# Sbte/RAILS

Hardware: AMD Instinct MI355X
Metric: RAILS iterations/sec (+ A*V SpMM HBM GB/s in roofline), m=1M rows/GPU, k=128, fp64 (higher is better)
Workload: dtype f64

## Files before the change

### include/rails_hip.h

```cpp
#ifndef RAILS_HIP_H
#define RAILS_HIP_H

#include <stddef.h>
#include <stdint.h>

#ifdef __cplusplus
extern "C" {
#endif

#define RAILS_OK 0
#define RAILS_EINVAL -1
#define RAILS_EHIP -2
#define RAILS_ENOMEM -3
#define RAILS_ELAPACK -4
#define RAILS_ECOMM -5
#define RAILS_ENODEV -6

typedef struct rails_ctx rails_ctx;
typedef struct rails_csr rails_csr;
typedef struct rails_panel rails_panel;

const char *rails_last_error(void);
const char *rails_version(void);

// ... 49 lines not shown
typedef struct rails_sptrsv rails_sptrsv;
int rails_sptrsv_create(rails_ctx *ctx, int64_t n, const int64_t *rowptr, const int32_t *col, const double *val, int lower, int unit_diag,
                        rails_sptrsv **out);
void rails_sptrsv_destroy(rails_sptrsv *T);
int64_t rails_sptrsv_levels(const rails_sptrsv *T);
int rails_sptrsv_solve(rails_ctx *ctx, const rails_sptrsv *T, rails_panel *X, int c0, int nc);
int rails_panel_permute_rows(rails_ctx *ctx, const rails_panel *X, int xc0, int nc, const int32_t *perm_dev, int scatter, rails_panel *Y, int yc0);
int rails_index_upload(rails_ctx *ctx, const int32_t *host, int64_t n, int32_t **out_dev);
void rails_index_free(rails_ctx *ctx, int32_t *dev);

typedef struct rails_lu rails_lu;
int rails_lu_create(rails_ctx *ctx, int64_t n, const int64_t *L_rowptr, const int32_t *L_col, const double *L_val, const int64_t *U_rowptr,
                    const int32_t *U_col, const double *U_val, const int32_t *perm_r, const int32_t *perm_c, const int32_t *rows, int64_t m_sub,
                    rails_lu **out);
void rails_lu_destroy(rails_lu *lu);
int rails_lu_solve(rails_ctx *ctx, rails_lu *lu, int trans, const rails_panel *X, int xc0, int nc, rails_panel *Y, int yc0);
int rails_lu_stats(const rails_lu *lu, int64_t *info, int cap);
int rails_csr_create_lu(rails_ctx *ctx, rails_lu *lu, rails_csr **out);


int rails_csr_transpose_host(int64_t n_rows, int64_t n_cols, const int64_t *rowptr, const int32_t *col, const double *val, int64_t *t_rowptr,
                             int32_t *t_col, double *t_val);
int rails_csr_gram_norm2_host(int64_t n_rows, int64_t n_cols, const int64_t *rowptr, const int32_t *col, const double *val,
                              const int64_t *t_rowptr, const int32_t *t_col, const double *t_val, double *out);

typedef struct rails_sprhs rails_sprhs;
int rails_sprhs_create(rails_ctx *ctx, int64_t m_local, int p, const int64_t *rowptr, const int32_t *col, const double *val, rails_sprhs **out);
void rails_sprhs_destroy(rails_sprhs *S);
int64_t rails_sprhs_rows(const rails_sprhs *S);
int64_t rails_sprhs_cols(const rails_sprhs *S);
int64_t rails_sprhs_nnz(const rails_sprhs *S);
double rails_sprhs_gram_norm2(const rails_sprhs *S);
int rails_sprhs_apply(rails_ctx *ctx, rails_sprhs *S, int trans, const rails_panel *X, int xc0, int nc, rails_panel *Y, int yc0);
int rails_csr_create_sprhs(rails_ctx *ctx, rails_sprhs *S, rails_csr **out);
int64_t rails_csr_cols(const rails_csr *A);
rails_sprhs *rails_csr_sprhs(const rails_csr *A);

typedef struct rails_sweep_plan rails_sweep_plan;
int rails_sweep_plan_create(int64_t m, int64_t ncols, const int64_t *rowptr, const int32_t *col, const double *val,
                            const int *params, rails_sweep_plan **out);
int rails_sweep_plan_destroy(rails_sweep_plan *plan);
int rails_sweep_plan_info(const rails_sweep_plan *plan, int64_t *iinfo, double *dinfo);
int rails_sweep_plan_array(const rails_sweep_plan *plan, int which, const void **ptr, int64_t *count);


int rails_panel_create(rails_ctx *ctx, int64_t m_local, int capacity, rails_panel **out);
int rails_panel_create_ld(rails_ctx *ctx, int64_t m_local, int capacity, int ld, rails_panel **out);
int rails_panel_destroy(rails_panel *P);
int64_t rails_panel_rows(const rails_panel *P);
int rails_panel_capacity(const rails_panel *P);
int rails_panel_ld(const rails_panel *P);
void *rails_panel_device_ptr(const rails_panel *P);
int rails_panel_reserve(rails_ctx *ctx, rails_panel *P, int capacity);

int rails_panel_upload(rails_ctx *ctx, rails_panel *P, int c0, int nc, const double *host, int64_t ldh);
int rails_panel_download(rails_ctx *ctx, const rails_panel *P, int c0, int nc, double *host, int64_t ldh);

int rails_panel_fill(rails_ctx *ctx, rails_panel *P, int c0, int nc, double value);
int rails_panel_scale(rails_ctx *ctx, rails_panel *P, int c0, int nc, double s);
int rails_panel_copy(rails_ctx *ctx, const rails_panel *X, int xc0, int nc, rails_panel *Y, int yc0);
int rails_panel_axpy(rails_ctx *ctx, double alpha, const rails_panel *X, int xc0, int nc, rails_panel *Y,
                     int yc0);
int rails_panel_random(rails_ctx *ctx, rails_panel *P, int c0, int nc);

int rails_gram(rails_ctx *ctx, const rails_panel *X, int xc0, int a, const rails_panel *Y, int yc0, int b,
               double *C_host, int ldc);

int rails_panel_gemm(rails_ctx *ctx, double alpha, const rails_panel *X, int xc0, int k, const double *C_host,
                     int ldc, int r, double beta, rails_panel *Y, int yc0);

int rails_ctx_enable_library_gemm(rails_ctx *ctx);
int rails_ctx_library_gemm_ready(const rails_ctx *ctx);

int rails_deferred_reserve(rails_ctx *ctx, int nslots, int64_t doubles_per_slot);
int rails_gram_deferred(rails_ctx *ctx, const rails_panel *X, int xc0, int a, const rails_panel *Y, int yc0, int b, int slot);
int rails_panel_gemm_deferred(rails_ctx *ctx, double alpha, const rails_panel *X, int xc0, int k, int slot, int ld, int r, double beta,
                              rails_panel *Y, int yc0);
int rails_chol_inverse_deferred(rails_ctx *ctx, int slot_in, int w, int slot_out);
int rails_update_gram_deferred(rails_ctx *ctx, double alpha, const rails_panel *X, int xc0, int k, const double *C_host, int ldc, int r,
                               rails_panel *Y, int yc0, int r2, int slot);
int rails_update_gram_deferred_out(rails_ctx *ctx, double alpha, const rails_panel *X, int xc0, int k, const double *C_host, int ldc, int r,
                                   const rails_panel *Y, int yc0, rails_panel *Yout, int oc0, int r2, int slot);
int rails_deferred_fetch(rails_ctx *ctx, int slot, int64_t n, double *host_out);

int rails_panel_gemm_wide(rails_ctx *ctx, double alpha, const rails_panel *X, int xc0, int k, const double *C_host, int ldc, int r,
                          double beta, rails_panel *Y, int yc0);

void rails_dense_set_tile_fit(int on);
int rails_dense_tile_fit(void);
int rails_dense_last_tiles(const rails_ctx *ctx, int *update_gram_nbw, int *gram_cols_ti, int *gemm_wide_tr);

int rails_orthogonalize(rails_ctx *ctx, rails_panel *V, int k_old, int w, int method, int *used);
int rails_orthogonalize_deflated(rails_ctx *ctx, rails_panel *V, int k_old, int w, const rails_panel *N, int nc0, int q, int method, int *used);

int rails_panel_colnorms2(rails_ctx *ctx, const rails_panel *X, int c0, int nc, double *out_host);

int rails_orthogonalize_range(rails_ctx *ctx, rails_panel *V, int k_old, int w, const rails_panel *N, int nc0, int q, double tol, int *kept,
                              int32_t *kept_idx);

int rails_resid_lanczos(rails_ctx *ctx, const rails_panel *AV, int avc0, const rails_panel *MV, int mvc0, int k,
                        const double *T_host, int ldt, const rails_panel *B, int bc0, int p, int L,
                        double *H_host, int ldh, int *steps);

int rails_resid_lanczos_sparse(rails_ctx *ctx, const rails_panel *AV, int avc0, const rails_panel *MV, int mvc0, int k, const double *T_host,
                               int ldt, const rails_sprhs *S, int L, double *H_host, int ldh, int *steps);

int rails_lanczos_start(rails_ctx *ctx, const rails_panel *AV, int avc0, const rails_panel *MV, int mvc0, int k,
                        const rails_panel *B, int bc0, int p, double *sums_host);

int rails_lanczos_vectors(rails_ctx *ctx, const double *S_host, int lds, int w, rails_panel *Out, int oc0);
int rails_lanczos_last_launch(rails_ctx *ctx, int *nch, int *unroll, int *nblocks);
int rails_lanczos_release(rails_ctx *ctx);

int rails_ctx_reserve_staging(rails_ctx *ctx, size_t bytes);
int rails_timer_start(rails_ctx *ctx);
int rails_timer_stop(rails_ctx *ctx, double *ms);


void rails_sb03md(char dico, char job, char fact, char trans, int n, double *A, int lda, double *X, int ldx,
                  double *scale, int *info);
void rails_sb03md_counts(long *smith, long *schur);
void rails_sb03md_adi_counts(long *extended, long *fresh);
void rails_sb03md_set_pause(int calls);
void rails_dsyev(char jobz, char uplo, int n, double *a, int lda, double *w, int *info);
void rails_dsteqr(char compz, int n, double *d, double *e, double *z, int ldz, double *work, int *info);
void rails_dgemm(char transa, char transb, int m, int n, int k, double alpha, const double *A, int lda, const double *B,
                 int ldb, double beta, double *C, int ldc);
void rails_dtrsm(char side, char uplo, char transa, char diag, int m, int n, double alpha, const double *A, int lda, double *B, int ldb);
void rails_dpotrf(char uplo, int n, double *a, int lda, int *info);
void rails_dpstrf(char uplo, int n, double *a, int lda, int *piv, int *rank, double tol, int *info);
void rails_range_basis(int m, int n, double *a, int lda, double tol, double *q, int ldq, int *rank, int *info);
int rails_host_lapack_init(const char *path);
const char *rails_host_lapack_path(void);

#ifdef __cplusplus
}
#endif
#endif
```

### rails_amd/_lib.py

```python
import ctypes as C
import os

_HERE = os.path.dirname(os.path.abspath(__file__))
LIB_PATH = os.path.join(_HERE, "lib", "librails_hip.so")

_dp = C.POINTER(C.c_double)
_ip = C.POINTER(C.c_int)
_i64p = C.POINTER(C.c_int64)
_i32p = C.POINTER(C.c_int32)
_vp = C.c_void_p

ALLREDUCE_FN = C.CFUNCTYPE(C.c_int, C.c_void_p, C.c_void_p, C.c_size_t, C.c_void_p)
HALO_FN = C.CFUNCTYPE(C.c_int, C.c_void_p, C.c_void_p, C.c_void_p, C.c_int, C.c_void_p)
APPLY_FN = C.CFUNCTYPE(C.c_int, C.c_void_p, C.c_int, C.c_void_p, C.c_int, C.c_int, C.c_void_p, C.c_int)

SIGNATURES = {
    "rails_last_error": (C.c_char_p, []),
    "rails_version": (C.c_char_p, []),
    "rails_ctx_create": (C.c_int, [C.c_int, _vp, C.POINTER(_vp)]),
    "rails_ctx_destroy": (C.c_int, [_vp]),
    "rails_ctx_sync": (C.c_int, [_vp]),
    "rails_ctx_stream": (_vp, [_vp]),
    "rails_ctx_set_meter": (C.c_int, [_vp, C.c_int]),
    "rails_ctx_enable_library_gemm": (C.c_int, [_vp]),
    "rails_ctx_library_gemm_ready": (C.c_int, [_vp]),
    "rails_deferred_reserve": (C.c_int, [_vp, C.c_int, C.c_int64]),
    "rails_gram_deferred": (C.c_int, [_vp, _vp, C.c_int, C.c_int, _vp, C.c_int, C.c_int, C.c_int]),
    "rails_update_gram_deferred": (C.c_int, [_vp, C.c_double, _vp, C.c_int, C.c_int, _dp, C.c_int, C.c_int, _vp, C.c_int, C.c_int, C.c_int]),
    "rails_update_gram_deferred_out": (C.c_int, [_vp, C.c_double, _vp, C.c_int, C.c_int, _dp, C.c_int, C.c_int, _vp, C.c_int, _vp, C.c_int, C.c_int, C.c_int]),
    "rails_panel_gemm_deferred": (C.c_int, [_vp, C.c_double, _vp, C.c_int, C.c_int, C.c_int, C.c_int, C.c_int, C.c_double, _vp, C.c_int]),
    "rails_chol_inverse_deferred": (C.c_int, [_vp, C.c_int, C.c_int, C.c_int]),
    "rails_deferred_fetch": (C.c_int, [_vp, C.c_int, C.c_int64, _dp]),
    "rails_ctx_stats": (C.c_int, [_vp, C.c_char_p, C.c_int]),
    "rails_ctx_set_seed": (C.c_int, [_vp, C.c_uint64, C.c_uint64]),
    "rails_ctx_rng_state": (C.c_int, [_vp, C.POINTER(C.c_uint64), C.POINTER(C.c_uint64)]),
    "rails_ctx_set_partition": (C.c_int, [_vp, C.c_int, C.c_int, C.c_int64, C.c_int64]),
    "rails_ctx_set_allreduce": (C.c_int, [_vp, ALLREDUCE_FN, _vp]),
    "rails_rccl_unique_id": (C.c_int, [_vp]),
    "rails_ctx_init_rccl": (C.c_int, [_vp, _vp, C.c_int, C.c_int]),
    "rails_ctx_set_rccl": (C.c_int, [_vp, _vp]),
    "rails_ctx_rccl_size": (C.c_int, [_vp]),
    "rails_csr_set_halo_counts": (C.c_int, [_vp, C.c_int, _i64p, _i64p]),
    "rails_csr_create": (C.c_int, [_vp, C.c_int64, C.c_int64, _i64p, _i32p, _dp, C.POINTER(_vp)]),
    "rails_csr_create_rect": (C.c_int, [_vp, C.c_int64, C.c_int64, _i64p, _i32p, _dp, C.POINTER(_vp)]),
    "rails_csr_create_callback": (C.c_int, [_vp, C.c_int64, APPLY_FN, _vp, C.POINTER(_vp)]),
    "rails_csr_destroy": (C.c_int, [_vp]),
    "rails_csr_rows": (C.c_int64, [_vp]),
    "rails_csr_nnz": (C.c_int64, [_vp]),
    "rails_csr_set_halo": (C.c_int, [_vp, C.c_int64, _i64p, C.c_int64, HALO_FN, _vp]),
    "rails_spmm": (C.c_int, [_vp, _vp, C.c_int, _vp, C.c_int, C.c_int, _vp, C.c_int]),
    "rails_csr_set_variant": (C.c_int, [_vp, C.c_int]),
    "rails_csr_sweep_stats": (C.c_int, [_vp, C.c_int, _dp]),
    "rails_csr_tile_stats": (C.c_int, [_vp, _dp]),
    "rails_csr_prepare": (C.c_int, [_vp, _vp, C.c_int, C.c_int, C.POINTER(C.c_int)]),
    "rails_csr_last_kernel": (C.c_char_p, [_vp]),
    "rails_sweep_plan_create": (C.c_int, [C.c_int64, C.c_int64, _i64p, _i32p, _dp, _ip, C.POINTER(_vp)]),
    "rails_sweep_plan_destroy": (C.c_int, [_vp]),
    "rails_sweep_plan_info": (C.c_int, [_vp, _i64p, _dp]),
    "rails_sweep_plan_array": (C.c_int, [_vp, C.c_int, C.POINTER(_vp), _i64p]),
    "rails_panel_create": (C.c_int, [_vp, C.c_int64, C.c_int, C.POINTER(_vp)]),
    "rails_panel_create_ld": (C.c_int, [_vp, C.c_int64, C.c_int, C.c_int, C.POINTER(_vp)]),
    "rails_panel_destroy": (C.c_int, [_vp]),
    "rails_panel_rows": (C.c_int64, [_vp]),
    "rails_panel_capacity": (C.c_int, [_vp]),
    "rails_panel_ld": (C.c_int, [_vp]),
    "rails_panel_device_ptr": (_vp, [_vp]),
    "rails_panel_reserve": (C.c_int, [_vp, _vp, C.c_int]),
    "rails_panel_upload": (C.c_int, [_vp, _vp, C.c_int, C.c_int, _dp, C.c_int64]),
    "rails_panel_download": (C.c_int, [_vp, _vp, C.c_int, C.c_int, _dp, C.c_int64]),
    "rails_panel_fill": (C.c_int, [_vp, _vp, C.c_int, C.c_int, C.c_double]),
    "rails_panel_scale": (C.c_int, [_vp, _vp, C.c_int, C.c_int, C.c_double]),
    "rails_panel_copy": (C.c_int, [_vp, _vp, C.c_int, C.c_int, _vp, C.c_int]),
    "rails_panel_axpy": (C.c_int, [_vp, C.c_double, _vp, C.c_int, C.c_int, _vp, C.c_int]),
    "rails_sptrsv_create": (C.c_int, [_vp, C.c_int64, _i64p, _i32p, _dp, C.c_int, C.c_int, C.POINTER(_vp)]),
    "rails_sptrsv_destroy": (None, [_vp]),
    "rails_sptrsv_levels": (C.c_int64, [_vp]),
    "rails_sptrsv_solve": (C.c_int, [_vp, _vp, _vp, C.c_int, C.c_int]),
    "rails_panel_permute_rows": (C.c_int, [_vp, _vp, C.c_int, C.c_int, _vp, C.c_int, _vp, C.c_int]),
    "rails_index_upload": (C.c_int, [_vp, _i32p, C.c_int64, C.POINTER(_vp)]),
    "rails_index_free": (None, [_vp, _vp]),
    "rails_lu_create": (C.c_int, [_vp, C.c_int64, _i64p, _i32p, _dp, _i64p, _i32p, _dp, _i32p, _i32p, _i32p, C.c_int64, C.POINTER(_vp)]),
    "rails_lu_destroy": (None, [_vp]),
    "rails_lu_solve": (C.c_int, [_vp, _vp, C.c_int, _vp, C.c_int, C.c_int, _vp, C.c_int]),
    "rails_lu_stats": (C.c_int, [_vp, _i64p, C.c_int]),
    "rails_csr_create_lu": (C.c_int, [_vp, _vp, C.POINTER(_vp)]),
    "rails_csr_transpose_host": (C.c_int, [C.c_int64, C.c_int64, _i64p, _i32p, _dp, _i64p, _i32p, _dp]),
    "rails_csr_gram_norm2_host": (C.c_int, [C.c_int64, C.c_int64, _i64p, _i32p, _dp, _i64p, _i32p, _dp, _dp]),
    "rails_sprhs_create": (C.c_int, [_vp, C.c_int64, C.c_int, _i64p, _i32p, _dp, C.POINTER(_vp)]),
    "rails_sprhs_destroy": (None, [_vp]),
    "rails_sprhs_rows": (C.c_int64, [_vp]),
    "rails_sprhs_cols": (C.c_int64, [_vp]),
    "rails_sprhs_nnz": (C.c_int64, [_vp]),
    "rails_sprhs_gram_norm2": (C.c_double, [_vp]),
    "rails_sprhs_apply": (C.c_int, [_vp, _vp, C.c_int, _vp, C.c_int, C.c_int, _vp, C.c_int]),
    "rails_csr_create_sprhs": (C.c_int, [_vp, _vp, C.POINTER(_vp)]),
    "rails_csr_cols": (C.c_int64, [_vp]),
    "rails_csr_sprhs": (_vp, [_vp]),
    "rails_resid_lanczos_sparse": (C.c_int, [_vp, _vp, C.c_int, _vp, C.c_int, C.c_int, _dp, C.c_int, _vp, C.c_int, _dp, C.c_int, _ip]),
    "rails_panel_random": (C.c_int, [_vp, _vp, C.c_int, C.c_int]),
    "rails_gram": (C.c_int, [_vp, _vp, C.c_int, C.c_int, _vp, C.c_int, C.c_int, _dp, C.c_int]),
    "rails_panel_gemm": (C.c_int, [_vp, C.c_double, _vp, C.c_int, C.c_int, _dp, C.c_int, C.c_int, C.c_double, _vp, C.c_int]),
    "rails_panel_gemm_wide": (C.c_int, [_vp, C.c_double, _vp, C.c_int, C.c_int, _dp, C.c_int, C.c_int, C.c_double, _vp, C.c_int]),
    "rails_dense_set_tile_fit": (None, [C.c_int]),
    "rails_dense_tile_fit": (C.c_int, []),
    "rails_dense_last_tiles": (C.c_int, [_vp, _ip, _ip, _ip]),
    "rails_orthogonalize": (C.c_int, [_vp, _vp, C.c_int, C.c_int, C.c_int, _ip]),
    "rails_orthogonalize_deflated": (C.c_int, [_vp, _vp, C.c_int, C.c_int, _vp, C.c_int, C.c_int, C.c_int, _ip]),
    "rails_panel_colnorms2": (C.c_int, [_vp, _vp, C.c_int, C.c_int, _dp]),
    "rails_orthogonalize_range": (C.c_int, [_vp, _vp, C.c_int, C.c_int, _vp, C.c_int, C.c_int, C.c_double, _ip, _i32p]),
    "rails_resid_lanczos": (C.c_int, [_vp, _vp, C.c_int, _vp, C.c_int, C.c_int, _dp, C.c_int, _vp, C.c_int, C.c_int, C.c_int,
                                      _dp, C.c_int, _ip]),
    "rails_lanczos_start": (C.c_int, [_vp, _vp, C.c_int, _vp, C.c_int, C.c_int, _vp, C.c_int, C.c_int, _dp]),
    "rails_lanczos_vectors": (C.c_int, [_vp, _dp, C.c_int, C.c_int, _vp, C.c_int]),
    "rails_lanczos_last_launch": (C.c_int, [_vp, _ip, _ip, _ip]),
    "rails_lanczos_release": (C.c_int, [_vp]),
# ... 55 lines not shown
```

### rails_amd/csrc/ctx.hip

```cpp
#include "rails_internal.h"

static thread_local char g_err[1024] = "";

void rails_set_error(const char *fmt, ...)
{
    va_list ap;
    va_start(ap, fmt);
    vsnprintf(g_err, sizeof(g_err), fmt, ap);
    va_end(ap);
}

extern "C" const char *rails_last_error(void) { return g_err; }
extern "C" const char *rails_version(void) { return "rails_amd 0.1 (gfx950)"; }


extern "C" int rails_ctx_create(int device, void *stream, rails_ctx **out)
{
    RAILS_REQUIRE(out != nullptr, "rails_ctx_create: out is null");
    int ndev = 0;
    hipError_t e = hipGetDeviceCount(&ndev);
    if (e != hipSuccess || ndev <= 0) {
        rails_set_error("rails_ctx_create: no HIP device visible (%s); the HIP path has no CPU fallback",
                        e == hipSuccess ? "device count 0" : hipGetErrorString(e));
        return RAILS_ENODEV;
// ... 4 lines not shown
    RAILS_HIP_CHECK(hipGetDeviceProperties(&prop, device));
    if (strncmp(prop.gcnArchName, "gfx950", 6) != 0) {
        rails_set_error("rails_ctx_create: device %d is %s; this library is built for gfx950 only", device,
                        prop.gcnArchName);
        return RAILS_ENODEV;
    }
    rails_ctx *c = new rails_ctx();
    c->device = device;
    c->num_cu = prop.multiProcessorCount;
    hipError_t he = hipSuccess;
    if (stream) {
        c->stream = (hipStream_t)stream;
        c->own_stream = false;
    } else {
        he = hipStreamCreateWithFlags(&c->stream, hipStreamNonBlocking);
        c->own_stream = he == hipSuccess;
    }
    if (he == hipSuccess) he = hipEventCreate(&c->ev0);
    if (he == hipSuccess) he = hipEventCreate(&c->ev1);
    if (he == hipSuccess) he = hipEventCreateWithFlags(&c->ev_h2d, hipEventDisableTiming);
    if (he != hipSuccess) {
        rails_set_error("rails_ctx_create: stream / event creation failed: %s", hipGetErrorString(he));
        if (c->ev0) hipEventDestroy(c->ev0);
        if (c->ev1) hipEventDestroy(c->ev1);
        if (c->ev_h2d) hipEventDestroy(c->ev_h2d);
    for (hipEvent_t e : c->meter_events) hipEventDestroy(e);
        if (c->own_stream) hipStreamDestroy(c->stream);
        delete c;
        return RAILS_EHIP;
    }
    rails_host_lapack_init(nullptr);
    *out = c;
    return RAILS_OK;
}

extern "C" int rails_ctx_destroy(rails_ctx *c)
{
    if (!c) return RAILS_OK;
    hipSetDevice(c->device);
    rails_stream_sync(c);
    rails_lanczos_release(c);
    rails_rccl_release(c);
    rails_library_gemm_release(c);
    for (auto &fp : c->free_panels) hipFree(fp.second);
    c->free_panels.clear();
    if (c->ws) hipFree(c->ws);
    if (c->small) hipFree(c->small);
    if (c->pinned) hipHostFree(c->pinned);
    if (c->defer_dev) hipFree(c->defer_dev);
    if (c->defer_pin) hipHostFree(c->defer_pin);
    if (c->ev0) hipEventDestroy(c->ev0);
    if (c->ev1) hipEventDestroy(c->ev1);
    if (c->ev_h2d) hipEventDestroy(c->ev_h2d);
    for (hipEvent_t e : c->meter_events) hipEventDestroy(e);
    if (c->stream2) hipStreamDestroy(c->stream2);
    if (c->ev_fork) hipEventDestroy(c->ev_fork);
    if (c->ev_join) hipEventDestroy(c->ev_join);
    if (c->own_stream) hipStreamDestroy(c->stream);
    delete c;
    return RAILS_OK;
}

int rails_ctx_second_stream(rails_ctx *c)
{
    if (c->stream2) return RAILS_OK;
    RAILS_HIP_CHECK(hipStreamCreateWithFlags(&c->stream2, hipStreamNonBlocking));
    RAILS_HIP_CHECK(hipEventCreateWithFlags(&c->ev_fork, hipEventDisableTiming));
    RAILS_HIP_CHECK(hipEventCreateWithFlags(&c->ev_join, hipEventDisableTiming));
    return RAILS_OK;
}

extern "C" int rails_ctx_sync(rails_ctx *c)
{
    RAILS_REQUIRE(c, "rails_ctx_sync: null context");
    RAILS_HIP_CHECK(rails_stream_sync(c));
    return RAILS_OK;
}

extern "C" int rails_ctx_stats(rails_ctx *c, char *buf, int cap)
{
    RAILS_REQUIRE(c && buf && cap > 0, "rails_ctx_stats: bad argument");
    int n = snprintf(buf, (size_t)cap,
                     "{\"orth_block\": %ld, \"orth_columnwise\": %ld, \"spmm_tiled\": %ld, \"spmm_planes\": %ld, \"spmm_halo_overlapped\": %ld, \"spmm_sweep\": %ld, \"spmm_rowgather\": %ld, \"spmm_callback\": %ld, \"device_allocations\": %ld, \"allreduce\": %ld, "
                     "\"lanczos\": %ld, \"lanczos_start\": %ld, \"orth_repair\": %ld, \"update_gram_fused\": %ld, \"rowquad\": %ld, \"orth_range\": %ld, \"orth_range_passes\": %ld, \"orth_range_syncs\": %ld, \"gpu_busy_ms\": %.3f}",
                     c->n_orth_block, c->n_orth_columnwise, c->n_spmm_tiled, c->n_spmm_planes, c->n_spmm_overlapped, c->n_spmm_sweep, c->n_spmm_rowgather, c->n_spmm_callback, c->n_dev_alloc, c->n_allreduce, c->n_lanczos, c->n_lanczos_start, c->n_orth_repair, c->n_update_gram_fused, c->n_rowquad, c->n_orth_range, c->n_orth_range_passes, c->n_orth_range_syncs, c->gpu_busy_ms);
    RAILS_REQUIRE(n > 0 && n < cap, "rails_ctx_stats: buffer too small");
    return RAILS_OK;
}

extern "C" void *rails_ctx_stream(rails_ctx *c) { return c ? (void *)c->stream : nullptr; }

extern "C" int rails_ctx_set_meter(rails_ctx *c, int on)
{
    RAILS_REQUIRE(c, "rails_ctx_set_meter: null context");
    hipSetDevice(c->device);
    RAILS_HIP_CHECK(rails_stream_sync(c));
    if (on && c->meter_events.empty()) {
        c->meter_events.resize(2 * RAILS_METER_PAIRS, nullptr);
        for (hipEvent_t &e : c->meter_events) RAILS_HIP_CHECK(hipEventCreate(&e));
    }
    c->meter = on != 0;
    return RAILS_OK;
}

extern "C" int rails_ctx_rng_state(rails_ctx *c, uint64_t *seed, uint64_t *next_stream)
{
    RAILS_REQUIRE(c && seed && next_stream, "rails_ctx_rng_state: null argument");
    *seed = c->seed;
    *next_stream = c->next_stream;
    return RAILS_OK;
}

extern "C" int rails_ctx_set_seed(rails_ctx *c, uint64_t seed, uint64_t first_stream)
{
    RAILS_REQUIRE(c, "null context");
    c->seed = seed;
    c->next_stream = first_stream;
    return RAILS_OK;
}

extern "C" int rails_ctx_set_partition(rails_ctx *c, int rank, int nranks, int64_t row0, int64_t m_global)
{
    RAILS_REQUIRE(c, "null context");
    RAILS_REQUIRE(nranks >= 1 && rank >= 0 && rank < nranks && row0 >= 0, "rails_ctx_set_partition: bad rank %d/%d row0 %lld",
                  rank, nranks, (long long)row0);
    c->rank = rank;
    c->nranks = nranks;
    c->row0 = row0;
    c->m_global = m_global;
    return RAILS_OK;
}

extern "C" int rails_ctx_set_allreduce(rails_ctx *c, rails_allreduce_fn fn, void *user)
{
    RAILS_REQUIRE(c, "null context");
    c->allreduce = fn;
    c->allreduce_user = user;
    return RAILS_OK;
}

int rails_allreduce_dev(rails_ctx *c, double *dev, size_t n)
{
    if (n == 0) return RAILS_OK;
    if (c->nranks <= 1 && !c->allreduce && !c->rccl) return RAILS_OK;
    if (!c->allreduce && c->rccl) {
        c->n_allreduce++;
        return rails_rccl_allreduce(c, dev, n);
    }
    if (!c->allreduce) {
        rails_set_error("row-partitioned run (nranks=%d) with neither an RCCL communicator (rails_ctx_init_rccl) nor an all-reduce hook", c->nranks);
        return RAILS_ECOMM;
    }
    c->n_allreduce++;
    int rc = c->allreduce(c->allreduce_user, dev, n, (void *)c->stream);
    if (rc != 0) {
        rails_set_error("all-reduce hook failed with code %d", rc);
        return RAILS_ECOMM;
    }
    return RAILS_OK;
}

static int grow(rails_ctx *c, double **p, size_t *have, size_t need, bool host)
{
    if (need <= *have) return RAILS_OK;
    RAILS_HIP_CHECK(rails_stream_sync(c));
    if (*p) {
        if (host)
            RAILS_HIP_CHECK(hipHostFree(*p));
        else
            RAILS_HIP_CHECK(hipFree(*p));
        *p = nullptr;
        *have = 0;
    }
// ... 213 lines not shown
        tile[i][tx] = (r < m && cc < nc) ? P[r * ld + cc] : 0.0;
    }
    __syncthreads();
    for (int j = ty; j < 32; j += 8) {
        int64_t r = r0 + tx;
        int cc = c0 + j;
        if (r < m && cc < nc) tmp[(int64_t)cc * m + r] = tile[tx][j];
    }
}

extern "C" int rails_panel_upload(rails_ctx *c, rails_panel *P, int c0, int nc, const double *host, int64_t ldh)
{
    if (c) hipSetDevice(c->device);
    RAILS_TRY(check_window(P, c0, nc, "rails_panel_upload"));
    RAILS_REQUIRE(host || nc == 0 || P->m == 0, "rails_panel_upload: null host buffer");
    RAILS_REQUIRE(ldh >= P->m, "rails_panel_upload: ldh %lld < rows %lld", (long long)ldh, (long long)P->m);
    if (nc == 0 || P->m == 0) return RAILS_OK;
    const int chunk = 32;
    RAILS_TRY(rails_ws_reserve(c, (size_t)P->m * chunk * sizeof(double)));
    for (int j0 = 0; j0 < nc; j0 += chunk) {
        int n = nc - j0 < chunk ? nc - j0 : chunk;
        RAILS_HIP_CHECK(hipMemcpy2DAsync(c->ws, (size_t)P->m * sizeof(double), host + (int64_t)j0 * ldh, (size_t)ldh * sizeof(double),
                                         (size_t)P->m * sizeof(double), n, hipMemcpyHostToDevice, c->stream));
        dim3 grid((unsigned)((P->m + 31) / 32), (unsigned)((n + 31) / 32));
        RAILS_LAUNCH(k_scatter_cm_to_panel, grid, dim3(256), 0, c->stream, c->ws, P->d + c0 + j0, P->ld, P->m, n);
        RAILS_HIP_CHECK(rails_stream_sync(c));
    }
    RAILS_HIP_CHECK(hipGetLastError());
    return RAILS_OK;
}

extern "C" int rails_panel_download(rails_ctx *c, const rails_panel *P, int c0, int nc, double *host, int64_t ldh)
{
    if (c) hipSetDevice(c->device);
    RAILS_TRY(check_window(P, c0, nc, "rails_panel_download"));
    RAILS_REQUIRE(host || nc == 0 || P->m == 0, "rails_panel_download: null host buffer");
    RAILS_REQUIRE(ldh >= P->m, "rails_panel_download: ldh %lld < rows %lld", (long long)ldh, (long long)P->m);
    if (nc == 0 || P->m == 0) return RAILS_OK;
    const int chunk = 32;
    RAILS_TRY(rails_ws_reserve(c, (size_t)P->m * chunk * sizeof(double)));
    for (int j0 = 0; j0 < nc; j0 += chunk) {
        int n = nc - j0 < chunk ? nc - j0 : chunk;
        dim3 grid((unsigned)((P->m + 31) / 32), (unsigned)((n + 31) / 32));
        RAILS_LAUNCH(k_gather_panel_to_cm, grid, dim3(256), 0, c->stream, P->d + c0 + j0, P->ld, c->ws, P->m, n);
        RAILS_HIP_CHECK(hipMemcpy2DAsync(host + (int64_t)j0 * ldh, (size_t)ldh * sizeof(double), c->ws, (size_t)P->m * sizeof(double),
                                         (size_t)P->m * sizeof(double), n, hipMemcpyDeviceToHost, c->stream));
        RAILS_HIP_CHECK(rails_stream_sync(c));
    }
    RAILS_HIP_CHECK(hipGetLastError());
    return RAILS_OK;
}


__global__ void k_fill(double *__restrict__ P, int ld, int64_t m, int nc, double v)
{
    int64_t total = m * nc;
    for (int64_t idx = (int64_t)blockIdx.x * blockDim.x + threadIdx.x; idx < total; idx += (int64_t)gridDim.x * blockDim.x) {
        int64_t r = idx / nc;
        int cidx = (int)(idx - r * nc);
        P[r * ld + cidx] = v;
    }
}

__global__ void k_scale(double *__restrict__ P, int ld, int64_t m, int nc, double s)
{
    int64_t total = m * nc;
    for (int64_t idx = (int64_t)blockIdx.x * blockDim.x + threadIdx.x; idx < total; idx += (int64_t)gridDim.x * blockDim.x) {
        int64_t r = idx / nc;
        int cidx = (int)(idx - r * nc);
        P[r * ld + cidx] *= s;
    }
}

__global__ void k_axpy(double alpha, const double *__restrict__ X, int ldx, double *__restrict__ Y, int ldy, int64_t m, int nc)
{
    int64_t total = m * nc;
    for (int64_t idx = (int64_t)blockIdx.x * blockDim.x + threadIdx.x; idx < total; idx += (int64_t)gridDim.x * blockDim.x) {
        int64_t r = idx / nc;
        int cidx = (int)(idx - r * nc);
        Y[r * ldy + cidx] += alpha * X[r * ldx + cidx];
    }
}

__device__ __forceinline__ uint64_t splitmix64(uint64_t x)
{
    x += 0x9E3779B97F4A7C15ull;
    x = (x ^ (x >> 30)) * 0xBF58476D1CE4E5B9ull;
    x = (x ^ (x >> 27)) * 0x94D049BB133111EBull;
    return x ^ (x >> 31);
}

__global__ void k_random(double *__restrict__ P, int ld, int64_t m, int nc, uint64_t seed, uint64_t stream, int64_t row0)
{
    uint64_t hs = splitmix64(seed ^ splitmix64(stream * 0xD1342543DE82EF95ull + 0x632BE59BD9B4E019ull));
    int64_t total = m * nc;
    for (int64_t idx = (int64_t)blockIdx.x * blockDim.x + threadIdx.x; idx < total; idx += (int64_t)gridDim.x * blockDim.x) {
        int64_t r = idx / nc;
        int cidx = (int)(idx - r * nc);
        uint64_t h = splitmix64(hs ^ splitmix64((uint64_t)(row0 + r) * 0x9E3779B97F4A7C15ull + (uint64_t)cidx * 0xC2B2AE3D27D4EB4Full + 1));
        double u = (double)(h >> 11) * (1.0 / 9007199254740992.0);
        P[r * ld + cidx] = 2.0 * u - 1.0;
    }
}

extern "C" int rails_panel_fill(rails_ctx *c, rails_panel *P, int c0, int nc, double value)
{
    if (c) hipSetDevice(c->device);
    RAILS_TRY(check_window(P, c0, nc, "rails_panel_fill"));
    if (nc == 0 || P->m == 0) return RAILS_OK;
    RAILS_LAUNCH(k_fill, dim3(grid_for(c, P->m * nc, 256)), dim3(256), 0, c->stream, P->d + c0, P->ld, P->m, nc, value);
    RAILS_HIP_CHECK(hipGetLastError());
    return RAILS_OK;
}

extern "C" int rails_panel_scale(rails_ctx *c, rails_panel *P, int c0, int nc, double s)
{
    RAILS_TRY(check_window(P, c0, nc, "rails_panel_scale"));
    if (nc == 0 || P->m == 0) return RAILS_OK;
    RAILS_LAUNCH(k_scale, dim3(grid_for(c, P->m * nc, 256)), dim3(256), 0, c->stream, P->d + c0, P->ld, P->m, nc, s);
    RAILS_HIP_CHECK(hipGetLastError());
    return RAILS_OK;
}

extern "C" int rails_panel_copy(rails_ctx *c, const rails_panel *X, int xc0, int nc, rails_panel *Y, int yc0)
{
    RAILS_TRY(check_window(X, xc0, nc, "rails_panel_copy(X)"));
    RAILS_TRY(check_window(Y, yc0, nc, "rails_panel_copy(Y)"));
    RAILS_REQUIRE(X->m == Y->m, "rails_panel_copy: row mismatch %lld vs %lld", (long long)X->m, (long long)Y->m);
    if (nc == 0 || X->m == 0) return RAILS_OK;
    if (X->d == Y->d) {
        if (xc0 == yc0) return RAILS_OK;
        RAILS_REQUIRE(xc0 + nc <= yc0 || yc0 + nc <= xc0, "rails_panel_copy: overlapping windows of one panel");
    }
    RAILS_LAUNCH(k_copy2d, dim3(grid_for(c, X->m * nc, 256)), dim3(256), 0, c->stream, X->d + xc0, X->ld, Y->d + yc0,
                       Y->ld, X->m, nc);
    RAILS_HIP_CHECK(hipGetLastError());
    return RAILS_OK;
}

extern "C" int rails_panel_axpy(rails_ctx *c, double alpha, const rails_panel *X, int xc0, int nc, rails_panel *Y, int yc0)
{
    RAILS_TRY(check_window(X, xc0, nc, "rails_panel_axpy(X)"));
    RAILS_TRY(check_window(Y, yc0, nc, "rails_panel_axpy(Y)"));
    RAILS_REQUIRE(X->m == Y->m, "rails_panel_axpy: row mismatch %lld vs %lld", (long long)X->m, (long long)Y->m);
    if (nc == 0 || X->m == 0) return RAILS_OK;
    RAILS_LAUNCH(k_axpy, dim3(grid_for(c, X->m * nc, 256)), dim3(256), 0, c->stream, alpha, X->d + xc0, X->ld,
                       Y->d + yc0, Y->ld, X->m, nc);
    RAILS_HIP_CHECK(hipGetLastError());
    return RAILS_OK;
}

extern "C" int rails_panel_random(rails_ctx *c, rails_panel *P, int c0, int nc)
{
    if (c) hipSetDevice(c->device);
    RAILS_TRY(check_window(P, c0, nc, "rails_panel_random"));
    uint64_t s = c->next_stream++;
    if (nc == 0 || P->m == 0) return RAILS_OK;
    RAILS_LAUNCH(k_random, dim3(grid_for(c, P->m * nc, 256)), dim3(256), 0, c->stream, P->d + c0, P->ld, P->m, nc,
                       c->seed, s, c->row0);
    RAILS_HIP_CHECK(hipGetLastError());
    return RAILS_OK;
}
```

### rails_amd/csrc/dense.hip

```cpp
#include "rails_internal.h"

#include <dlfcn.h>
#include <atomic>
#include <mutex>

#include <algorithm>

namespace {

typedef double v4f64 __attribute__((ext_vector_type(4)));
typedef double v2f64 __attribute__((ext_vector_type(2)));

std::atomic<int> g_tile_fit{-1};

bool dense_tile_fit()
{
    int v = g_tile_fit.load(std::memory_order_relaxed);
    if (v < 0) {
        const char *e = getenv("RAILS_DENSE_TILE_FIT");
        int undecided = -1;
        g_tile_fit.compare_exchange_strong(undecided, (e ? atoi(e) : 1) ? 1 : 0);
        v = g_tile_fit.load(std::memory_order_relaxed);
    }
    return v != 0;
}

__device__ __forceinline__ v4f64 mfma_f64(double a, double b, v4f64 c)
{
    return __builtin_amdgcn_mfma_f64_16x16x4f64(a, b, c, 0, 0, 0);
}

struct OneSeg {
    const double *X;
    int ld;
    struct Row {
        const double *x;
    };
    __device__ int col(int c) const { return c; }
    __device__ Row row(int64_t r) const { return {X + r * ld}; }
    __device__ static const double *at(Row r, int c) { return r.x + c; }
};
struct TwoSeg {
    const double *X1;
    int ld1, a1;
    const double *X2;
    int ld2;
    struct Col {
        int off;
        bool second;
    };
    struct Row {
        const double *x1, *x2;
    };
    __device__ Col col(int c) const
    {
        const bool second = c >= a1;
        return {second ? c - a1 : c, second};
    }
    __device__ Row row(int64_t r) const { return {X1 + r * ld1, X2 + r * ld2}; }
    __device__ static const double *at(Row r, Col c) { return (c.second ? r.x2 : r.x1) + c.off; }
};

template <int TI, int TJ>
__global__ __launch_bounds__(256) __attribute__((amdgpu_waves_per_eu(3, 8))) void k_gram(const double *__restrict__ X, int ldx, int a, const double *__restrict__ Y, int ldy,
                                              int b, int64_t m, int64_t rows_per_slab, int ngj, double *__restrict__ partial)
{
    const OneSeg Xo{X, ldx};
#include "dense_gram.inc"
}

template <int TI, int TJ>
__global__ __launch_bounds__(256) void k_gram2(const double *__restrict__ X1, int ldx1, int a1, const double *__restrict__ X2, int ldx2, int a,
                                               const double *__restrict__ Y, int ldy, int b, int64_t m, int64_t rows_per_slab, int ngj,
                                               double *__restrict__ partial)
{
    const TwoSeg Xo{X1, ldx1, a1, X2, ldx2};
#include "dense_gram.inc"
}

template <int TI, int TJ, int NE = 0>
__global__ __launch_bounds__(256) __attribute__((amdgpu_waves_per_eu(3, 8))) void k_gram_cols(const double *__restrict__ X, int ldx, int a,
                                                                                             const double *__restrict__ Y, int ldy, int b, int64_t m,
                                                                                             int64_t rows_per_slab, double *__restrict__ partial)
{
    const OneSeg Xo{X, ldx};
#include "dense_gram_cols.inc"
}

template <int TI, int TJ, int NE>
__global__ __launch_bounds__(256) void k_gram_cols2(const double *__restrict__ X1, int ldx1, int a1, const double *__restrict__ X2, int ldx2, int a,
                                                    const double *__restrict__ Y, int ldy, int b, int64_t m, int64_t rows_per_slab,
                                                    double *__restrict__ partial)
{
    const TwoSeg Xo{X1, ldx1, a1, X2, ldx2};
#include "dense_gram_cols.inc"
}

__global__ __launch_bounds__(1024) void k_reduce_partials(const double *__restrict__ partial, int64_t nslab, int64_t n, double *__restrict__ out)
{
    __shared__ double sh[16][64];
    const int tx = threadIdx.x & 63, ty = threadIdx.x >> 6;
    const int64_t e = (int64_t)blockIdx.x * 64 + tx;
    double s = 0.0;
    if (e < n)
        for (int64_t t = ty; t < nslab; t += 16) s += partial[t * n + e];
    sh[ty][tx] = s;
    __syncthreads();
    if (ty == 0 && e < n) {
        double r = 0.0;
#pragma unroll
        for (int g = 0; g < 16; ++g) r += sh[g][tx];
        out[e] = r;
    }
}

template <int TI, int TJ>
void launch_gram(rails_ctx *c, const double *X, int ldx, int a, const double *Y, int ldy, int b, int64_t m, int64_t rps,
                 int64_t nslab, double *partial)
{
    int ngi = (a + 16 * TI - 1) / (16 * TI), ngj = (b + 16 * TJ - 1) / (16 * TJ);
    RAILS_LAUNCH((k_gram<TI, TJ>), dim3((unsigned)nslab, (unsigned)(ngi * ngj)), dim3(256), 0, c->stream, X, ldx, a, Y, ldy, b,
                       m, rps, ngj, partial);
}

template <int TI, int TJ>
void launch_gram2(rails_ctx *c, const double *X1, int ldx1, int a1, const double *X2, int ldx2, int a, const double *Y, int ldy, int b, int64_t m,
                  int64_t rps, int64_t nslab, double *partial)
{
    int ngi = (a + 16 * TI - 1) / (16 * TI), ngj = (b + 16 * TJ - 1) / (16 * TJ);
    RAILS_LAUNCH((k_gram2<TI, TJ>), dim3((unsigned)nslab, (unsigned)(ngi * ngj)), dim3(256), 0, c->stream, X1, ldx1, a1, X2, ldx2, a, Y, ldy, b,
                 m, rps, ngj, partial);
}

template <int TR, int KC>
__global__ __launch_bounds__(256) void k_panel_gemm(double alpha, const double *X, int ldx, int k,
                                                    const double *__restrict__ C, int r, double beta, double *Yp,
                                                    int ldy, int64_t m, int vec_ok)
{
    const OneSeg Xo{X, ldx};
#define RAILS_PG_VEC4(c) (vec_ok && (c) + 4 <= k)
#include "dense_panel_gemm.inc"
}

template <int TR, int KC>
__global__ __launch_bounds__(256) void k_panel_gemm2(double alpha, const double *X1, int ldx1, int a1, const double *X2, int ldx2, int a,
                                                     const double *__restrict__ C, int r, double beta, double *Yp, int ldy, int64_t m, int vec1,
                                                     int vec2)
{
    const TwoSeg Xo{X1, ldx1, a1, X2, ldx2};
    const int k = a;
#define RAILS_PG_VEC4(c) (((c) + 4 <= a1 && vec1) || ((c) >= a1 && (c) + 4 <= a && vec2))
#include "dense_panel_gemm.inc"
}

template <int TR, int KC>
void launch_pg(rails_ctx *c, double alpha, const double *X, int ldx, int k, const double *C, int r, double beta, double *Y,
               int ldy, int64_t m, int vec_ok)
{
    int64_t grid = (m + 63) / 64;
    RAILS_LAUNCH((k_panel_gemm<TR, KC>), dim3((unsigned)grid), dim3(256), 0, c->stream, alpha, X, ldx, k, C, r, beta, Y,
                       ldy, m, vec_ok);
}

__global__ void k_pack_ct(const double *__restrict__ C, int k, int r, int kpad, int RL, double *__restrict__ out)
{
    const int64_t n = (int64_t)kpad * RL;
    for (int64_t q = (int64_t)blockIdx.x * blockDim.x + threadIdx.x; q < n; q += (int64_t)gridDim.x * blockDim.x) {
        const int kl = (int)(q / RL), j = (int)(q % RL);
        out[q] = (kl < k && j < r) ? C[kl + (int64_t)j * k] : 0.0;
    }
}

template <int TR>
__global__ __launch_bounds__(512) void k_panel_gemm_wide(double alpha, const double *__restrict__ X, int ldx, int k, const double *__restrict__ Ct ,
                                                         int r, double beta, double *__restrict__ Yp, int ldy, int64_t m, int vec_ok, int skip_tail)
{
    constexpr int KC = 32, RL = 16 * TR + 4, CHUNK_B = KC * RL * 8, PIECES = CHUNK_B / 1024;
    static_assert(CHUNK_B % 1024 == 0, "whole LDS-DMA pieces per chunk");
    extern __shared__ double Cs[];
    const int lane = threadIdx.x & 63;
    const int wave = __builtin_amdgcn_readfirstlane((int)(threadIdx.x >> 6));
    const int li = lane & 15, kk = lane >> 4;
    const int64_t r0 = ((int64_t)blockIdx.x * 8 + wave) * 16;
    const int64_t myrow = r0 + li;
    const bool rowok = myrow < m;
    const int nchunks = (k + KC - 1) / KC;
    const uint32_t lds_base = (uint32_t)(uintptr_t)(__attribute__((address_space(3))) unsigned char *)Cs;
    const uint32_t lane16 = (uint32_t)lane * 16u;
    auto stage = [&](int chunk) {
        const char *src = reinterpret_cast<const char *>(Ct) + (size_t)chunk * CHUNK_B;
        const uint32_t dst = lds_base + (uint32_t)((chunk & 1) * CHUNK_B);
        for (int p = wave; p < PIECES; p += 8) {
            uint32_t keep;
            asm volatile("s_mov_b32 %0, m0\n\ts_mov_b32 m0, %3\n\ts_nop 0\n\tglobal_load_lds_dwordx4 %1, %2\n\ts_mov_b32 m0, %0"
                         : "=&s"(keep) : "v"(lane16), "s"(src + (size_t)p * 1024), "s"(dst + (uint32_t)(p * 1024)) : "memory");
// ... 73 lines not shown
    const int kpad = (k + 31) / 32 * 32;
    RAILS_LAUNCH(k_pack_ct, dim3((unsigned)std::min<int64_t>(512, ((int64_t)kpad * RL + 255) / 256)), dim3(256), 0, c->stream, C, k, r, kpad, RL, ct);
    const size_t lds = (size_t)2 * 32 * RL * sizeof(double);
    RAILS_HIP_CHECK(hipFuncSetAttribute((const void *)k_panel_gemm_wide<TR>, hipFuncAttributeMaxDynamicSharedMemorySize, (int)lds));
    RAILS_LAUNCH((k_panel_gemm_wide<TR>), dim3((unsigned)((m + 127) / 128)), dim3(512), lds, c->stream, alpha, X, ldx, k, ct, r, beta, Y, ldy, m, vec_ok,
                 dense_tile_fit() ? 1 : 0);
    c->last_gemm_wide_tr = TR;
    return RAILS_OK;
}

void gram_slabs(int64_t m, int a, int b, int64_t *nslab_out, int64_t *rps_out)
{
    double bound = 0.02 * (double)m * (double)(a + b) / ((double)a * (double)b);
    int64_t nslab = (int64_t)std::min<double>(1024.0, std::max<double>(1.0, bound));
    int64_t maxslab = (m + 15) / 16;
    if (nslab > maxslab) nslab = std::max<int64_t>(1, maxslab);
    int64_t rps = (m + nslab - 1) / nslab;
    rps = (rps + 15) / 16 * 16;
    if (rps < 16) rps = 16;
    *nslab_out = std::max<int64_t>(1, (m + rps - 1) / rps);
    *rps_out = rps;
}

int gram_cols_tiles(int ntiles, bool one_tile)
{
    const int cand2[3] = {3, 4, 5}, cand1[3] = {4, 6, 8};
    const int *cand = one_tile ? cand1 : cand2;
    int best = cand[1], best_cost = 1 << 30;
    for (int q = 0; q < 3; ++q) {
        int ti = cand[q], strips = (ntiles + ti - 1) / ti, cost = (strips + 3) / 4 * 4 * ti;
        if (cost < best_cost) best = ti, best_cost = cost;
    }
    if (one_tile && best == 6 && (ntiles + 4) / 5 == (ntiles + 5) / 6 && dense_tile_fit()) best = 5;
    return best;
}

#define RAILS_GRAM_COLS_CASE(K, TI, TJ, NE, ...) RAILS_LAUNCH((K<TI, TJ, NE>), grid, dim3(256), 0, c->stream, __VA_ARGS__, Y, ldy, b, m, rps, c->ws)
#define RAILS_GRAM_COLS(K, ...)                                                                                                            \
    do {                                                                                                                                   \
        const int ntiles = (a + 15) / 16, best = gram_cols_tiles(ntiles, b <= 16 || extra);                                                \
        const dim3 grid((unsigned)nslab, (unsigned)(((ntiles + best - 1) / best + 3) / 4));                                                \
        c->last_gram_cols_ti = best;                                                                                                       \
        if (extra) {                                                                                                                       \
            if (best == 4)                                                                                                                 \
                RAILS_GRAM_COLS_CASE(K, 4, 1, 1, __VA_ARGS__);                                                                             \
            else if (best == 5)                                                                                                            \
                RAILS_GRAM_COLS_CASE(K, 5, 1, 1, __VA_ARGS__);                                                                             \
            else if (best == 6)                                                                                                            \
                RAILS_GRAM_COLS_CASE(K, 6, 1, 1, __VA_ARGS__);                                                                             \
            else                                                                                                                           \
                RAILS_GRAM_COLS_CASE(K, 8, 1, 1, __VA_ARGS__);                                                                             \
        } else if (b <= 16) {                                                                                                              \
            if (best == 4)                                                                                                                 \
                RAILS_GRAM_COLS_CASE(K, 4, 1, 0, __VA_ARGS__);                                                                             \
            else if (best == 5)                                                                                                            \
                RAILS_GRAM_COLS_CASE(K, 5, 1, 0, __VA_ARGS__);                                                                             \
            else if (best == 6)                                                                                                            \
                RAILS_GRAM_COLS_CASE(K, 6, 1, 0, __VA_ARGS__);                                                                             \
            else                                                                                                                           \
                RAILS_GRAM_COLS_CASE(K, 8, 1, 0, __VA_ARGS__);                                                                             \
        } else if (best == 3)                                                                                                              \
            RAILS_GRAM_COLS_CASE(K, 3, 2, 0, __VA_ARGS__);                                                                                 \
        else if (best == 4)                                                                                                                \
            RAILS_GRAM_COLS_CASE(K, 4, 2, 0, __VA_ARGS__);                                                                                 \
        else                                                                                                                               \
            RAILS_GRAM_COLS_CASE(K, 5, 2, 0, __VA_ARGS__);                                                                                 \
    } while (0)

}

extern "C" void rails_dense_set_tile_fit(int on) { g_tile_fit.store(on ? 1 : 0); }

extern "C" int rails_dense_tile_fit(void) { return dense_tile_fit() ? 1 : 0; }

extern "C" int rails_dense_last_tiles(const rails_ctx *c, int *update_gram_nbw, int *gram_cols_ti, int *gemm_wide_tr)
{
    RAILS_REQUIRE(c, "rails_dense_last_tiles: null context");
    if (update_gram_nbw) *update_gram_nbw = c->last_update_gram_nbw;
    if (gram_cols_ti) *gram_cols_ti = c->last_gram_cols_ti;
    if (gemm_wide_tr) *gemm_wide_tr = c->last_gemm_wide_tr;
    return RAILS_OK;
}

int rails_gram_dev(rails_ctx *c, const double *X, int ldx, const double *Y, int ldy, int64_t m, int a, int b, double *C_dev)
{
    if (a <= 0 || b <= 0) return RAILS_OK;
    int64_t nslab, rps;
    gram_slabs(m, a, b, &nslab, &rps);
    size_t n = (size_t)a * b;
    RAILS_TRY(rails_ws_reserve(c, (size_t)nslab * n * sizeof(double)));
    if (b <= 16 && a <= 16)
        launch_gram<1, 1>(c, X, ldx, a, Y, ldy, b, m, rps, nslab, c->ws);
    else if (b <= 32 && a >= 128) {
        static const int cols_form = getenv("RAILS_GRAM_COLS") ? atoi(getenv("RAILS_GRAM_COLS")) : 1;
        if (cols_form) {
            static const int extra_env = getenv("RAILS_GRAM_EXTRA_COLUMN") ? atoi(getenv("RAILS_GRAM_EXTRA_COLUMN")) : 1;
            const bool extra = extra_env && b == 17;
            RAILS_GRAM_COLS(k_gram_cols, X, ldx, a);
        } else if (b <= 16)
            launch_gram<8, 1>(c, X, ldx, a, Y, ldy, b, m, rps, nslab, c->ws);
        else
            launch_gram<4, 2>(c, X, ldx, a, Y, ldy, b, m, rps, nslab, c->ws);
    } else if (b <= 16)
        launch_gram<8, 1>(c, X, ldx, a, Y, ldy, b, m, rps, nslab, c->ws);
    else if (a <= 16)
        launch_gram<1, 8>(c, X, ldx, a, Y, ldy, b, m, rps, nslab, c->ws);
    else if (a <= 32 && b <= 32)
        launch_gram<2, 2>(c, X, ldx, a, Y, ldy, b, m, rps, nslab, c->ws);
    else if (b <= 32)
        launch_gram<4, 2>(c, X, ldx, a, Y, ldy, b, m, rps, nslab, c->ws);
    else if (a <= 32)
        launch_gram<2, 4>(c, X, ldx, a, Y, ldy, b, m, rps, nslab, c->ws);
    else
        launch_gram<2, 4>(c, X, ldx, a, Y, ldy, b, m, rps, nslab, c->ws);
    RAILS_LAUNCH(k_reduce_partials, dim3((unsigned)((n + 63) / 64)), dim3(1024), 0, c->stream, c->ws, nslab, (int64_t)n, C_dev);
    RAILS_HIP_CHECK(hipGetLastError());
    return RAILS_OK;
}

int rails_gram2_dev(rails_ctx *c, const double *X1, int ldx1, int a1, const double *X2, int ldx2, int a2, const double *Y, int ldy, int64_t m, int b,
                    double *C_dev)
{
    const int a = a1 + a2;
    if (a <= 0 || b <= 0) return RAILS_OK;
    int64_t nslab, rps;
    gram_slabs(m, a, b, &nslab, &rps);
    const size_t n = (size_t)a * b;
    RAILS_TRY(rails_ws_reserve(c, (size_t)nslab * n * sizeof(double)));
    if (a >= 128 && b <= 32) {
        const bool extra = b == 17;
        RAILS_GRAM_COLS(k_gram_cols2, X1, ldx1, a1, X2, ldx2, a);
    } else if (a <= 16 && b <= 16)
        launch_gram2<1, 1>(c, X1, ldx1, a1, X2, ldx2, a, Y, ldy, b, m, rps, nslab, c->ws);
    else if (b <= 16)
        launch_gram2<8, 1>(c, X1, ldx1, a1, X2, ldx2, a, Y, ldy, b, m, rps, nslab, c->ws);
    else
        launch_gram2<4, 2>(c, X1, ldx1, a1, X2, ldx2, a, Y, ldy, b, m, rps, nslab, c->ws);
    RAILS_LAUNCH(k_reduce_partials, dim3((unsigned)((n + 63) / 64)), dim3(1024), 0, c->stream, c->ws, nslab, (int64_t)n, C_dev);
    RAILS_HIP_CHECK(hipGetLastError());
    return RAILS_OK;
}

extern "C" int rails_gram(rails_ctx *c, const rails_panel *X, int xc0, int a, const rails_panel *Y, int yc0, int b, double *C_host,
                          int ldc)
{
    if (c) hipSetDevice(c->device);
    rails_slow_guard slow__(c, "rails_gram", a, b);
    RAILS_REQUIRE(c && X && Y, "rails_gram: null argument");
    RAILS_REQUIRE(a >= 0 && b >= 0 && xc0 >= 0 && yc0 >= 0 && xc0 + a <= X->cap && yc0 + b <= Y->cap,
                  "rails_gram: windows [%d,%d) / [%d,%d) outside capacities %d / %d", xc0, xc0 + a, yc0, yc0 + b, X->cap, Y->cap);
    RAILS_REQUIRE(X->m == Y->m, "rails_gram: row mismatch %lld vs %lld", (long long)X->m, (long long)Y->m);
    RAILS_REQUIRE(a == 0 || b == 0 || (C_host && ldc >= a), "rails_gram: bad output buffer (ldc %d < %d)", ldc, a);
    if (a == 0 || b == 0) return RAILS_OK;
    size_t n = (size_t)a * b;
    RAILS_TRY(rails_small_reserve(c, n * sizeof(double)));
    RAILS_TRY(rails_pinned_reserve(c, n * sizeof(double)));
    if (X->m > 0)
        RAILS_TRY(rails_gram_dev(c, X->d + xc0, X->ld, Y->d + yc0, Y->ld, X->m, a, b, c->small));
    else
        RAILS_HIP_CHECK(hipMemsetAsync(c->small, 0, n * sizeof(double), c->stream));
    RAILS_TRY(rails_allreduce_dev(c, c->small, n));
    RAILS_HIP_CHECK(hipMemcpyAsync(c->pinned, c->small, n * sizeof(double), hipMemcpyDeviceToHost, c->stream));
    RAILS_HIP_CHECK(rails_stream_sync(c));
    for (int j = 0; j < b; ++j) memcpy(C_host + (size_t)j * ldc, c->pinned + (size_t)j * a, sizeof(double) * a);
    return RAILS_OK;
}

namespace {

__global__ __launch_bounds__(256) void k_colnorms2(const double *__restrict__ X, int ldx, int nc, int64_t m, int64_t rows_per_slab, int tx_bits,
                                                   int vec_ok, double *__restrict__ partial)
{
    __shared__ double sh[256][2];
    const int TX = 1 << tx_bits, TY = 256 >> tx_bits;
    const int tx = threadIdx.x & (TX - 1), ty = threadIdx.x >> tx_bits;
    const int c = 2 * tx;
    const bool has0 = c < nc, has1 = c + 1 < nc;
    const int64_t r_begin = (int64_t)blockIdx.x * rows_per_slab;
    const int64_t r_end = r_begin + rows_per_slab < m ? r_begin + rows_per_slab : m;
    double s0[4] = {0.0, 0.0, 0.0, 0.0}, s1[4] = {0.0, 0.0, 0.0, 0.0};
    if (has0) {
        const bool pair = has1 && vec_ok;
        auto load = [&](int64_t r, double &a, double &b) {
            const double *src = X + r * ldx + c;
            if (pair) {
                const v2f64 t = *reinterpret_cast<const v2f64 *>(src);
                a = t.x;
                b = t.y;
            } else {
                a = src[0];
                b = has1 ? src[1] : 0.0;
            }
        };
        int64_t r = r_begin + ty;
        for (; r + 3 * (int64_t)TY < r_end; r += 4 * (int64_t)TY) {
            double a[4], b[4];
#pragma unroll
            for (int s = 0; s < 4; ++s) load(r + s * (int64_t)TY, a[s], b[s]);
#pragma unroll
            for (int s = 0; s < 4; ++s) {
                s0[s] += a[s] * a[s];
                s1[s] += b[s] * b[s];
            }
        }
#pragma unroll
        for (int s = 0; s < 3; ++s)
            if (r + s * (int64_t)TY < r_end) {
                double a, b;
                load(r + s * (int64_t)TY, a, b);
                s0[s] += a * a;
                s1[s] += b * b;
            }
    }
    sh[threadIdx.x][0] = ((s0[0] + s0[1]) + s0[2]) + s0[3];
    sh[threadIdx.x][1] = ((s1[0] + s1[1]) + s1[2]) + s1[3];
    __syncthreads();
    for (int half = TY >> 1; half > 0; half >>= 1) {
        if (ty < half) {
            sh[threadIdx.x][0] += sh[threadIdx.x + (half << tx_bits)][0];
            sh[threadIdx.x][1] += sh[threadIdx.x + (half << tx_bits)][1];
        }
        __syncthreads();
    }
    if (ty == 0 && has0) {
        double *dst = partial + (int64_t)blockIdx.x * nc + c;
        dst[0] = sh[tx][0];
        if (has1) dst[1] = sh[tx][1];
    }
}

}

int rails_colnorms2_dev(rails_ctx *c, const double *X, int ldx, int64_t m, int nc, double *out_dev)
{
    if (nc <= 0) return RAILS_OK;
    if (m <= 0) {
        RAILS_HIP_CHECK(hipMemsetAsync(out_dev, 0, (size_t)nc * sizeof(double), c->stream));
        return RAILS_OK;
    }
    const int pairs = (nc + 1) / 2;
    int tx_bits = 0;
    while ((1 << tx_bits) < pairs) ++tx_bits;
    const int TY = 256 >> tx_bits;
    int64_t nslab = std::max<int64_t>(1, std::min<int64_t>(1024, m / ((int64_t)TY * 8)));
    const int64_t rps = (m + nslab - 1) / nslab;
    nslab = (m + rps - 1) / rps;
    RAILS_TRY(rails_ws_reserve(c, (size_t)nslab * nc * sizeof(double)));
    const int vec_ok = ((((uintptr_t)X) & 15) == 0 && (ldx % 2) == 0) ? 1 : 0;
    RAILS_LAUNCH(k_colnorms2, dim3((unsigned)nslab), dim3(256), 0, c->stream, X, ldx, nc, m, rps, tx_bits, vec_ok, c->ws);
    RAILS_LAUNCH(k_reduce_partials, dim3((unsigned)((nc + 63) / 64)), dim3(1024), 0, c->stream, c->ws, nslab, (int64_t)nc, out_dev);
    RAILS_HIP_CHECK(hipGetLastError());
    return RAILS_OK;
}

extern "C" int rails_panel_colnorms2(rails_ctx *c, const rails_panel *X, int c0, int nc, double *out_host)
{
    if (c) hipSetDevice(c->device);
    RAILS_REQUIRE(c && X, "rails_panel_colnorms2: null argument");
    RAILS_REQUIRE(c0 >= 0 && nc >= 0 && c0 + nc <= X->cap, "rails_panel_colnorms2: window [%d,%d) outside capacity %d", c0, c0 + nc, X->cap);
    RAILS_REQUIRE(nc == 0 || out_host, "rails_panel_colnorms2: null output buffer");
    if (nc == 0) return RAILS_OK;
    RAILS_TRY(rails_small_reserve(c, (size_t)nc * sizeof(double)));
    RAILS_TRY(rails_pinned_reserve(c, (size_t)nc * sizeof(double)));
    for (int j0 = 0; j0 < nc; j0 += 512)
        RAILS_TRY(rails_colnorms2_dev(c, X->d + c0 + j0, X->ld, X->m, std::min(512, nc - j0), c->small + j0));
    RAILS_TRY(rails_allreduce_dev(c, c->small, (size_t)nc));
    RAILS_HIP_CHECK(hipMemcpyAsync(c->pinned, c->small, (size_t)nc * sizeof(double), hipMemcpyDeviceToHost, c->stream));
    RAILS_HIP_CHECK(rails_stream_sync(c));
    memcpy(out_host, c->pinned, (size_t)nc * sizeof(double));
    return RAILS_OK;
}


namespace {

__global__ void k_compact_cols(const double *__restrict__ src, int ld, int k, int r, double *__restrict__ dst)
{
    const int64_t n = (int64_t)k * r;
    for (int64_t q = (int64_t)blockIdx.x * blockDim.x + threadIdx.x; q < n; q += (int64_t)gridDim.x * blockDim.x) dst[q] = src[(q / k) * ld + (q % k)];
}

__global__ __launch_bounds__(64) void k_small_chol(const double *__restrict__ G, int w, double *__restrict__ M)
{
    constexpr int LD = 49;
    __shared__ double S[48 * LD], Ri[48 * LD], d[48];
    const int t = threadIdx.x;
    const bool mine = t < w;
    for (int q = t; q < w * w; q += 64) S[(q / w) * LD + (q % w)] = G[q];
    __syncthreads();
    if (mine) d[t] = sqrt(S[t * LD + t]);
    __syncthreads();
    for (int q = t; q < w * w; q += 64) S[(q / w) * LD + (q % w)] /= d[q % w] * d[q / w];
    __syncthreads();
    for (int i = 0; i < w; ++i) {
        const double piv = sqrt(S[i * LD + i]);
        double rij = 0.0;
        if (mine && t >= i) rij = (t == i) ? piv : S[t * LD + i] / piv;
        __syncthreads();
        if (mine && t >= i) S[t * LD + i] = rij;
        __syncthreads();
        if (mine && t > i)
            for (int l = i + 1; l <= t; ++l) S[t * LD + l] -= S[l * LD + i] * rij;
        __syncthreads();
    }
    if (mine) {
        for (int l = 0; l < w; ++l) Ri[t * LD + l] = 0.0;
        for (int i = t; i >= 0; --i) {
            double s = (i == t) ? 1.0 : 0.0;
            for (int l = i + 1; l <= t; ++l) s -= S[l * LD + i] * Ri[t * LD + l];
            Ri[t * LD + i] = s / S[i * LD + i];
        }
    }
    __syncthreads();
    for (int q = t; q < w * w; q += 64) {
        const int j = q / w, i = q % w;
        M[q] = i <= j ? Ri[j * LD + i] / d[i] : 0.0;
    }
}

}

extern "C" int rails_deferred_reserve(rails_ctx *c, int nslots, int64_t doubles_per_slot)
{
    RAILS_REQUIRE(c && nslots >= 1 && doubles_per_slot >= 1, "rails_deferred_reserve: bad argument");
    hipSetDevice(c->device);
    if (c->defer_dev && c->defer_nslots >= nslots && c->defer_slot >= (size_t)doubles_per_slot) return RAILS_OK;
    RAILS_HIP_CHECK(rails_stream_sync(c));
    if (c->defer_dev) hipFree(c->defer_dev);
    if (c->defer_pin) hipHostFree(c->defer_pin);
    c->defer_dev = c->defer_pin = nullptr;
    const size_t slot = ((size_t)doubles_per_slot * 3 / 2 + 63) / 64 * 64, bytes = slot * (size_t)nslots * sizeof(double);
    c->n_dev_alloc++;
    RAILS_HIP_CHECK(hipMalloc((void **)&c->defer_dev, bytes));
    RAILS_HIP_CHECK(hipHostMalloc((void **)&c->defer_pin, bytes, hipHostMallocDefault));
    c->defer_slot = slot;
    c->defer_nslots = nslots;
    return RAILS_OK;
}

#define RAILS_SLOT_CHECK(slot, n, what)                                                                                                    \
    RAILS_REQUIRE(c && c->defer_dev && (slot) >= 0 && (slot) < c->defer_nslots && (size_t)(n) <= c->defer_slot,                            \
                  what ": slot %d / %lld doubles outside the arena (rails_deferred_reserve)", (int)(slot), (long long)(n))

extern "C" int rails_gram_deferred(rails_ctx *c, const rails_panel *X, int xc0, int a, const rails_panel *Y, int yc0, int b, int slot)
{
    if (c) hipSetDevice(c->device);
    RAILS_REQUIRE(c && X && Y, "rails_gram_deferred: null argument");
    RAILS_REQUIRE(a >= 1 && b >= 1 && xc0 >= 0 && yc0 >= 0 && xc0 + a <= X->cap && yc0 + b <= Y->cap && X->m == Y->m, "rails_gram_deferred: bad windows");
    const size_t n = (size_t)a * b;
    RAILS_SLOT_CHECK(slot, n, "rails_gram_deferred");
    double *out = c->defer_dev + (size_t)slot * c->defer_slot;
    if (X->m > 0)
        RAILS_TRY(rails_gram_dev(c, X->d + xc0, X->ld, Y->d + yc0, Y->ld, X->m, a, b, out));
    else
        RAILS_HIP_CHECK(hipMemsetAsync(out, 0, n * sizeof(double), c->stream));
    RAILS_TRY(rails_allreduce_dev(c, out, n));
    RAILS_HIP_CHECK(hipMemcpyAsync(c->defer_pin + (size_t)slot * c->defer_slot, out, n * sizeof(double), hipMemcpyDeviceToHost, c->stream));
    return RAILS_OK;
}

extern "C" int rails_panel_gemm_deferred(rails_ctx *c, double alpha, const rails_panel *X, int xc0, int k, int slot, int ld, int r, double beta,
                                         rails_panel *Y, int yc0)
{
    if (c) hipSetDevice(c->device);
    RAILS_REQUIRE(c && X && Y, "rails_panel_gemm_deferred: null argument");
    RAILS_REQUIRE(k >= 1 && r >= 1 && r <= 256 && ld >= k && xc0 >= 0 && yc0 >= 0 && xc0 + k <= X->cap && yc0 + r <= Y->cap && X->m == Y->m,
                  "rails_panel_gemm_deferred: bad shapes");
    RAILS_SLOT_CHECK(slot, (size_t)ld * r, "rails_panel_gemm_deferred");
    if (X->d == Y->d) RAILS_REQUIRE(xc0 == yc0 || xc0 + k <= yc0 || yc0 + r <= xc0, "rails_panel_gemm_deferred: partially overlapping windows of one panel");
    if (X->m == 0) return RAILS_OK;
    const double *C = c->defer_dev + (size_t)slot * c->defer_slot;
    if (ld != k) {
        RAILS_TRY(rails_small_reserve(c, (size_t)k * r * sizeof(double)));
        RAILS_LAUNCH(k_compact_cols, dim3((unsigned)std::min<int64_t>(256, ((int64_t)k * r + 255) / 256)), dim3(256), 0, c->stream, C, ld, k, r, c->small);
        C = c->small;
    }
    return rails_panel_gemm_dev(c, alpha, X->d + xc0, X->ld, k, C, r, beta, Y->d + yc0, Y->ld, X->m);
}

template <int NBW, int NE>
__global__ __launch_bounds__(256, (NBW <= 6 ? 2 : 1)) void k_update_gram(double alpha, const double *__restrict__ X, int ldx, int k, const double *__restrict__ C, int r,
                                                     const double *Yp, int ldy, double *Yo, int ldo, int r2, int64_t m, int64_t ntiles,
                                                     double *__restrict__ partial)
{
    constexpr int KMAX = 64 * NBW, RL = 20;
    __shared__ double Cs[KMAX * RL];
    __shared__ double red[4][4][64];
    __shared__ double rede[4][1][16];
    __shared__ double awL[16 * 16];
    __shared__ __attribute__((aligned(16))) double T[4][16 * 16];
    const int lane = threadIdx.x & 63, wave = threadIdx.x >> 6;
    const int li = lane & 15, kk = lane >> 4;
    for (int idx = threadIdx.x; idx < KMAX * RL; idx += 256) {
        const int kl = idx / RL, j = idx % RL;
        Cs[idx] = (kl < k && j < r) ? C[kl + (int64_t)j * k] : 0.0;
    }
    v4f64 acc2[NBW];
#pragma unroll
    for (int b = 0; b < NBW; ++b) acc2[b] = (v4f64){0.0, 0.0, 0.0, 0.0};

    const int k4 = (k + 3) & ~3;
    auto fetch = [&](int64_t tile, double (*xs)[4]) {
        const int64_t myrow = (tile < ntiles ? tile : ntiles - 1) * 16 + li;
        const double *xrow = X + (myrow < m ? myrow : m - 1) * ldx;
#pragma unroll
        for (int b = 0; b < NBW; ++b) {
            const int kcol = (b * 4 + wave) * 16 + 4 * kk;
            const double *src = xrow + (kcol < k4 ? kcol : 0);
            const v2f64 t0 = *reinterpret_cast<const v2f64 *>(src);
            const v2f64 t1 = *reinterpret_cast<const v2f64 *>(src + 2);
            xs[b][0] = t0.x;
            xs[b][1] = t0.y;
            xs[b][2] = t1.x;
            xs[b][3] = t1.y;
        }
    };
    const int erow = threadIdx.x & 15, ene = threadIdx.x >> 4;
    auto fetch_y = [&](int64_t tile, double &yv, double &ye) {
        const int64_t t16 = (tile < ntiles ? tile : ntiles - 1) * 16;
        const int64_t yrow = t16 + kk + 4 * wave, er = t16 + erow;
        yv = Yp[(yrow < m ? yrow : m - 1) * ldy + (li < r ? li : 0)];
        ye = NE > 0 ? Yp[(er < m ? er : m - 1) * ldy + (16 + ene < r ? 16 + ene : 0)] : 0.0;
    };
    auto work = [&](int64_t tile, double (*xs)[4], double yv, double ye, double (*xn)[4], double &yvn, double &yen) {
        const int64_t row0 = tile * 16;
        fetch(tile + gridDim.x, xn);
        fetch_y(tile + gridDim.x, yvn, yen);
        const int64_t yrow = row0 + kk + 4 * wave;
        const bool yok = yrow < m && li < r;
        const bool eok = ene < NE && 16 + ene < r && row0 + erow < m;
        v4f64 p = (v4f64){0.0, 0.0, 0.0, 0.0};
        double e[NE > 0 ? NE : 1];
#pragma unroll
        for (int q = 0; q < NE; ++q) e[q] = 0.0;
#pragma unroll
        for (int b = 0; b < NBW; ++b)
#pragma unroll
            for (int s = 0; s < 4; ++s) {
                const double *crow = &Cs[((b * 4 + wave) * 16 + 4 * kk + s) * RL];
                p = mfma_f64(xs[b][s], crow[li], p);
#pragma unroll
                for (int q = 0; q < NE; ++q) e[q] += xs[b][s] * crow[16 + q];
            }
#pragma unroll
        for (int v = 0; v < 4; ++v) red[wave][v][lane] = p[v];
#pragma unroll
        for (int q = 0; q < NE; ++q) {
            double t = e[q];
            t += __shfl_xor(t, 16, 64);
            t += __shfl_xor(t, 32, 64);
            if (kk == 0) rede[wave][q][li] = t;
        }
        __syncthreads();
        {
            const double sum = ((red[0][wave][lane] + red[1][wave][lane]) + red[2][wave][lane]) + red[3][wave][lane];
            const double ynew = yv + alpha * sum;
            if (yok) Yo[yrow * ldo + li] = ynew;
            awL[(kk + 4 * wave) * 16 + li] = (yok && li < r2) ? ynew : 0.0;
            if (NE > 0 && eok) {
                const double se = ((rede[0][ene][erow] + rede[1][ene][erow]) + rede[2][ene][erow]) + rede[3][ene][erow];
                Yo[(row0 + erow) * ldo + 16 + ene] = ye + alpha * se;
            }
        }
        __syncthreads();
        double bq[4];
#pragma unroll
        for (int q = 0; q < 4; ++q) bq[q] = awL[(4 * q + kk) * 16 + li];
        double *Tw = T[wave];
#pragma unroll
        for (int b = 0; b < NBW; ++b) {
            *reinterpret_cast<v2f64 *>(&Tw[li * 16 + 4 * kk]) = (v2f64){xs[b][0], xs[b][1]};
            *reinterpret_cast<v2f64 *>(&Tw[li * 16 + 4 * kk + 2]) = (v2f64){xs[b][2], xs[b][3]};
            __builtin_amdgcn_fence(__ATOMIC_RELEASE, "wavefront");
            __builtin_amdgcn_wave_barrier();
            __builtin_amdgcn_fence(__ATOMIC_ACQUIRE, "wavefront");
            double a4[4];
#pragma unroll
            for (int q = 0; q < 4; ++q) a4[q] = Tw[(4 * q + kk) * 16 + li];
            __builtin_amdgcn_fence(__ATOMIC_RELEASE, "wavefront");
            __builtin_amdgcn_wave_barrier();
#pragma unroll
            for (int q = 0; q < 4; ++q) acc2[b] = mfma_f64(a4[q], bq[q], acc2[b]);
        }
    };
    double xa[NBW][4], xb[NBW][4], yva, yea, yvb, yeb;
    fetch(blockIdx.x, xa);
    fetch_y(blockIdx.x, yva, yea);
    __syncthreads();
    for (int64_t tile = blockIdx.x; tile < ntiles; tile += 2 * (int64_t)gridDim.x) {
        work(tile, xa, yva, yea, xb, yvb, yeb);
        if (tile + gridDim.x < ntiles) work(tile + gridDim.x, xb, yvb, yeb, xa, yva, yea);
    }
    double *P = partial + (int64_t)blockIdx.x * k * r2;
#pragma unroll
    for (int b = 0; b < NBW; ++b)
#pragma unroll
        for (int v = 0; v < 4; ++v) {
            const int ci = (b * 4 + wave) * 16 + kk + 4 * v;
            if (ci < k && li < r2) P[ci + (int64_t)li * k] = acc2[b][v];
        }
}

template <int NBW>
static void launch_update_gram(rails_ctx *c, int ne, unsigned grid, double alpha, const double *X, int ldx, int k, const double *C, int r, const double *Y, int ldy,
                               double *Yo, int ldo, int r2, int64_t m, int64_t ntiles)
{
    if (ne == 0)
        RAILS_LAUNCH((k_update_gram<NBW, 0>), dim3(grid), dim3(256), 0, c->stream, alpha, X, ldx, k, C, r, Y, ldy, Yo, ldo, r2, m, ntiles, c->ws);
    else
        RAILS_LAUNCH((k_update_gram<NBW, 1>), dim3(grid), dim3(256), 0, c->stream, alpha, X, ldx, k, C, r, Y, ldy, Yo, ldo, r2, m, ntiles, c->ws);
    c->last_update_gram_nbw = NBW;
}

extern "C" int rails_update_gram_deferred_out(rails_ctx *c, double alpha, const rails_panel *X, int xc0, int k, const double *C_host, int ldc, int r,
                                              const rails_panel *Y, int yc0, rails_panel *Yout, int oc0, int r2, int slot)
{
    if (c) hipSetDevice(c->device);
    rails_slow_guard slow__(c, "rails_update_gram_deferred", k, r);
    RAILS_REQUIRE(c && X && Y && Yout && C_host, "rails_update_gram_deferred: null argument");
    RAILS_REQUIRE(k >= 1 && r >= 1 && r <= 256 && r2 >= 1 && r2 <= r && ldc >= k && xc0 >= 0 && yc0 >= 0 && xc0 + k <= X->cap && yc0 + r <= Y->cap && X->m == Y->m,
                  "rails_update_gram_deferred: bad shapes");
    RAILS_REQUIRE(oc0 >= 0 && oc0 + r <= Yout->cap && Yout->m == X->m, "rails_update_gram_deferred: output window [%d,%d) outside capacity %d, or row mismatch", oc0,
                  oc0 + r, Yout->cap);
    if (X->d == Y->d) RAILS_REQUIRE(xc0 + k <= yc0 || yc0 + r <= xc0, "rails_update_gram_deferred: overlapping windows of one panel");
    if (X->d == Yout->d) RAILS_REQUIRE(xc0 + k <= oc0 || oc0 + r <= xc0, "rails_update_gram_deferred: overlapping windows of one panel");
    if (Y->d == Yout->d) RAILS_REQUIRE(yc0 == oc0 || yc0 + r <= oc0 || oc0 + r <= yc0, "rails_update_gram_deferred: partially overlapping windows of one panel");
    const size_t n = (size_t)k * r2;
    RAILS_SLOT_CHECK(slot, n, "rails_update_gram_deferred");
    double *out = c->defer_dev + (size_t)slot * c->defer_slot;
    if (X->m == 0) {
        RAILS_HIP_CHECK(hipMemsetAsync(out, 0, n * sizeof(double), c->stream));
    } else {
        const size_t nc = (size_t)k * r;
        RAILS_TRY(rails_small_reserve(c, nc * sizeof(double)));
        RAILS_TRY(rails_pinned_begin_write(c, nc * sizeof(double)));
        for (int j = 0; j < r; ++j) memcpy(c->pinned + (size_t)j * k, C_host + (size_t)j * ldc, sizeof(double) * k);
        RAILS_HIP_CHECK(hipMemcpyAsync(c->small, c->pinned, nc * sizeof(double), hipMemcpyHostToDevice, c->stream));
        RAILS_TRY(rails_pinned_end_write(c));
        static const int fused_env = getenv("RAILS_FUSED_UPDATE_GRAM") ? atoi(getenv("RAILS_FUSED_UPDATE_GRAM")) : 1;
        const double *Xp = X->d + xc0;
        const double *Ypp = Y->d + yc0;
        double *Yop = Yout->d + oc0;
        const int k4 = (k + 3) & ~3;
        const bool rows_ok = ((((uintptr_t)Xp) & 15) == 0 && (X->ld % 2) == 0) && (k4 == k || (X->d == Y->d && yc0 == xc0 + k && r >= k4 - k));
        if (fused_env && rows_ok && r <= 17 && r2 <= 16 && k >= 32 && k <= 512 && X->m >= 4096) {
            const int64_t ntiles = (X->m + 15) / 16;
            const unsigned grid = (unsigned)std::min<int64_t>(ntiles, 2 * (int64_t)std::max(c->num_cu, 1));
            const int ne = r > 16 ? r - 16 : 0;
            RAILS_TRY(rails_ws_reserve(c, (size_t)grid * n * sizeof(double)));
            if (k <= 256)
                launch_update_gram<4>(c, ne, grid, alpha, Xp, X->ld, k, c->small, r, Ypp, Y->ld, Yop, Yout->ld, r2, X->m, ntiles);
            else if (k <= 320 && dense_tile_fit())
                launch_update_gram<5>(c, ne, grid, alpha, Xp, X->ld, k, c->small, r, Ypp, Y->ld, Yop, Yout->ld, r2, X->m, ntiles);
            else if (k <= 384)
                launch_update_gram<6>(c, ne, grid, alpha, Xp, X->ld, k, c->small, r, Ypp, Y->ld, Yop, Yout->ld, r2, X->m, ntiles);
            else
                launch_update_gram<8>(c, ne, grid, alpha, Xp, X->ld, k, c->small, r, Ypp, Y->ld, Yop, Yout->ld, r2, X->m, ntiles);
            RAILS_LAUNCH(k_reduce_partials, dim3((unsigned)((n + 63) / 64)), dim3(1024), 0, c->stream, c->ws, (int64_t)grid, (int64_t)n, out);
            RAILS_HIP_CHECK(hipGetLastError());
            c->n_update_gram_fused++;
        } else {
            if (Yop != Ypp) RAILS_TRY(rails_panel_copy(c, Y, yc0, r, Yout, oc0));
            RAILS_TRY(rails_panel_gemm_dev(c, alpha, Xp, X->ld, k, c->small, r, 1.0, Yop, Yout->ld, X->m));
            RAILS_TRY(rails_gram_dev(c, Xp, X->ld, Yop, Yout->ld, X->m, k, r2, out));
        }
    }
    RAILS_TRY(rails_allreduce_dev(c, out, n));
    RAILS_HIP_CHECK(hipMemcpyAsync(c->defer_pin + (size_t)slot * c->defer_slot, out, n * sizeof(double), hipMemcpyDeviceToHost, c->stream));
    return RAILS_OK;
}

extern "C" int rails_update_gram_deferred(rails_ctx *c, double alpha, const rails_panel *X, int xc0, int k, const double *C_host, int ldc, int r,
                                          rails_panel *Y, int yc0, int r2, int slot)
{
    return rails_update_gram_deferred_out(c, alpha, X, xc0, k, C_host, ldc, r, Y, yc0, Y, yc0, r2, slot);
}

extern "C" int rails_chol_inverse_deferred(rails_ctx *c, int slot_in, int w, int slot_out)
{
    if (c) hipSetDevice(c->device);
    RAILS_REQUIRE(c && w >= 1 && w <= 48 && slot_in != slot_out, "rails_chol_inverse_deferred: bad argument (w = %d)", w);
    RAILS_SLOT_CHECK(slot_in, (size_t)w * w, "rails_chol_inverse_deferred");
    RAILS_SLOT_CHECK(slot_out, (size_t)w * w, "rails_chol_inverse_deferred");
    RAILS_LAUNCH(k_small_chol, dim3(1), dim3(64), 0, c->stream, c->defer_dev + (size_t)slot_in * c->defer_slot, w, c->defer_dev + (size_t)slot_out * c->defer_slot);
    RAILS_HIP_CHECK(hipGetLastError());
    RAILS_HIP_CHECK(hipMemcpyAsync(c->defer_pin + (size_t)slot_out * c->defer_slot, c->defer_dev + (size_t)slot_out * c->defer_slot, (size_t)w * w * sizeof(double),
                                   hipMemcpyDeviceToHost, c->stream));
    return RAILS_OK;
}

extern "C" int rails_deferred_fetch(rails_ctx *c, int slot, int64_t n, double *host_out)
{
    RAILS_REQUIRE(host_out && n >= 0, "rails_deferred_fetch: bad argument");
    RAILS_SLOT_CHECK(slot, n, "rails_deferred_fetch");
    memcpy(host_out, c->defer_pin + (size_t)slot * c->defer_slot, (size_t)n * sizeof(double));
    return RAILS_OK;
}

int rails_panel_gemm_dev(rails_ctx *c, double alpha, const double *X, int ldx, int k, const double *C_dev, int r, double beta,
                         double *Y, int ldy, int64_t m)
{
    if (r <= 0 || m <= 0) return RAILS_OK;
    int vec_ok = ((((uintptr_t)X) & 15) == 0 && (ldx % 2) == 0) ? 1 : 0;
    int tr = (r + 15) / 16;
    if (tr <= 1)
        launch_pg<1, 32>(c, alpha, X, ldx, k, C_dev, r, beta, Y, ldy, m, vec_ok);
    else if (tr <= 2)
        launch_pg<2, 32>(c, alpha, X, ldx, k, C_dev, r, beta, Y, ldy, m, vec_ok);
    else if (tr <= 4)
        launch_pg<4, 32>(c, alpha, X, ldx, k, C_dev, r, beta, Y, ldy, m, vec_ok);
    else if (tr <= 8)
        launch_pg<8, 32>(c, alpha, X, ldx, k, C_dev, r, beta, Y, ldy, m, vec_ok);
    else
        launch_pg<16, 16>(c, alpha, X, ldx, k, C_dev, r, beta, Y, ldy, m, vec_ok);
    RAILS_HIP_CHECK(hipGetLastError());
    return RAILS_OK;
}

int rails_panel_gemm2_dev(rails_ctx *c, double alpha, const double *X1, int ldx1, int a1, const double *X2, int ldx2, int a2, const double *C_dev,
                          int r, double *Y, int ldy, int64_t m)
{
    if (r <= 0 || m <= 0) return RAILS_OK;
    const int a = a1 + a2;
    const int vec1 = ((((uintptr_t)X1) & 15) == 0 && (ldx1 % 2) == 0) ? 1 : 0;
    const int vec2 = ((((uintptr_t)X2) & 15) == 0 && (ldx2 % 2) == 0 && (a1 % 2) == 0) ? 1 : 0;
    const unsigned grid = (unsigned)((m + 63) / 64);
    if (r <= 16)
        RAILS_LAUNCH((k_panel_gemm2<1, 32>), dim3(grid), dim3(256), 0, c->stream, alpha, X1, ldx1, a1, X2, ldx2, a, C_dev, r, 1.0, Y, ldy, m, vec1, vec2);
    else
        RAILS_LAUNCH((k_panel_gemm2<2, 32>), dim3(grid), dim3(256), 0, c->stream, alpha, X1, ldx1, a1, X2, ldx2, a, C_dev, r, 1.0, Y, ldy, m, vec1, vec2);
    RAILS_HIP_CHECK(hipGetLastError());
    return RAILS_OK;
}

namespace {
struct RocblasApi {
    void *handle = nullptr;
    int (*create)(void **) = nullptr;
    int (*destroy)(void *) = nullptr;
    int (*set_stream)(void *, hipStream_t) = nullptr;
    int (*dgemm)(void *, int, int, int, int, int, const double *, const double *, int, const double *, int, const double *, double *, int) = nullptr;
    bool tried = false, ok = false;
};
RocblasApi g_rocblas;
std::mutex g_rocblas_mutex;

bool load_rocblas()
{
    std::lock_guard<std::mutex> lock(g_rocblas_mutex);
    if (g_rocblas.tried) return g_rocblas.ok;
    g_rocblas.tried = true;
    const char *e = getenv("RAILS_WIDE_GEMM");
    if (!e || strcmp(e, "rocblas")) return false;
    const char *names[] = {getenv("RAILS_ROCBLAS_LIB"), "librocblas.so", "/opt/rocm/lib/librocblas.so", "librocblas.so.5", "librocblas.so.4"};
    for (const char *n : names) {
        if (!n || !*n) continue;
        if ((g_rocblas.handle = dlopen(n, RTLD_NOW | RTLD_LOCAL))) break;
    }
    if (!g_rocblas.handle) return false;
    g_rocblas.create = (int (*)(void **))dlsym(g_rocblas.handle, "rocblas_create_handle");
    g_rocblas.destroy = (int (*)(void *))dlsym(g_rocblas.handle, "rocblas_destroy_handle");
    g_rocblas.set_stream = (int (*)(void *, hipStream_t))dlsym(g_rocblas.handle, "rocblas_set_stream");
    g_rocblas.dgemm = (decltype(g_rocblas.dgemm))dlsym(g_rocblas.handle, "rocblas_dgemm");
    g_rocblas.ok = g_rocblas.create && g_rocblas.destroy && g_rocblas.set_stream && g_rocblas.dgemm;
    return g_rocblas.ok;
}
constexpr int ROCBLAS_OP_N = 111, ROCBLAS_OP_T = 112;
}

namespace {
// ... 127 lines not shown
```

### rails_amd/csrc/rails_internal.h

```cpp
#ifndef RAILS_INTERNAL_H
#define RAILS_INTERNAL_H

#include <hip/hip_runtime.h>

#include <cstdarg>
#include <cstdint>
#include <cstdio>
#include <cstring>
#include <ctime>
#include <string>
#include <vector>

#include "rails_hip.h"

void rails_set_error(const char *fmt, ...);

#define RAILS_HIP_CHECK(expr)                                                                      \
    do {                                                                                           \
        hipError_t e__ = (expr);                                                                   \
        if (e__ != hipSuccess) {                                                                   \
            rails_set_error("%s:%d: %s failed: %s", __FILE__, __LINE__, #expr, hipGetErrorString(e__)); \
            return RAILS_EHIP;                                                                     \
        }                                                                                          \
    } while (0)

#define RAILS_REQUIRE(cond, ...)                                                                   \
    do {                                                                                           \
        if (!(cond)) {                                                                             \
            rails_set_error(__VA_ARGS__);                                                          \
            return RAILS_EINVAL;                                                                   \
        }                                                                                          \
    } while (0)

#define RAILS_TRY(expr)                                                                            \
    do {                                                                                           \
        int rc__ = (expr);                                                                         \
        if (rc__ != RAILS_OK) return rc__;                                                         \
    } while (0)

static inline int rails_pad_ld(int capacity) { return ((capacity < 1 ? 1 : capacity) + 15) / 16 * 16; }

struct rails_ctx {
    int device = 0;
    hipStream_t stream = nullptr;
    bool own_stream = false;
    hipStream_t stream2 = nullptr;
    hipEvent_t ev_fork = nullptr, ev_join = nullptr;
    int num_cu = 256;
    uint64_t seed = 1;
    uint64_t next_stream = 0;
    int rank = 0, nranks = 1;
    int64_t row0 = 0, m_global = -1;
    rails_allreduce_fn allreduce = nullptr;
    void *allreduce_user = nullptr;
    void *rccl = nullptr;
    bool own_rccl = false;
    int rccl_nranks = 0, rccl_rank = 0;
    double *ws = nullptr;
    size_t ws_bytes = 0;
    std::vector<std::pair<size_t, double *>> free_panels;
    size_t free_panel_bytes = 0;
    double *small = nullptr;
    size_t small_bytes = 0;
    double *pinned = nullptr;
    size_t pinned_bytes = 0;
    hipEvent_t ev0 = nullptr, ev1 = nullptr;
    hipEvent_t ev_h2d = nullptr;
    bool h2d_pending = false;
    double *defer_dev = nullptr, *defer_pin = nullptr;
    size_t defer_slot = 0;
    int defer_nslots = 0;
    bool meter = false;
    std::vector<hipEvent_t> meter_events;
    int meter_open = 0;
    long meter_missed = 0;
    double gpu_busy_ms = 0.0;
    void *lz = nullptr;
    long n_orth_block = 0, n_orth_columnwise = 0, n_spmm_tiled = 0, n_spmm_planes = 0, n_spmm_overlapped = 0, n_spmm_sweep = 0, n_spmm_rowgather = 0, n_spmm_callback = 0, n_dev_alloc = 0, n_allreduce = 0, n_lanczos = 0, n_lanczos_start = 0, n_orth_repair = 0, n_update_gram_fused = 0, n_rowquad = 0;
    long n_orth_range = 0, n_orth_range_passes = 0, n_orth_range_syncs = 0;
    int last_update_gram_nbw = 0, last_gram_cols_ti = 0, last_gemm_wide_tr = 0;
};

constexpr int RAILS_METER_PAIRS = 512;
inline bool rails_meter_before(rails_ctx *c)
{
    if (!c->meter) return false;
    if (c->meter_open >= RAILS_METER_PAIRS) {
        c->meter_missed++;
        return false;
    }
    hipEventRecord(c->meter_events[2 * c->meter_open], c->stream);
    return true;
}
inline void rails_meter_after(rails_ctx *c) { hipEventRecord(c->meter_events[2 * c->meter_open++ + 1], c->stream); }
inline hipError_t rails_stream_sync(rails_ctx *c)
{
    const hipError_t e = hipStreamSynchronize(c->stream);
    for (int i = 0; i < c->meter_open; ++i) {
        float ms = 0.0f;
        if (e == hipSuccess && hipEventElapsedTime(&ms, c->meter_events[2 * i], c->meter_events[2 * i + 1]) == hipSuccess) c->gpu_busy_ms += ms;
    }
    c->meter_open = 0;
    return e;
}
#define RAILS_LAUNCH(...)                                                                                                                  \
    do {                                                                                                                                   \
        const bool rails_metered = rails_meter_before(c);                                                                                  \
        hipLaunchKernelGGL(__VA_ARGS__);                                                                                                   \
        if (rails_metered) rails_meter_after(c);                                                                                           \
    } while (0)

struct rails_panel {
    rails_ctx *ctx = nullptr;
    double *d = nullptr;
    int64_t m = 0;
    int cap = 0;
    int ld = 0;
};

struct rails_planes_plan;
struct rails_sweep_cache;
struct rails_tile_cache;

struct rails_csr {
    rails_ctx *ctx = nullptr;
    rails_sweep_cache *sweep = nullptr;
    rails_planes_plan *planes = nullptr;
    rails_tile_cache *tiled = nullptr;
    int64_t m = 0, ncols_ext = 0, nnz = 0;
    bool rect = false;
    int64_t *rowptr = nullptr;
    int32_t *col = nullptr;
    double *val = nullptr;
    int max_row_nnz = 0;
    int64_t window_rows = 0;
    rails_csr *AT = nullptr;
    std::vector<int64_t> h_rowptr;
    std::vector<int32_t> h_col;
    std::vector<double> h_val;
    int64_t n_send = 0, n_ghost = 0;
    int64_t int_lo = 0, int_hi = 0;
    int64_t window_rows_int = 0;
    int64_t *send_rows = nullptr;
    double *send_buf = nullptr;
    double *ext = nullptr;
    size_t send_cap = 0, ext_cap = 0;
    rails_halo_fn halo = nullptr;
    void *halo_user = nullptr;
    std::vector<int64_t> send_counts, recv_counts;
    int variant = 0;
    int is_grid = -1;
    const char *last_kernel = "";
    rails_apply_fn apply_cb = nullptr;
    void *apply_user = nullptr;
    rails_lu *lu = nullptr;
    rails_sprhs *sprhs = nullptr;
};

constexpr int RAILS_SPRHS_SHORT = 32;
constexpr int RAILS_SPRHS_CHUNK = 512;
struct rails_sprhs {
    rails_ctx *ctx = nullptr;
    int64_t m = 0, nnz = 0;
    int p = 0;
    rails_csr *B = nullptr;
    rails_csr *Bt = nullptr;
    double gram_norm2 = 0.0;
    int64_t n_items = 0, n_long = 0;
    int64_t *item_beg = nullptr;
    int32_t *item_len = nullptr;
    int32_t *long_row = nullptr;
    int64_t *long_item0 = nullptr;
    double *item_partial = nullptr;
};

struct rails_slow_guard {
    rails_ctx *c;
    const char *what;
    long long a, b;
    double t0 = 0.0;
    static double limit_ms()
    {
        static const double v = getenv("RAILS_TRACE_SLOW_MS") ? atof(getenv("RAILS_TRACE_SLOW_MS")) : 0.0;
        return v;
    }
    static double now()
    {
        timespec ts;
        clock_gettime(CLOCK_MONOTONIC, &ts);
        return ts.tv_sec * 1e3 + ts.tv_nsec * 1e-6;
    }
    rails_slow_guard(rails_ctx *ctx, const char *w, long long a_ = 0, long long b_ = 0) : c(ctx), what(w), a(a_), b(b_)
    {
        if (limit_ms() > 0.0 && c) {
            hipStreamSynchronize(c->stream);
            t0 = now();
        }
    }
    ~rails_slow_guard()
    {
        if (limit_ms() > 0.0 && c) {
            hipStreamSynchronize(c->stream);
            const double dt = now() - t0;
            if (dt > limit_ms()) fprintf(stderr, "[rails slow] %s(%lld, %lld): %.2f ms\n", what, a, b, dt);
        }
    }
};

inline int spmm_env(const char *name, int def)
{
    const char *e = getenv(name);
    return e ? atoi(e) : def;
}

int rails_ws_reserve(rails_ctx *ctx, size_t bytes);
void rails_library_gemm_release(rails_ctx *ctx);
int rails_small_reserve(rails_ctx *ctx, size_t bytes);
int rails_pinned_reserve(rails_ctx *ctx, size_t bytes);
int rails_pinned_begin_write(rails_ctx *ctx, size_t bytes);
int rails_pinned_end_write(rails_ctx *ctx);
int rails_allreduce_dev(rails_ctx *ctx, double *dev, size_t n);
int rails_ctx_second_stream(rails_ctx *ctx);

int rails_rccl_allreduce(rails_ctx *c, double *dev, size_t n);
int rails_rccl_halo(rails_ctx *c, const rails_csr *A, const double *send_buf, double *recv_buf, int ncols);
void rails_rccl_release(rails_ctx *c);

int rails_spmm_sweep(rails_ctx *c, rails_csr *A, const double *X, int ldx, const double *Xg, int ldg, double *Y, int ldy, int nc, bool aligned,
                     bool force, bool *done);
int rails_sweep_prepare(rails_ctx *c, rails_csr *A, int nc, bool *fits);
void rails_sweep_release(rails_csr *A);
int rails_spmm_sweep_interior(rails_ctx *c, rails_csr *A, const double *X, int ldx, double *Y, int ldy, int nc, bool aligned, hipStream_t st, bool *done);
int rails_sweep_prepare_interior(rails_ctx *c, rails_csr *A, int nc, bool *fits);
int rails_spmm_planes(rails_ctx *c, rails_csr *A, const double *X, int ldx, double *Y, int ldy, int nc, bool aligned, bool build, bool *done);
void rails_planes_release(rails_csr *A);
int rails_spmm_planes_interior(rails_ctx *c, rails_csr *A, const double *X, int ldx, double *Y, int ldy, int nc, bool aligned, hipStream_t st, bool *done);
bool planes_last_interior(const rails_csr *A);
int rails_spmm_tiled(rails_ctx *c, rails_csr *A, const double *X, int ldx, const double *Xg, int ldg, double *Y, int ldy, int nc, bool vec2,
                     int x_room, bool *done);
void rails_tiled_release(rails_csr *A);
int rails_gram_dev(rails_ctx *ctx, const double *X, int ldx, const double *Y, int ldy, int64_t m, int a, int b,
                   double *C_dev);
int rails_panel_gemm_dev(rails_ctx *ctx, double alpha, const double *X, int ldx, int k, const double *C_dev,
                         int r, double beta, double *Y, int ldy, int64_t m);
int rails_colnorms2_dev(rails_ctx *ctx, const double *X, int ldx, int64_t m, int nc, double *out_dev);
int rails_gram2_dev(rails_ctx *ctx, const double *X1, int ldx1, int a1, const double *X2, int ldx2, int a2, const double *Y, int ldy, int64_t m,
                    int b, double *C_dev);
int rails_panel_gemm2_dev(rails_ctx *ctx, double alpha, const double *X1, int ldx1, int a1, const double *X2, int ldx2, int a2,
                          const double *C_dev, int r, double *Y, int ldy, int64_t m);

#endif
```

### rails_amd/csrc/solver_capi.cpp

```cpp
#include <cmath>
#include <cstdio>
#include <cstring>
#include <map>
#include <string>
#include <vector>

#include <exception>
#include <new>

#include "rails/HipSolverOps.hpp"
#include "rails/SubspaceSolverOps.hpp"
#include "rails_solution.h"
#include "rails_solver.h"

void rails_set_error(const char *fmt, ...);

namespace
{

class ParameterList
{
    std::map<std::string, double> params_;

public:
// ... 246 lines not shown
    s->start = rails::HipMultiVectorWrapper();
    return RAILS_OK;
}

extern "C" int rails_solver_set_start_space(rails_solver *s, const rails_panel *P, int c0, int k)
{
    if (!s || !P) {
        rails_set_error("rails_solver_set_start_space: null argument");
        return RAILS_EINVAL;
    }
    if (k < 1 || c0 < 0 || c0 + k > rails_panel_capacity(P)) {
        rails_set_error("rails_solver_set_start_space: columns [%d,%d) of a panel of capacity %d", c0, c0 + k, rails_panel_capacity(P));
        return RAILS_EINVAL;
    }
    if (rails_panel_rows(P) != s->m_local) {
        rails_set_error("rails_solver_set_start_space: the panel has %lld rows, the solver %lld local rows", (long long)rails_panel_rows(P),
                        (long long)s->m_local);
        return RAILS_EINVAL;
    }
    rails::HipMultiVectorWrapper W(s->m_local, k, s->ctx);
    W.set_global_rows(s->m_global);
    const int rc = rails_panel_copy(s->ctx, P, c0, k, W.panel(), 0);
    if (rc != RAILS_OK) return rc;
    s->start = W;
    s->have_start = true;
    s->have_V0 = false;
    return RAILS_OK;
}

extern "C" int rails_solver_start_rank(rails_solver *s) { return s ? s->start_rank : -1; }

static int solve_in_coordinates(rails_solver *s)
{
    const int p = s->B.N();
    const int restart = s->params.get("Restart size", -1);
    const int expand = s->params.get("Expand size", 3);
    rails::HipSolver::Projection proj;
    const bool pair = rails::HipSolver::parse_projection(s->params.get("Projection method", 1.0), proj) && proj.pair;
    const int kmax = std::max(restart > 0 ? restart : 100, 1) + (pair ? 2 : 1) * expand + 100 + (s->have_start ? s->start.N() : 0);
    auto basis = std::make_shared<rails::SubspaceBasis>(s->ctx, s->m_local, s->m_global, 2 * kmax + p + 128);
    if (restart > 0 || s->params.get("Restart iterations", 20) > 0) basis->preallocate_compress_panel();
    rails::SubspaceMultiVector Bc = rails::SubspaceMultiVector::Absorb(basis, s->B);
    rails::SubspaceOperator Ac(s->A, basis);
    rails::SubspaceOperator Mc(s->mass ? s->M : s->A, basis);
    rails::SubspaceSolver solver(Ac, Bc, Mc);
    if (s->has_inv) solver.set_inverse(rails::SubspaceOperator(s->Ainv, basis));
    if (s->null_q > 0) solver.set_nullspace(rails::SubspaceMultiVector::Absorb(basis, s->N));
    ParameterList params = s->params;
    if (s->have_start) params.set("Restart from solution", 1.0);
    int prc = solver.set_parameters(params);
    if (prc != 0) return prc + 100;
    solver.set_verbose(s->verbose);
    solver.set_max_trips(s->max_trips);
    solver.use_mass_matrix(s->mass);
    solver.use_mass_orthogonalisation(s->ortho_m);
    if (s->trip_fn) solver.set_trip_callback([s](int trip) { s->trip_fn(s->trip_user, trip); });
    solver.set_failure_check([basis]() { return basis->failed; });
    rails::SubspaceMultiVector Vc(basis, 1);
    if (s->have_V0) {
        Vc = rails::SubspaceMultiVector::Absorb(basis, s->V);
        Vc.set_orthogonalized(Vc.N());
    }
    if (s->have_start) {
        if (s->start.orthogonalize_range(nullptr, 0.0) < 1) {
            if (rails::sticky_error() == RAILS_OK) std::cerr << "rails::Solver: no column of the start space is left after orthonormalisation" << std::endl;
            return -2;
        }
        const bool overlap = basis->overlap;
        basis->overlap = false;
        Vc = rails::SubspaceMultiVector::Absorb(basis, s->start);
        basis->overlap = overlap;
        Vc.set_orthogonalized(Vc.N());
    }
    int rc = solver.solve(Vc, s->T);
    s->null_rank = solver.nullspace_rank();
    s->start_rank = solver.start_rank();
    if (rc == -2) return rc;
    s->V = Vc.materialise();
    s->V.set_orthogonalized(s->V.N());
    s->sub_trips = solver.trips();
    s->sub_hist = solver.residual_history();
    s->sub_profile = solver.profile();
    char buf[1536];
    snprintf(buf, sizeof(buf), "{\"dim\": %d, \"absorb\": %ld, \"absorb_columns\": %ld, \"one_by_one\": %ld, \"dropped\": %ld, \"compress\": %ld, \"materialise\": %ld, \"prefetched_random\": %ld, \"second_rounds\": %ld, \"delicate_blocks\": %ld, \"reprojected_blocks\": %ld, \"overlapped_blocks\": %ld, \"scratch_blocks\": %ld, \"replaced_columns\": %ld, \"verified\": %d, \"verify_representation\": %.3e, \"verify_orthonormality\": %.3e, \"seconds\": {\"materialise\": %.4f, \"absorb\": %.4f, \"compress_qr\": %.4f, \"compress_rotate\": %.4f, "
             "\"compress_coefficients\": %.4f}}",
             basis->dim, basis->n_absorb, basis->n_absorb_cols, basis->n_single, basis->n_dropped, basis->n_compress, basis->n_materialise, basis->n_prefetched, basis->n_second_round, basis->n_delicate, basis->n_reprojected, basis->n_overlapped, basis->n_scratch_blocks, basis->n_replaced, basis->verify ? 1 : 0, basis->verify_repr, basis->verify_orth,
             basis->t_materialise, basis->t_absorb, basis->t_qr, basis->t_rotate, basis->t_recoef);
    s->sub_stats = buf;
    if (basis->failed) {
        rails_set_error("coordinate-space back end: a device operation failed (%s)", rails_last_error());
        return -1000;
    }
    return rc;
}

extern "C" int rails_solver_solve(rails_solver *s, int *code, int *k)
{
    if (!s) return RAILS_EINVAL;
    const bool restart_from_solution = s->params.get("Restart from solution", 0.0) != 0.0;
    s->last_was_subspace = s->subspace && !s->sprhs && (s->have_V0 || s->have_start || !restart_from_solution) && !(s->have_start && s->null_q > 0);
    {
        rails::HipSolver::Projection proj;
        const double method = s->params.get("Projection method", 1.0);
        if (!rails::HipSolver::parse_projection(method, proj)) {
            rails_set_error("rails_solver_solve: 'Projection method' %g is none of 1, 1.1, 1.2, 1.3, 2.1, 2.2, 2.3", method);
            return RAILS_EINVAL;
        }
        if (proj.uses_inverse() && !s->has_inv) {
            rails_set_error("rails_solver_solve: 'Projection method' %g needs an inverse (rails_solver_set_inverse)", method);
            return RAILS_EINVAL;
        }
    }
    rails::clear_sticky_error();
    int rc;
    try {
        if (s->last_was_subspace) {
            rc = solve_in_coordinates(s);
            if (rc == -1000) return RAILS_EHIP;
        } else if (s->have_start) {
            const bool was_warm = s->solver->settings().warm_start;
            struct Restore {
                rails_solver *s;
                bool warm;
                ~Restore()
                {
                    ParameterList back = s->params;
                    back.set("Restart from solution", warm ? 1.0 : 0.0);
                    s->solver->set_raw_start_space(false);
                    s->solver->set_parameters(back);
                }
            } restore{s, was_warm};
            ParameterList params = s->params;
            params.set("Restart from solution", 1.0);
            const int prc = s->solver->set_parameters(params);
            if (prc != 0) {
                rails_set_error("rails_solver_solve: the parameters are not valid (code %d, rails_solver_apply_parameters)", prc);
                return RAILS_EINVAL;
            }
            s->solver->set_raw_start_space(true);
            rails::HipMultiVectorWrapper Vs = s->start;
            rc = s->solver->solve(Vs, s->T);
            s->null_rank = s->solver->nullspace_rank();
            s->start_rank = s->solver->start_rank();
            if (rc != -2) s->V = Vs;
        } else {
            rc = s->solver->solve(s->V, s->T);
            s->null_rank = s->solver->nullspace_rank();
            s->start_rank = s->solver->start_rank();
        }
    } catch (std::bad_alloc const &) {
        rails_set_error("rails_solver_solve: out of host memory");
        return RAILS_ENOMEM;
    } catch (std::exception const &e) {
        rails_set_error("rails_solver_solve: %s", e.what());
        return RAILS_EINVAL;
    }
    s->have_start = false;
    s->start = rails::HipMultiVectorWrapper();
    s->have_V0 = false;
    if (code) *code = rc;
    if (k) *k = s->V.N();
    if (rails_ctx_sync(s->ctx) != RAILS_OK) return RAILS_EHIP;
    if (rails::sticky_error() != RAILS_OK) {
        const int err = rails::sticky_error();
        rails_set_error("rails_solver_solve: a device operation failed during the solve (code %d, first failure; see stderr): %s", err, rails_last_error());
        return err;
    }
    return RAILS_OK;
}
// ... 157 lines not shown
```

### rails_amd/csrc/spmm.hip

```cpp
#include "rails_internal.h"
#include "row_choice.h"
#include "tile_plan.h"

#include <algorithm>

namespace {

typedef double double2_t __attribute__((ext_vector_type(2)));
typedef double2_t double2_a8_t __attribute__((aligned(8)));

template <int VEC>
struct Acc;
template <>
struct Acc<1> {
    double v;
    __device__ __forceinline__ void zero() { v = 0.0; }
    __device__ __forceinline__ void fma(double a, const double *x) { v = __builtin_fma(a, *x, v); }
    __device__ __forceinline__ void store(double *y) { *y = v; }
};
template <>
struct Acc<2> {
    double2_t v;
    __device__ __forceinline__ void zero() { v = (double2_t){0.0, 0.0}; }
    __device__ __forceinline__ void fma(double a, const double *x)
    {
        double2_t t = *reinterpret_cast<const double2_a8_t *>(x);
        v.x = __builtin_fma(a, t.x, v.x);
        v.y = __builtin_fma(a, t.y, v.y);
    }
    __device__ __forceinline__ void store(double *y) { *reinterpret_cast<double2_a8_t *>(y) = v; }
};

template <int LPR, int VEC, int RPG>
__global__ __launch_bounds__(256) void k_spmm_rowgather(int64_t m, const int64_t *__restrict__ rowptr,
                                                        const int32_t *__restrict__ col, const double *__restrict__ val,
                                                        const double *__restrict__ X, int ldx, const double *__restrict__ Xg,
                                                        int ldg, double *__restrict__ Y, int ldy, int nc, int64_t blocks_per_xcd, int64_t mc)
{
    constexpr int GROUPS = 256 / LPR;
    constexpr int U = 8;
    const int g = threadIdx.x / LPR;
    const int l = threadIdx.x % LPR;
    int64_t lb = blockIdx.x;
    if (blocks_per_xcd > 0) lb = (int64_t)(blockIdx.x & 7) * blocks_per_xcd + (blockIdx.x >> 3);
    int64_t row_base = (lb * GROUPS + g) * RPG;
    if (LPR == 64) row_base = (lb * GROUPS + __builtin_amdgcn_readfirstlane(g)) * RPG;

    for (int rr = 0; rr < RPG; ++rr) {
        const int64_t row = row_base + rr;
        if (row >= m) break;
        const int64_t p0 = rowptr[row], p1 = rowptr[row + 1];
        for (int cb = l * VEC; cb < nc; cb += LPR * VEC) {
            const bool full = (cb + VEC <= nc);
            Acc<VEC> acc;
            acc.zero();
            double tail = 0.0;
            for (int64_t p = p0; p < p1; p += U) {
                int32_t c[U];
                double a[U];
                const int cnt = (int)((p1 - p) < U ? (p1 - p) : U);
#pragma unroll
                for (int u = 0; u < U; ++u) {
                    const bool ok = u < cnt;
                    c[u] = col[ok ? p + u : p0];
                    a[u] = ok ? val[p + u] : 0.0;
                }
                const double *src[U];
#pragma unroll
                for (int u = 0; u < U; ++u)
                    src[u] = (c[u] < mc) ? (X + (int64_t)c[u] * ldx + cb) : (Xg + ((int64_t)c[u] - mc) * ldg + cb);
                if (full) {
#pragma unroll
                    for (int u = 0; u < U; ++u) acc.fma(a[u], src[u]);
                } else {
#pragma unroll
                    for (int u = 0; u < U; ++u) tail = __builtin_fma(a[u], *src[u], tail);
                }
            }
            double *dst = Y + row * ldy + cb;
            if (full)
                acc.store(dst);
            else
                *dst = tail;
        }
    }
}

__global__ void k_pack_rows(const int64_t *__restrict__ rows, int64_t n, const double *__restrict__ X, int ldx, int nc,
                            double *__restrict__ out)
{
    int64_t total = n * nc;
    for (int64_t idx = (int64_t)blockIdx.x * blockDim.x + threadIdx.x; idx < total; idx += (int64_t)gridDim.x * blockDim.x) {
        int64_t i = idx / nc;
        int cidx = (int)(idx - i * nc);
        out[idx] = X[rows[i] * ldx + cidx];
    }
}

struct RowSpan {
    int64_t r0 = 0, nrows = -1;
    hipStream_t st = nullptr;
};
#define RAILS_LAUNCH_ON(st__, kern__, grid__, block__, lds__, ...)                           \
    do {                                                                                     \
        if ((st__) == c->stream)                                                             \
            RAILS_LAUNCH(kern__, grid__, block__, lds__, c->stream, __VA_ARGS__);            \
        else                                                                                 \
            hipLaunchKernelGGL(kern__, grid__, block__, lds__, (st__), __VA_ARGS__);        \
    } while (0)

template <int LPR, int VEC>
int launch_rg(rails_ctx *c, const rails_csr *A, const double *X, int ldx, const double *Xg, int ldg, double *Y, int ldy, int nc, const RowSpan &sp)
{
    const int64_t m_rows = sp.nrows < 0 ? A->m : sp.nrows;
    hipStream_t st = sp.st ? sp.st : c->stream;
    constexpr int GROUPS = 256 / LPR;
    constexpr int RPG = (LPR >= 32) ? 4 : 2;
    int64_t rows_per_block = (int64_t)GROUPS * RPG;
    int64_t grid = (m_rows + rows_per_block - 1) / rows_per_block;
    static const int xcd_aware = spmm_env("RAILS_SPMM_XCD", 1);
    int64_t bpx = 0;
    if (xcd_aware && grid >= 64) {
        bpx = (grid + 7) / 8;
        grid = bpx * 8;
    }
    RAILS_REQUIRE(grid <= 0x7fffffffLL, "rails_spmm: grid too large");
    RAILS_LAUNCH_ON(st, (k_spmm_rowgather<LPR, VEC, RPG>), dim3((unsigned)grid), dim3(256), 0, m_rows, A->rowptr + sp.r0, A->col,
                    A->val, X, ldx, Xg, ldg, Y + sp.r0 * ldy, ldy, nc, bpx, A->m);
    return RAILS_OK;
}


template <int LPR, int RPG>
__global__ __launch_bounds__(256) void k_spmm_rowgather_cc(int64_t m, const int64_t *__restrict__ rowptr, const int32_t *__restrict__ col,
                                                           const double *__restrict__ val, const double *__restrict__ X, int ldx,
                                                           const double *__restrict__ Xg, int ldg, double *__restrict__ Y, int ldy, int nc,
                                                           int64_t blocks_per_xcd, int lds_cap, int y_vec, int64_t mc)
{
    constexpr int GROUPS = 256 / LPR;
    constexpr int ROWS = GROUPS * RPG;
    constexpr int CC = 2 * LPR;
    constexpr int U = 8;
    extern __shared__ double smem[];
    double *s_val = smem;
    int32_t *s_col = reinterpret_cast<int32_t *>(smem + lds_cap);
    const int g = threadIdx.x / LPR;
    const int l = threadIdx.x % LPR;
    const int64_t s = blockIdx.x >> 3;
    const int chunk = (int)(s / blocks_per_xcd);
    const int64_t lb = (int64_t)(blockIdx.x & 7) * blocks_per_xcd + (s - (int64_t)chunk * blocks_per_xcd);
    const int64_t r0 = lb * ROWS;
    if (r0 >= m) return;
    const int64_t r1 = (r0 + ROWS < m) ? r0 + ROWS : m;
    const int64_t nz0 = rowptr[r0], nz1 = rowptr[r1];
    const bool staged = (nz1 - nz0) <= lds_cap;
    if (staged) {
        for (int64_t q = nz0 + threadIdx.x; q < nz1; q += 256) {
            s_col[q - nz0] = col[q];
            s_val[q - nz0] = val[q];
        }
        __syncthreads();
    }
    const int cb = chunk * CC + l * 2;
    if (cb >= nc) return;
    const bool full = (cb + 2 <= nc);
    for (int rr = 0; rr < RPG; ++rr) {
        const int64_t row = r0 + (int64_t)rr * GROUPS + g;
        if (row >= m) break;
        const int64_t p0 = rowptr[row], p1 = rowptr[row + 1];
        double2_t acc = (double2_t){0.0, 0.0};
        for (int64_t p = p0; p < p1; p += U) {
            int32_t c[U];
            double a[U];
            const int cnt = (int)((p1 - p) < U ? (p1 - p) : U);
#pragma unroll
            for (int u = 0; u < U; ++u) {
                const bool ok = u < cnt;
                const int64_t q = ok ? p + u : p0;
                c[u] = staged ? s_col[q - nz0] : col[q];
                const double av = staged ? s_val[q - nz0] : val[q];
                a[u] = ok ? av : 0.0;
            }
            if (full) {
                double2_t x[U];
#pragma unroll
                for (int u = 0; u < U; ++u) {
                    const double *src = (c[u] < mc) ? (X + (int64_t)c[u] * ldx + cb) : (Xg + ((int64_t)c[u] - mc) * ldg + cb);
                    x[u] = *reinterpret_cast<const double2_t *>(src);
                }
#pragma unroll
                for (int u = 0; u < U; ++u) {
                    acc.x = __builtin_fma(a[u], x[u].x, acc.x);
                    acc.y = __builtin_fma(a[u], x[u].y, acc.y);
                }
            } else {
#pragma unroll
                for (int u = 0; u < U; ++u) {
                    const double *src = (c[u] < mc) ? (X + (int64_t)c[u] * ldx + cb) : (Xg + ((int64_t)c[u] - mc) * ldg + cb);
                    acc.x = __builtin_fma(a[u], *src, acc.x);
                }
            }
        }
        double *dst = Y + row * ldy + cb;
        if (full && y_vec)
            *reinterpret_cast<double2_t *>(dst) = acc;
        else if (full) {
            dst[0] = acc.x;
            dst[1] = acc.y;
        } else
            *dst = acc.x;
    }
}

template <int RPG, bool GHOST, int LPR = 8>
__global__ __launch_bounds__(256) void k_spmm_narrow(int64_t m, const int64_t *__restrict__ rowptr, const int32_t *__restrict__ col,
                                                     const double *__restrict__ val, const double *__restrict__ X, uint32_t ldx8,
                                                     const double *__restrict__ Xg, uint32_t ldg8, double *__restrict__ Y, int ldy, int nc,
                                                     int64_t blocks_per_xcd, int y_vec, int64_t mc)
{
    constexpr int GROUPS = 256 / LPR, ROWS = GROUPS * RPG, CAP = 2048;
    __shared__ double s_val[CAP];
    __shared__ int32_t s_col[CAP];
    const int g = threadIdx.x / LPR;
    const int l = threadIdx.x % LPR;
    const int64_t lb = (int64_t)(blockIdx.x & 7) * blocks_per_xcd + (blockIdx.x >> 3);
    const int64_t r0 = lb * ROWS;
    if (r0 >= m) return;
    const int64_t r1 = (r0 + ROWS < m) ? r0 + ROWS : m;
    const int64_t nz0 = rowptr[r0], nz1 = rowptr[r1];
    const bool staged = (nz1 - nz0) <= CAP;
    if (staged) {
        for (int q = threadIdx.x; q < (int)(nz1 - nz0); q += 256) {
            s_col[q] = col[nz0 + q];
            s_val[q] = val[nz0 + q];
        }
        __syncthreads();
    }
    const int cb = l * 2;
    if (cb >= nc) return;
    const bool full = (cb + 2 <= nc);
    const uint32_t cb8 = (uint32_t)cb * 8u, m32 = (uint32_t)mc;
    const char *Xb = reinterpret_cast<const char *>(X), *Gb = reinterpret_cast<const char *>(Xg);
    auto xrow = [&](uint32_t c) -> const char * {
        if (!GHOST) return Xb + (__umul24(c, ldx8) + cb8);
        const bool local = c < m32;
        return (local ? Xb : Gb) + ((local ? __umul24(c, ldx8) : __umul24(c - m32, ldg8)) + cb8);
    };
    for (int rr = 0; rr < RPG; ++rr) {
        const int64_t row = r0 + (int64_t)rr * GROUPS + g;
        if (row >= m) break;
        double2_t acc = (double2_t){0.0, 0.0};
        if (staged && full) {
            int i = (int)(rowptr[row] - nz0);
            const int i1 = (int)(rowptr[row + 1] - nz0);
            for (; i + 8 <= i1; i += 8) {
                double2_t x[8];
                double a[8];
#pragma unroll
                for (int u = 0; u < 8; ++u) {
                    x[u] = *reinterpret_cast<const double2_a8_t *>(xrow((uint32_t)s_col[i + u]));
                    a[u] = s_val[i + u];
                }
#pragma unroll
                for (int u = 0; u < 8; ++u) {
                    acc.x = __builtin_fma(a[u], x[u].x, acc.x);
                    acc.y = __builtin_fma(a[u], x[u].y, acc.y);
                }
            }
            for (; i < i1; i += 4) {
                double2_t x[4];
                double a[4];
#pragma unroll
                for (int u = 0; u < 4; ++u) {
                    const int q = i + u < i1 ? i + u : i1 - 1;
                    x[u] = *reinterpret_cast<const double2_a8_t *>(xrow((uint32_t)s_col[q]));
                    a[u] = i + u < i1 ? s_val[q] : 0.0;
                }
#pragma unroll
                for (int u = 0; u < 4; ++u) {
                    acc.x = __builtin_fma(a[u], x[u].x, acc.x);
                    acc.y = __builtin_fma(a[u], x[u].y, acc.y);
                }
            }
        } else {
            for (int64_t p = rowptr[row]; p < rowptr[row + 1]; ++p) {
                const double a = val[p];
                const double *src = reinterpret_cast<const double *>(xrow((uint32_t)col[p]));
                acc.x = __builtin_fma(a, src[0], acc.x);
                if (full) acc.y = __builtin_fma(a, src[1], acc.y);
            }
        }
        double *dst = Y + row * ldy + cb;
        if (full && y_vec)
            *reinterpret_cast<double2_t *>(dst) = acc;
        else if (full) {
            dst[0] = acc.x;
            dst[1] = acc.y;
        } else
            *dst = acc.x;
    }
}

template <int LPR>
int launch_rg_cc(rails_ctx *c, const rails_csr *A, const RowChoice &ch, const double *X, int ldx, const double *Xg, int ldg, double *Y, int ldy, int nc,
                 const RowSpan &sp)
{
    const int64_t m_rows = sp.nrows < 0 ? A->m : sp.nrows;
    hipStream_t st = sp.st ? sp.st : c->stream;
    const int64_t *rowptr = A->rowptr + sp.r0;
    Y += sp.r0 * ldy;
    constexpr int GROUPS = 256 / LPR;
    constexpr int RPG = (LPR >= 32) ? 8 : (LPR >= 16 ? 4 : 2);
    constexpr int ROWS = GROUPS * RPG;
    constexpr int CC = 2 * LPR;
    constexpr int NLPR = LPR == 16 ? 16 : 8;
    const int nchunks = (nc + CC - 1) / CC;
    const int64_t blocks = (m_rows + ROWS - 1) / ROWS;
    const int64_t bpx = (blocks + 7) / 8;
    const int64_t grid = bpx * 8 * nchunks;
    RAILS_REQUIRE(grid <= 0x7fffffffLL, "rails_spmm: grid too large");
    const int y_vec = ch.y_vec ? 1 : 0;
    if (ch.kind == RowChoice::NARROW && !ch.ghost)
        RAILS_LAUNCH_ON(st, (k_spmm_narrow<RPG, false, NLPR>), dim3((unsigned)grid), dim3(256), 0, m_rows, rowptr, A->col, A->val, X, (uint32_t)ldx * 8u, X, 0u, Y, ldy, nc,
                        bpx, y_vec, A->m);
    else if (ch.kind == RowChoice::NARROW)
        RAILS_LAUNCH_ON(st, (k_spmm_narrow<RPG, true, NLPR>), dim3((unsigned)grid), dim3(256), 0, m_rows, rowptr, A->col, A->val, X, (uint32_t)ldx * 8u, Xg,
                        (uint32_t)ldg * 8u, Y, ldy, nc, bpx, y_vec, A->m);
    else {
        const int lds_cap = 2048;
        RAILS_LAUNCH_ON(st, (k_spmm_rowgather_cc<LPR, RPG>), dim3((unsigned)grid), dim3(256), (size_t)lds_cap * 12, m_rows, rowptr, A->col, A->val, X, ldx, Xg, ldg, Y,
                        ldy, nc, bpx, lds_cap, y_vec, A->m);
    }
    return RAILS_OK;
}

template <int VEC>
int dispatch_rg(rails_ctx *c, const rails_csr *A, int lpr, const double *X, int ldx, const double *Xg, int ldg, double *Y, int ldy, int nc, const RowSpan &sp)
{
    switch (lpr) {
    case 64: return launch_rg<64, VEC>(c, A, X, ldx, Xg, ldg, Y, ldy, nc, sp);
    case 32: return launch_rg<32, VEC>(c, A, X, ldx, Xg, ldg, Y, ldy, nc, sp);
    case 16: return launch_rg<16, VEC>(c, A, X, ldx, Xg, ldg, Y, ldy, nc, sp);
    case 8: return launch_rg<8, VEC>(c, A, X, ldx, Xg, ldg, Y, ldy, nc, sp);
    case 4: return launch_rg<4, VEC>(c, A, X, ldx, Xg, ldg, Y, ldy, nc, sp);
    case 2: return launch_rg<2, VEC>(c, A, X, ldx, Xg, ldg, Y, ldy, nc, sp);
    default: return launch_rg<1, VEC>(c, A, X, ldx, Xg, ldg, Y, ldy, nc, sp);
    }
}

RowFacts row_facts(const rails_csr *A, int nc, bool x_vec2, bool y_vec2, bool vec2, const double *X, int ldx, const double *Xg, int ldg, int span_ghost)
{
    static const int narrow_cc = spmm_env("RAILS_SPMM_NARROW_CC", 1), narrow_fast = spmm_env("RAILS_SPMM_NARROW_FAST", 1),
                     chunk_env = spmm_env("RAILS_SPMM_CHUNK", 0);
    RowFacts f;
    f.variant = A->variant; f.max_row_nnz = A->max_row_nnz; f.m = A->m; f.ncols_ext = A->ncols_ext; f.n_ghost = A->n_ghost; f.rect = A->rect;
    f.nc = nc; f.x_vec2 = x_vec2; f.y_vec2 = y_vec2; f.vec2 = vec2; f.ldx = ldx; f.ldg = ldg;
    f.xg_is_tail = Xg == X + (int64_t)A->m * ldx;
    f.span_ghost = span_ghost;
    f.narrow_cc = narrow_cc != 0; f.narrow_fast = narrow_fast != 0; f.chunk_env = chunk_env;
    return f;
}

const char *const ROW_KERNEL[3] = {"k_spmm_rowgather", "k_spmm_rowgather_cc", "k_spmm_narrow"};

int launch_rows(rails_ctx *c, const rails_csr *A, const RowChoice &ch, const double *X, int ldx, const double *Xg, int ldg, double *Y, int ldy, int nc,
                const RowSpan &sp = RowSpan())
{
    if (ch.kind == RowChoice::PLAIN)
        return ch.vec == 2 ? dispatch_rg<2>(c, A, ch.lpr, X, ldx, Xg, ldg, Y, ldy, nc, sp) : dispatch_rg<1>(c, A, ch.lpr, X, ldx, Xg, ldg, Y, ldy, nc, sp);
    if (ch.lpr == 8) return launch_rg_cc<8>(c, A, ch, X, ldx, Xg, ldg, Y, ldy, nc, sp);
    if (ch.lpr == 16) return launch_rg_cc<16>(c, A, ch, X, ldx, Xg, ldg, Y, ldy, nc, sp);
    return launch_rg_cc<32>(c, A, ch, X, ldx, Xg, ldg, Y, ldy, nc, sp);
}

int spmm_span(rails_ctx *c, const rails_csr *A, const RowChoice &ch, const double *X, int ldx, const double *Xg, int ldg, double *Y, int ldy, int nc,
              const RowSpan &sp)
{
    return sp.nrows <= 0 ? RAILS_OK : launch_rows(c, A, ch, X, ldx, Xg, ldg, Y, ldy, nc, sp);
}

int64_t mean_row_window(const int64_t *rowptr, const int32_t *col, int64_t r0, int64_t r1)
{
    const int64_t stride = std::max<int64_t>(1, (r1 - r0) / 4096);
    int64_t sum = 0, cnt = 0;
    for (int64_t i = r0; i < r1; i += stride) {
        if (rowptr[i + 1] == rowptr[i]) continue;
        int32_t lo = col[rowptr[i]], hi = lo;
        for (int64_t q = rowptr[i]; q < rowptr[i + 1]; ++q) {
            lo = std::min(lo, col[q]);
            hi = std::max(hi, col[q]);
        }
        sum += (int64_t)hi - lo + 1;
        cnt++;
    }
    return cnt ? sum / cnt : 0;
}

int build_transpose(rails_csr *A)
{
    if (A->AT) return RAILS_OK;
    RAILS_REQUIRE(A->n_ghost == 0 && A->ncols_ext == A->m, "rails_spmm: transposed apply is single-GPU only");
    const int64_t m = A->m, nnz = A->nnz;
    std::vector<int64_t> rp(m + 1, 0);
    for (int64_t p = 0; p < nnz; ++p) rp[A->h_col[p] + 1]++;
    for (int64_t i = 0; i < m; ++i) rp[i + 1] += rp[i];
    std::vector<int32_t> ci(nnz);
    std::vector<double> va(nnz);
    std::vector<int64_t> next(rp.begin(), rp.end() - 1);
    for (int64_t i = 0; i < m; ++i)
        for (int64_t p = A->h_rowptr[i]; p < A->h_rowptr[i + 1]; ++p) {
// ... 135 lines not shown
    RAILS_REQUIRE(!A->sprhs, "rails_csr_set_halo: a sparse right-hand side is single GPU only");
    RAILS_REQUIRE(n_send >= 0 && n_ghost >= 0 && A->m + n_ghost == A->ncols_ext,
                  "rails_csr_set_halo: m_local %lld + ghosts %lld != extended columns %lld", (long long)A->m, (long long)n_ghost,
                  (long long)A->ncols_ext);
    RAILS_REQUIRE((n_send == 0 && n_ghost == 0) || fn || A->ctx->rccl,
                  "rails_csr_set_halo: neither a halo hook nor an RCCL communicator on the context (rails_ctx_init_rccl)");
    for (int64_t i = 0; i < n_send; ++i)
        RAILS_REQUIRE(send_rows[i] >= 0 && send_rows[i] < A->m, "rails_csr_set_halo: send row %lld out of range", (long long)send_rows[i]);
    rails_ctx *c = A->ctx;
    if (A->send_rows) {
        RAILS_HIP_CHECK(rails_stream_sync(c));
        RAILS_HIP_CHECK(hipFree(A->send_rows));
        A->send_rows = nullptr;
    }
    A->n_send = n_send;
    A->n_ghost = n_ghost;
    A->halo = fn;
    A->halo_user = user;
    A->int_lo = 0;
    A->int_hi = A->m;
    if (n_ghost > 0) {
        const int64_t m = A->m, mid = m / 2;
        for (int64_t r = 0; r < m; ++r) {
            bool boundary = false;
            for (int64_t p2 = A->h_rowptr[r]; p2 < A->h_rowptr[r + 1] && !boundary; ++p2) boundary = A->h_col[p2] >= m;
            if (!boundary) continue;
            if (r < mid)
                A->int_lo = r + 1;
            else {
                A->int_hi = r;
                break;
            }
        }
        A->window_rows_int = mean_row_window(A->h_rowptr.data(), A->h_col.data(), A->int_lo, A->int_hi);
    }
    if (n_send) {
        RAILS_HIP_CHECK(hipMalloc((void **)&A->send_rows, (size_t)n_send * sizeof(int64_t)));
        RAILS_HIP_CHECK(hipMemcpy(A->send_rows, send_rows, (size_t)n_send * sizeof(int64_t), hipMemcpyHostToDevice));
    }
    return RAILS_OK;
}

static bool rails_csr_is_grid(rails_csr *A)
{
    if (A->is_grid < 0) {
        int64_t gx = 0, gy = 0, gz = 0;
        A->is_grid = (spmm_env("RAILS_SPMM_TILE_BOX", 1) && rails_detect_grid(A->m, A->h_rowptr.data(), A->h_col.data(), &gx, &gy, &gz)) ? 1 : 0;
    }
    return A->is_grid == 1;
}

static bool sweep_worthwhile(rails_csr *A, int nc)
{
    if (!(nc >= 64 && nc <= 256 && nc % 16 == 0 && 32 % (nc / 16) == 0 && A->n_ghost == 0 && A->window_rows > 0)) return false;
    const int64_t phases = 32 / (nc / 16), part_rows = A->m / 8;
    if (!(A->window_rows + 256 <= (phases - 1) * 2816 && A->m >= 8 * phases * 2816 &&
          (double)phases * (double)(part_rows + A->window_rows + 1024) <= 8.0 * (double)part_rows))
        return false;
    return !rails_csr_is_grid(A);
}

extern "C" int rails_csr_prepare(rails_ctx *c, rails_csr *A, int trans, int nc, int *kernel_ready)
{
    RAILS_REQUIRE(c && A && nc >= 1, "rails_csr_prepare: bad argument");
    if (kernel_ready) *kernel_ready = 0;
    if (A->apply_cb || A->lu || A->sprhs) return RAILS_OK;
    if (trans) {
        RAILS_TRY(build_transpose(A));
        A->AT->variant = A->variant;
        return rails_csr_prepare(c, A->AT, 0, nc, kernel_ready);
    }
    if (A->variant == 7 || (A->variant == 0 && sweep_worthwhile(A, nc))) {
        bool fits = false;
        RAILS_TRY(rails_sweep_prepare(c, A, nc, &fits));
        if (kernel_ready) *kernel_ready = fits ? 1 : 0;
    } else if (A->variant == 0 && A->n_ghost > 0 && !rails_csr_is_grid(A)) {
        bool fits = false;
        RAILS_TRY(rails_sweep_prepare_interior(c, A, nc, &fits));
        if (kernel_ready) *kernel_ready = fits ? 1 : 0;
    }
    return RAILS_OK;
}

extern "C" int rails_spmm(rails_ctx *c, rails_csr *A, int trans, const rails_panel *X, int xc0, int nc, rails_panel *Y, int yc0)
{
    if (c) hipSetDevice(c->device);
    rails_slow_guard slow__(c, "rails_spmm", nc, A ? A->m : 0);
    RAILS_REQUIRE(c && A && X && Y, "rails_spmm: null argument");
    if (A->sprhs) return rails_sprhs_apply(c, A->sprhs, trans, X, xc0, nc, Y, yc0);
    RAILS_REQUIRE(xc0 >= 0 && nc >= 0 && xc0 + nc <= X->cap, "rails_spmm: X columns [%d,%d) outside capacity %d", xc0, xc0 + nc, X->cap);
    RAILS_REQUIRE(yc0 >= 0 && yc0 + nc <= Y->cap, "rails_spmm: Y columns [%d,%d) outside capacity %d", yc0, yc0 + nc, Y->cap);
    RAILS_REQUIRE(X->m == (A->rect ? A->ncols_ext : A->m) && Y->m == A->m, "rails_spmm: operator is %lld x %lld, X has %lld rows, Y %lld", (long long)A->m,
                  (long long)(A->rect ? A->ncols_ext : A->m), (long long)X->m, (long long)Y->m);
    RAILS_REQUIRE(!(A->rect && trans), "rails_spmm: a rectangular operator has no transposed apply (create the transposed matrix)");
    if (X->d == Y->d) RAILS_REQUIRE(xc0 + nc <= yc0 || yc0 + nc <= xc0, "rails_spmm: X and Y windows alias");
    if (nc == 0 || A->m == 0) return RAILS_OK;
    if (A->lu) return rails_lu_solve(c, A->lu, trans, X, xc0, nc, Y, yc0);
    if (A->apply_cb) {
        int rc = A->apply_cb(A->apply_user, trans ? 1 : 0, X, xc0, nc, Y, yc0);
        if (rc != 0) {
            rails_set_error("rails_spmm: the operator callback failed with code %d", rc);
            return RAILS_ECOMM;
        }
        c->n_spmm_callback++;
        return RAILS_OK;
    }
    if (trans) {
        RAILS_TRY(build_transpose(A));
        A->AT->variant = A->variant;
        int rc = rails_spmm(c, A->AT, 0, X, xc0, nc, Y, yc0);
        A->last_kernel = A->AT->last_kernel;
        return rc;
    }
    const double *Xp = X->d + xc0;
    double *Yp = Y->d + yc0;
    const double *Xg = A->rect ? Xp + (size_t)std::min(A->m, A->ncols_ext) * X->ld : Xp;
    int ldg = X->ld;
    if (A->n_ghost > 0 || A->n_send > 0) {
        size_t sbytes = (size_t)(A->n_send ? A->n_send : 1) * nc * sizeof(double);
        size_t gbytes = (size_t)(A->n_ghost ? A->n_ghost : 1) * nc * sizeof(double);
        if (sbytes > A->send_cap) {
            RAILS_HIP_CHECK(rails_stream_sync(c));
            if (A->send_buf) RAILS_HIP_CHECK(hipFree(A->send_buf));
            A->send_buf = nullptr;
            RAILS_HIP_CHECK(hipMalloc((void **)&A->send_buf, sbytes));
            A->send_cap = sbytes;
        }
        if (gbytes > A->ext_cap) {
            RAILS_HIP_CHECK(rails_stream_sync(c));
            if (A->ext) RAILS_HIP_CHECK(hipFree(A->ext));
            A->ext = nullptr;
            RAILS_HIP_CHECK(hipMalloc((void **)&A->ext, gbytes));
            A->ext_cap = gbytes;
        }
        const int overlap_env = spmm_env("RAILS_SPMM_HALO_OVERLAP", 1);
        const bool x_vec2o = (xc0 & 1) == 0 && (X->ld % 2 == 0) && (nc % 2 == 0), y_vec2o = (yc0 & 1) == 0 && (Y->ld % 2 == 0);
        bool interior_sweep = false;
        const bool overlap = overlap_env && A->n_ghost > 0 && !A->rect && (A->variant == 0 || A->variant == 1 || A->variant == 3) &&
                             A->int_hi - A->int_lo >= A->m / 2 && A->int_hi - A->int_lo >= 1024;
        if (overlap) {
            RAILS_TRY(rails_ctx_second_stream(c));
            RAILS_HIP_CHECK(hipEventRecord(c->ev_fork, c->stream));
            RAILS_HIP_CHECK(hipStreamWaitEvent(c->stream2, c->ev_fork, 0));
            const RowSpan in = {A->int_lo, A->int_hi - A->int_lo, c->stream2};
            bool planes_done = false, sweep_done = false;
            RAILS_TRY(rails_spmm_planes_interior(c, A, Xp, X->ld, Yp, Y->ld, nc, x_vec2o, c->stream2, &planes_done));
            if (!planes_done) RAILS_TRY(rails_spmm_sweep_interior(c, A, Xp, X->ld, Yp, Y->ld, nc, x_vec2o && y_vec2o, c->stream2, &sweep_done));
            interior_sweep = sweep_done;
            if (!planes_done && !sweep_done)
                RAILS_TRY(spmm_span(c, A, rails_row_choice(row_facts(A, nc, x_vec2o, y_vec2o, false, Xp, X->ld, Xp, X->ld, 0)), Xp, X->ld, Xp, X->ld, Yp, Y->ld, nc, in));
            RAILS_HIP_CHECK(hipEventRecord(c->ev_join, c->stream2));
            c->n_spmm_overlapped++;
        }
        if (A->n_send) {
            int64_t total = A->n_send * nc;
            int grid = (int)std::min<int64_t>((total + 255) / 256, (int64_t)c->num_cu * 8);
            RAILS_LAUNCH(k_pack_rows, dim3(grid), dim3(256), 0, c->stream, A->send_rows, A->n_send, Xp, X->ld, nc, A->send_buf);
        }
        if (A->halo) {
            int rc = A->halo(A->halo_user, A->send_buf, A->ext, nc, (void *)c->stream);
            if (rc != 0) {
                rails_set_error("rails_spmm: halo hook failed with code %d", rc);
                return RAILS_ECOMM;
            }
        } else {
            RAILS_REQUIRE(c->rccl, "rails_spmm: ghost rows but neither a halo hook nor an RCCL communicator");
            RAILS_TRY(rails_rccl_halo(c, A, A->send_buf, A->ext, nc));
        }
        if (overlap) {
            const RowSpan lo = {0, A->int_lo, nullptr}, hi = {A->int_hi, A->m - A->int_hi, nullptr};
            const RowChoice ch = rails_row_choice(row_facts(A, nc, x_vec2o, y_vec2o, false, Xp, X->ld, A->ext, nc, 1));
            RAILS_TRY(spmm_span(c, A, ch, Xp, X->ld, A->ext, nc, Yp, Y->ld, nc, lo));
            RAILS_TRY(spmm_span(c, A, ch, Xp, X->ld, A->ext, nc, Yp, Y->ld, nc, hi));
            RAILS_HIP_CHECK(hipStreamWaitEvent(c->stream, c->ev_join, 0));
            static const char *const overlapped[3][3] = {
                {"k_spmm_rowgather (halo overlapped)", "k_spmm_rowgather_cc (halo overlapped)", "k_spmm_narrow (halo overlapped)"},
                {"k_spmm_rowgather + k_spmm_planes (halo overlapped)", "k_spmm_rowgather + k_spmm_planes (halo overlapped)", "k_spmm_narrow + k_spmm_planes (halo overlapped)"},
                {"k_spmm_rowgather + k_spmm_sweep (halo overlapped)", "k_spmm_rowgather + k_spmm_sweep (halo overlapped)", "k_spmm_rowgather + k_spmm_sweep (halo overlapped)"}};
            const RowChoice::Kind boundary = (lo.nrows > 0 || hi.nrows > 0) ? ch.kind : RowChoice::PLAIN;
            A->last_kernel = overlapped[interior_sweep ? 2 : planes_last_interior(A) ? 1 : 0][boundary];
            c->n_spmm_rowgather++;
            RAILS_HIP_CHECK(hipGetLastError());
            return RAILS_OK;
        }
        Xg = A->ext;
        ldg = nc;
    }
    bool done = false;
    const bool vec2 = ((xc0 | yc0) & 1) == 0 && (ldg % 2 == 0);
    const bool sweep_auto = A->variant == 0 && sweep_worthwhile(A, nc);
    if (A->variant == 7 || sweep_auto) {
        const bool al = ((xc0 | yc0) & 1) == 0 && X->ld % 2 == 0 && Y->ld % 2 == 0 && ldg % 2 == 0;
        RAILS_TRY(rails_spmm_sweep(c, A, Xp, X->ld, Xg, ldg, Yp, Y->ld, nc, al, A->variant == 7, &done));
        if (done) return RAILS_OK;
    }
    if (A->variant == 9 || (A->variant == 0 && nc >= 2 && A->n_ghost == 0 && !A->rect && spmm_env("RAILS_SPMM_PLANES", 1) && rails_csr_is_grid(A))) {
        const bool al = (xc0 & 1) == 0 && X->ld % 2 == 0;
        RAILS_TRY(rails_spmm_planes(c, A, Xp, X->ld, Yp, Y->ld, nc, al, true, &done));
        if (done) {
            c->n_spmm_planes++;
            return RAILS_OK;
        }
        RAILS_REQUIRE(A->variant != 9, "rails_spmm: plane-sweep kernel requested but not applicable to this operator/shape");
    }
    static const int narrow_first = spmm_env("RAILS_SPMM_NARROW_CC", 1) && spmm_env("RAILS_SPMM_NARROW_FAST", 1);
    const bool leave_to_narrow = A->variant == 0 && narrow_first && nc > 8 && nc <= 16 && A->max_row_nnz <= 64 && A->ncols_ext < (1 << 24);
    if ((A->variant == 0 && !leave_to_narrow) || A->variant == 2 || A->variant == 6)
        RAILS_TRY(rails_spmm_tiled(c, A, Xp, X->ld, Xg, ldg, Yp, Y->ld, nc, vec2, X->ld - xc0, &done));
    if (done) c->n_spmm_tiled++;
    if (!done) {
        RAILS_REQUIRE(A->variant != 2 && A->variant != 6, "rails_spmm: LDS-staged kernel requested but not applicable to this operator/shape");
        const bool x_vec2 = (xc0 & 1) == 0 && (X->ld % 2 == 0) && (ldg % 2 == 0);
        const bool y_vec2 = (yc0 & 1) == 0 && (Y->ld % 2 == 0);
        const RowChoice ch = rails_row_choice(row_facts(A, nc, x_vec2, y_vec2, vec2, Xp, X->ld, Xg, ldg, -1));
        RAILS_TRY(launch_rows(c, A, ch, Xp, X->ld, Xg, ldg, Yp, Y->ld, nc));
        A->last_kernel = ROW_KERNEL[ch.kind];
        c->n_spmm_rowgather++;
    }
    RAILS_HIP_CHECK(hipGetLastError());
    return RAILS_OK;
}
```

### rails_amd/include/rails/HipWrappers.hpp

```cpp
#ifndef RAILS_HIPWRAPPERS_HPP
#define RAILS_HIPWRAPPERS_HPP

#include <algorithm>
#include <cmath>
#include <cstring>
#include <functional>
#include <iostream>
#include <memory>
#include <vector>

#include "rails/HostDenseMatrix.hpp"
#include "rails_hip.h"
#include "rails_solution.h"

namespace rails
{

inline rails_ctx *&default_context()
{
    static rails_ctx *ctx = nullptr;
    return ctx;
}
inline void set_default_context(rails_ctx *ctx) { default_context() = ctx; }

// ... 471 lines not shown
    HipOperatorWrapper(rails_ctx *ctx, rails_csr *A, int64_t m_global = -1)
        : ctx_(ctx ? ctx : default_context()), transpose_(false), m_global_(m_global < 0 && A ? rails_csr_rows(A) : m_global)
    {
        if (A) h_ = std::make_shared<CsrHandle>(ctx_, A, false);
        if (A && rails_csr_sprhs(A)) n_cols_ = rails_csr_cols(A);
    }

    HipOperatorWrapper(rails_ctx *ctx, rails_sprhs *S) : ctx_(ctx ? ctx : default_context()), transpose_(false), m_global_(S ? rails_sprhs_rows(S) : -1)
    {
        rails_csr *A = nullptr;
        if (S && hip_ok(rails_csr_create_sprhs(ctx_, S, &A), "rails_csr_create_sprhs")) {
            h_ = std::make_shared<CsrHandle>(ctx_, A);
            n_cols_ = rails_sprhs_cols(S);
        }
    }

    typedef std::function<bool(bool, HipMultiVectorWrapper const &, HipMultiVectorWrapper &)> ApplyFunction;
    static HipOperatorWrapper FromCallback(rails_ctx *ctx, int64_t m_local, ApplyFunction apply, int64_t m_global = -1)
    {
        HipOperatorWrapper out;
        out.ctx_ = ctx ? ctx : default_context();
        out.m_global_ = m_global < 0 ? m_local : m_global;
        auto h = std::make_shared<CsrHandle>(out.ctx_, nullptr);
        h->apply = std::move(apply);
        if (hip_ok(rails_csr_create_callback(out.ctx_, m_local, &HipOperatorWrapper::trampoline, h.get(), &h->A), "rails_csr_create_callback")) out.h_ = h;
        return out;
    }

    virtual ~HipOperatorWrapper() {}

    rails_csr *csr() const { return h_ ? h_->A : nullptr; }
    bool transposed() const { return transpose_; }
    rails_ctx *context() const { return ctx_; }

    int M() const { return (int)m_global_; }
    int N() const { return (int)(n_cols_ < 0 ? m_global_ : n_cols_); }
    rails_sprhs *sprhs() const { return h_ && h_->A ? rails_csr_sprhs(h_->A) : nullptr; }

    HipOperatorWrapper transpose() const
    {
        HipOperatorWrapper out(*this);
        out.transpose_ = !transpose_;
        return out;
    }

    bool prepare(int nc) const
    {
        int ready = 0;
        if (!h_ || !hip_ok(rails_csr_prepare(ctx_, h_->A, transpose_ ? 1 : 0, nc, &ready), "rails_csr_prepare")) return false;
        return ready != 0;
    }

private:
    static int trampoline(void *user, int trans, const rails_panel *X, int xc0, int nc, rails_panel *Y, int yc0)
    {
        CsrHandle *h = static_cast<CsrHandle *>(user);
        HipMultiVectorWrapper x = HipMultiVectorWrapper::Window(h->ctx, const_cast<rails_panel *>(X), xc0, nc);
        HipMultiVectorWrapper y = HipMultiVectorWrapper::Window(h->ctx, Y, yc0, nc);
        return h->apply(trans != 0, x, y) ? 0 : RAILS_EINVAL;
    }

public:
    HipMultiVectorWrapper operator*(HipMultiVectorWrapper const &X) const
    {
        if (n_cols_ >= 0) {
            HipMultiVectorWrapper out(transpose_ ? n_cols_ : m_global_, X.n_, ctx_);
            if (h_) apply_into(X, out, 0);
            return out;
        }
        HipMultiVectorWrapper out(X, X.n_);
        out.m_global_ = X.m_global_;
        if (!h_) {
            std::cerr << "rails_amd: operator* on an empty HipOperatorWrapper" << std::endl;
            return out;
        }
        apply_into(X, out, 0);
        return out;
    }

    bool apply_into(HipMultiVectorWrapper const &X, HipMultiVectorWrapper &Y, int ycol) const
    {
        if (X.n_ <= 0) return true;
        return hip_ok(rails_spmm(ctx_, h_->A, transpose_ ? 1 : 0, X.panel_->p, X.c0_, X.n_, Y.panel_->p, Y.c0_ + ycol), "rails_spmm");
    }

    double norm_rectangular(int64_t m, int64_t nc) const
    {
        const int steps = (int)std::min<int64_t>(nc, 200);
        HipMultiVectorWrapper v(nc, 1, ctx_), vp(nc, 1, ctx_), w(nc, 1, ctx_), y(m, 1, ctx_);
        v.random();
        const double nv = v.norm();
        if (nv == 0.0) return 0.0;
        v /= nv;
        std::vector<double> d, e;
        double beta = 0.0;
        for (int j = 0; j < steps; ++j) {
            if (rails_spmm(ctx_, h_->A, transpose_ ? 1 : 0, v.panel_->p, 0, 1, y.panel_->p, 0) != RAILS_OK) return 0.0;
            if (rails_spmm(ctx_, h_->A, transpose_ ? 0 : 1, y.panel_->p, 0, 1, w.panel_->p, 0) != RAILS_OK) return 0.0;
            const double ny = y.norm(), alpha = ny * ny;
            d.push_back(alpha);
            rails_panel_axpy(ctx_, -alpha, v.panel_->p, 0, 1, w.panel_->p, 0);
            if (j > 0) rails_panel_axpy(ctx_, -beta, vp.panel_->p, 0, 1, w.panel_->p, 0);
            beta = w.norm();
            if (j + 1 == steps || !(beta > 1e-14 * d[0])) break;
            e.push_back(beta);
            w /= beta;
            std::swap(vp.panel_, v.panel_);
            std::swap(v.panel_, w.panel_);
        }
        const int n = (int)d.size();
        e.resize(std::max(n, 1), 0.0);
        std::vector<double> work(1);
        int info = 0;
        rails_dsteqr('N', n, d.data(), e.data(), nullptr, 1, work.data(), &info);
        if (info != 0) return 0.0;
        const double lam = *std::max_element(d.begin(), d.end());
        return lam > 0.0 ? std::sqrt(lam) : 0.0;
    }

    double norm() const
    {
        if (!h_) return 0.0;
        int64_t m = rails_csr_rows(h_->A), nc = rails_csr_cols(h_->A);
        if (transpose_) std::swap(m, nc);
        if (m == 0 || nc == 0) return 0.0;
        if (n_cols_ >= 0) return norm_rectangular(m, nc);
        HipMultiVectorWrapper x(nc, 1, ctx_), y(m, 1, ctx_);
        x.random();
        double lam = 0.0;
        for (int it = 0; it < 200; ++it) {
            double nx = x.norm();
            if (nx == 0.0) return 0.0;
            x /= nx;
            rails_spmm(ctx_, h_->A, transpose_ ? 1 : 0, x.panel_->p, 0, 1, y.panel_->p, 0);
            rails_spmm(ctx_, h_->A, transpose_ ? 0 : 1, y.panel_->p, 0, 1, x.panel_->p, 0);
            double l2 = y.norm();
            if (std::abs(l2 - lam) <= 1e-14 * l2) {
                lam = l2;
                break;
            }
            lam = l2;
        }
        return lam;
    }
};

}

#endif
```

### rails_amd/include/rails/SubspaceWrappers.hpp

```cpp
#ifndef RAILS_SUBSPACEWRAPPERS_HPP
#define RAILS_SUBSPACEWRAPPERS_HPP

#include <algorithm>
#include <chrono>
#include <cmath>
#include <cstdlib>
#include <cstring>
#include <iostream>
#include <memory>
#include <vector>

#include "rails/BlockOrthHost.hpp"
#include "rails/HipWrappers.hpp"

namespace rails
{

class SubspaceBasis
{
public:
    rails_ctx *ctx;
    int64_t m_local, m_global;
    HipMultiVectorWrapper P, P2;
    int dim = 0;
    int row_cap;
    std::vector<std::weak_ptr<CoefStore>> live;
    long n_absorb = 0, n_absorb_cols = 0, n_single = 0, n_compress = 0, n_materialise = 0, n_dropped = 0, n_prefetched = 0, n_second_round = 0, n_delicate = 0, n_reprojected = 0;
    bool failed = false;
    long n_replaced = 0;
    double t_materialise = 0, t_absorb = 0, t_qr = 0, t_rotate = 0, t_recoef = 0;
    bool profile_sync = getenv("RAILS_SUBSPACE_PROFILE") != nullptr;
    bool trace = getenv("RAILS_SUBSPACE_TRACE") != nullptr;
    double reorth_survival = getenv("RAILS_SUBSPACE_REORTH") ? atof(getenv("RAILS_SUBSPACE_REORTH")) : block_orth::reorth_survival;
    double slow_ms = getenv("RAILS_SUBSPACE_SLOW_MS") ? atof(getenv("RAILS_SUBSPACE_SLOW_MS")) : 0.0;
    struct Tick {
        SubspaceBasis *b;
        double *acc;
        const char *what;
        std::chrono::steady_clock::time_point t0;
        Tick(SubspaceBasis *bb, double *a, const char *w = "") : b(bb), acc(a), what(w)
        {
            if (b->profile_sync) rails_ctx_sync(b->ctx);
            t0 = std::chrono::steady_clock::now();
        }
        ~Tick()
        {
            if (b->profile_sync) rails_ctx_sync(b->ctx);
            const double dt = std::chrono::duration<double>(std::chrono::steady_clock::now() - t0).count();
            *acc += dt;
            if (b->slow_ms > 0.0 && dt * 1e3 > b->slow_ms)
                std::cerr << "[subspace] " << what << ": " << dt * 1e3 << " ms (dim " << b->dim << ", absorbs so far " << b->n_absorb << ")" << std::endl;
        }
    };
    std::shared_ptr<CoefStore> cached_random;
    bool cached_valid = false;
    bool prefetch_random = true;

    bool overlap = !(getenv("RAILS_SUBSPACE_OVERLAP") && atoi(getenv("RAILS_SUBSPACE_OVERLAP")) == 0);
    double overlap_min_survival = block_orth::overlap_min_survival;
    long n_overlapped = 0;
    struct Pending {
        bool active = false;
        int dim0 = 0, w = 0, w2 = 0;
        std::vector<double> Rfp;
        std::vector<double> g0diag;
    } pending;
    enum { SLOT_C2 = 0, SLOT_G = 1, SLOT_M1 = 2, SLOT_G2 = 3, SLOT_M2 = 4, N_SLOTS = 5 };
    bool block_scratch = !(getenv("RAILS_SUBSPACE_BLOCK_SCRATCH") && atoi(getenv("RAILS_SUBSPACE_BLOCK_SCRATCH")) == 0);
    long n_scratch_blocks = 0;
    std::shared_ptr<PanelHandle> S;
    rails_panel *scratch_panel(int w)
    {
        if (S && S->p && rails_panel_capacity(S->p) >= w) return S->p;
        const int ld = (w + 1) & ~1;
        S = std::make_shared<PanelHandle>(ctx, m_local, ld, ld);
        return S->p;
    }

    SubspaceBasis(rails_ctx *c, int64_t ml, int64_t mg, int rows) : ctx(c), m_local(ml), m_global(mg), P(ml, std::max(rows, 16), c), row_cap(std::max(rows, 16))
    {
        P.set_global_rows(mg);
        P.resize(0);
    }

    void preallocate_compress_panel()
    {
        const size_t cap = (size_t)P.capacity();
        hip_ok(rails_ctx_reserve_staging(ctx, cap * cap / 2 * sizeof(double)), "rails_ctx_reserve_staging");
        if (P2.N() >= 0 && P2.capacity() >= P.capacity()) return;
        P2 = HipMultiVectorWrapper(m_local, P.capacity(), ctx);
        P2.set_global_rows(m_global);
        const int kw = std::min(256, (int)P.capacity());
        if (kw >= 64 && rails_ctx_library_gemm_ready(ctx)) {
            std::vector<double> Z((size_t)kw * kw, 0.0);
            const int keep = P.N();
            P.resize(kw);
            P2.resize(kw);
            hip_ok(rails_panel_fill(ctx, P.panel(), keep, kw - keep, 0.0), "rails_panel_fill");
            hip_ok(rails_panel_gemm_wide(ctx, 1.0, P.panel(), 0, kw, Z.data(), kw, kw, 0.0, P2.panel(), 0), "rails_panel_gemm_wide");
            P.resize(keep);
        }
        P2.resize(0);
    }

    std::shared_ptr<CoefStore> new_store(int ncap, bool in_basis, int rows = 0)
    {
        auto s = std::make_shared<CoefStore>(in_basis ? row_cap : rows, ncap, in_basis);
        if (in_basis) live.push_back(s);
        return s;
    }

    void ensure_rows(int need)
    {
        if (need <= row_cap) return;
        int ncap = std::max(need + 64, row_cap + row_cap / 2);
        for (auto &w : live)
            if (auto s = w.lock()) {
                std::vector<double> nc((size_t)ncap * s->ncap, 0.0);
                for (int j = 0; j < s->ncap; ++j) memcpy(nc.data() + (size_t)j * ncap, s->col(j), sizeof(double) * dim);
                s->c.swap(nc);
                s->ld = ncap;
            }
        row_cap = ncap;
    }

    HipMultiVectorWrapper scratch;
    HipMultiVectorWrapper materialise(const double *C, int ldc, int n)
    {
        if (scratch.N() < 0 || scratch.capacity() < std::max(n, 1)) {
            scratch = HipMultiVectorWrapper(m_local, std::max(n, 16), ctx);
            scratch.set_global_rows(m_global);
        }
        if (!resolve_pending()) return scratch;
        scratch.resize(n);
        HipMultiVectorWrapper out;
        out = scratch;
        n_materialise++;
        Tick tick(this, &t_materialise, "materialise");
        if (n <= 0) return out;
        if (dim == 0) {
            out = 0.0;
            return out;
        }
        for (int j0 = 0; j0 < n; j0 += 128) {
            int nc = std::min(128, n - j0);
            if (!hip_ok(rails_panel_gemm(ctx, 1.0, P.panel(), 0, dim, C + (size_t)j0 * ldc, ldc, nc, 0.0, out.panel(), j0), "rails_panel_gemm")) failed = true;
        }
        return out;
    }

    int tail(int w)
    {
        if (dim + w > P.capacity()) {
            P.resize(dim);
            P.resize(dim + w + 64);
        }
        P.resize(dim);
        ensure_rows(dim + w);
        return dim;
    }

    template <class Fill, class Dest>
    void absorb_filled(int n, Fill &&fill, Dest &&dest)
    {
        for (int j0 = 0; j0 < n; j0 += 64) {
// ... 70 lines not shown
                ncols += s->ncap;
            }
        live.swap(still);
        if (dim == 0 || ncols == 0) return;
        std::vector<double> Call((size_t)dim * ncols);
        int c0 = 0;
        for (auto &s : stores)
            for (int j = 0; j < s->ncap; ++j)
                if (s->in_use(j, dim)) memcpy(Call.data() + (size_t)c0++ * dim, s->col(j), sizeof(double) * dim);
        ncols = c0;
        if (trace) {
            std::cerr << "compress: dim " << dim << ", " << stores.size() << " live stores, columns in use:";
            for (auto &st : stores) {
                int used = 0;
                for (int j = 0; j < st->ncap; ++j) used += st->in_use(j, dim) ? 1 : 0;
                std::cerr << " " << used << "/" << st->ncap;
            }
            std::cerr << " -> " << ncols << " columns" << std::endl;
        }
        if (ncols == 0) return;
        std::vector<double> Q((size_t)dim * std::min(dim, ncols));
        int rank = 0, info = 0;
        {
            Tick tick(this, &t_qr, "compress: pivoted QR");
            rails_range_basis(dim, ncols, Call.data(), dim, 1e-14, Q.data(), dim, &rank, &info);
        }
        if (info != 0 || rank <= 0 || rank >= dim - 8) return;
        if (P2.N() < 0 || P2.capacity() < rank + 64) {
            P2 = HipMultiVectorWrapper(m_local, rank + 128, ctx);
            P2.set_global_rows(m_global);
        }
        P2.resize(rank);
        {
            Tick rot(this, &t_rotate, "compress: rotation");
            if (!hip_ok(rails_panel_gemm_wide(ctx, 1.0, P.panel(), 0, dim, Q.data(), dim, rank, 0.0, P2.panel(), 0), "rails_panel_gemm_wide")) {
                failed = true;
                return;
            }
        }
        Tick tick(this, &t_recoef, "compress: coefficients");
        for (auto &s : stores) {
            int used = 0;
            for (int j = s->ncap - 1; j >= 0 && !used; --j)
                if (s->in_use(j, dim)) used = j + 1;
            if (used == 0) continue;
            std::vector<double> nc((size_t)rank * used);
            rails_dgemm('T', 'N', rank, used, dim, 1.0, Q.data(), dim, s->c.data(), s->ld, 0.0, nc.data(), rank);
            for (int j = 0; j < used; ++j) {
                memcpy(s->col(j), nc.data() + (size_t)j * rank, sizeof(double) * rank);
                std::fill(s->col(j) + rank, s->col(j) + dim, 0.0);
            }
        }
        std::swap(P, P2);
        dim = rank;
        n_compress++;
    }

    bool start_overlapped(int w, int w2, double *coef, std::vector<double> const &CG, std::vector<double> const &G0)
    {
        const int ld = row_cap, dw = dim + w;
        if (!block_orth::predict_block(CG.data(), dim, w, pending.Rfp)) return false;
        if (!hip_ok(rails_deferred_reserve(ctx, N_SLOTS, (int64_t)(P.capacity() + 64) * (w <= 32 ? 32 : 48)), "rails_deferred_reserve")) return false;
        rails_panel *pp = P.panel();
        rails_panel *bp = pp;
        int b0 = dim;
        if (block_scratch) {
            bp = scratch_panel(w);
            b0 = 0;
            if (!bp) return fail("no scratch panel for the overlapped block orthogonalisation");
        }
        bool ok = true;
        rails_panel *xp = bp;
        int x0 = b0;
        if (w2 > 0) {
            ok = ok && hip_ok(rails_update_gram_deferred_out(ctx, -1.0, pp, 0, dim, CG.data(), dw, w, pp, dim, bp, b0, w2, SLOT_C2), "rails_update_gram_deferred_out");
            ok = ok && hip_ok(rails_panel_gemm_deferred(ctx, -1.0, pp, 0, dim, SLOT_C2, dim, w2, 1.0, bp, b0), "rails_panel_gemm_deferred");
        } else {
            ok = ok && hip_ok(rails_panel_gemm(ctx, -1.0, pp, 0, dim, CG.data(), dw, w, 1.0, pp, dim), "rails_panel_gemm");
            xp = pp;
            x0 = dim;
        }
        ok = ok && hip_ok(rails_gram_deferred(ctx, xp, x0, w, xp, x0, w, SLOT_G), "rails_gram_deferred");
        ok = ok && hip_ok(rails_chol_inverse_deferred(ctx, SLOT_G, w, SLOT_M1), "rails_chol_inverse_deferred");
        ok = ok && hip_ok(rails_panel_gemm_deferred(ctx, 1.0, xp, x0, w, SLOT_M1, w, w, 0.0, bp, b0), "rails_panel_gemm_deferred");
        ok = ok && hip_ok(rails_gram_deferred(ctx, bp, b0, w, bp, b0, w, SLOT_G2), "rails_gram_deferred");
        ok = ok && hip_ok(rails_chol_inverse_deferred(ctx, SLOT_G2, w, SLOT_M2), "rails_chol_inverse_deferred");
        ok = ok && hip_ok(rails_panel_gemm_deferred(ctx, 1.0, bp, b0, w, SLOT_M2, w, w, 0.0, pp, dim), "rails_panel_gemm_deferred");
        if (!ok) return fail("the overlapped block orthogonalisation could not be queued");
        pending.active = true;
        pending.dim0 = dim;
        pending.w = w;
        pending.w2 = w2;
        pending.g0diag.resize(w);
        for (int b = 0; b < w; ++b) {
            pending.g0diag[b] = G0[b + (size_t)b * w];
            for (int a = 0; a <= b; ++a) coef[(dim + a) + (size_t)b * ld] = pending.Rfp[a + (size_t)b * w];
        }
        if (w2 > 0) n_second_round++;
        n_overlapped++;
        if (block_scratch) n_scratch_blocks++;
        static const long spoil = getenv("RAILS_SUBSPACE_TEST_SPOIL_PREDICTION") ? atol(getenv("RAILS_SUBSPACE_TEST_SPOIL_PREDICTION")) : 0;
        if (spoil > 0 && n_overlapped == spoil) {
            pending.Rfp[0] *= 1.01;
            coef[dim] = pending.Rfp[0];
        }
        dim += w;
        P.resize(dim);
        return true;
    }

    bool resolve_pending()
    {
        if (!pending.active) return !failed;
        pending.active = false;
        const int d0 = pending.dim0, w = pending.w, w2 = pending.w2;
        if (!hip_ok(rails_ctx_sync(ctx), "rails_ctx_sync")) return fail();
        std::vector<double> C2((size_t)d0 * w, 0.0), G((size_t)w * w), G2((size_t)w * w);
        if (w2 > 0 && !hip_ok(rails_deferred_fetch(ctx, SLOT_C2, (int64_t)d0 * w2, C2.data()), "rails_deferred_fetch")) return fail();
        if (!hip_ok(rails_deferred_fetch(ctx, SLOT_G, (int64_t)w * w, G.data()), "rails_deferred_fetch")) return fail();
        if (!hip_ok(rails_deferred_fetch(ctx, SLOT_G2, (int64_t)w * w, G2.data()), "rails_deferred_fetch")) return fail();
        block_orth::RebaseMaps maps;
        if (const char *why = block_orth::rebase_maps(C2.data(), d0, w2, G.data(), G2.data(), w, pending.Rfp, pending.g0diag, maps)) return fail(why);
        if (trace) std::cerr << "absorb (overlapped): dim " << d0 << " w " << w << ": prediction off by " << maps.off << std::endl;
        for (auto &wk : live)
            if (auto st = wk.lock())
                for (int j = 0; j < st->ncap; ++j)
                    if (st->in_use(j, d0 + w, d0)) block_orth::rebase_column(maps, st->col(j));
        if (verify && !failed) {
            OrthDefect o;
            if (!measure_orthonormality(dim, o)) return false;
            if (trace) std::cerr << "absorb (overlapped) verified: dim " << d0 << " -> " << dim << ": |P'P - I| = " << o.orth << std::endl;
            verify_orth = std::max(verify_orth, o.orth);
        }
        return !failed;
    }

private:
    bool fail(const char *what = nullptr)
    {
        if (what) std::cerr << "rails_amd: SubspaceBasis: " << what << std::endl;
        failed = true;
        return false;
    }

    struct OrthDefect { double orth = 0.0, against_old = 0.0; int i = -1, j = -1; };
    bool measure_orthonormality(int dim_before, OrthDefect &o)
    {
        std::vector<double> PP((size_t)dim * dim);
        if (!hip_ok(rails_gram(ctx, P.panel(), 0, dim, P.panel(), 0, dim, PP.data(), dim), "rails_gram")) return fail();
        for (int j = 0; j < dim; ++j)
            for (int i = 0; i < dim; ++i) {
                const double e = std::fabs(PP[i + (size_t)j * dim] - (i == j ? 1.0 : 0.0));
                if (e > o.orth) { o.orth = e; o.i = i; o.j = j; }
                if (j >= dim_before && i < dim_before) o.against_old = std::max(o.against_old, e);
            }
        return true;
    }

    static void add_scaled(double *coefcol, const double *Ccol, int nb, double scale) { for (int i = 0; i < nb; ++i) coefcol[i] += scale * Ccol[i]; }
    bool project_tail(int c, int n, int nb, std::vector<double> &C, int rows, double scale = 0.0, double *coef = nullptr)
    {
        C.resize((size_t)rows * n);
        if (!hip_ok(rails_gram(ctx, P.panel(), 0, rows, P.panel(), dim + c, n, C.data(), rows), "rails_gram")) return fail();
        if (!hip_ok(rails_panel_gemm(ctx, -1.0, P.panel(), 0, nb, C.data(), rows, n, 1.0, P.panel(), dim + c), "rails_panel_gemm")) return fail();
        for (int j = 0; coef && j < n; ++j) add_scaled(coef + (size_t)j * row_cap, C.data() + (size_t)j * rows, nb, scale);
        return true;
    }

// ... 479 lines not shown
            for (int l = 0; l < r; ++l) v[l] /= nr;
        }
        orthogonalized_ = n_;
    }

public:
    HipMultiVectorWrapper materialise() const { return basis_->materialise(cptr(), ld(), n_); }
    void to_host(double *data, int64_t ldd) const
    {
        if (!in_basis()) {
            for (int j = 0; j < n_; ++j) memcpy(data + (size_t)j * ldd, cptr(j), sizeof(double) * rows());
            return;
        }
        materialise().to_host(data, ldd);
    }

    void from_host(const double *data, int64_t ldd)
    {
        orthogonalized_ = 0;
        if (!store_ || n_ <= 0) return;
        if (!in_basis()) {
            for (int j = 0; j < n_; ++j) memcpy(cptr(j), data + (size_t)j * ldd, sizeof(double) * rows());
            return;
        }
        HipMultiVectorWrapper X(basis_->m_local, n_, basis_->ctx);
        X.from_host(data, ldd);
        SubspaceMultiVector tmp = Absorb(basis_, X);
        for (int j = 0; j < n_; ++j) memcpy(cptr(j), tmp.cptr(j), sizeof(double) * ld());
    }
    int64_t local_rows() const { return in_basis() ? basis_->m_local : rows(); }
    int orthogonalized() const { return orthogonalized_; }
    void set_orthogonalized(int n) { orthogonalized_ = n; }
    int capacity() const { return store_ ? store_->ncap - c0_ : 0; }
    bool replicated() const { return !in_basis(); }
    const double *host_data() const { return cptr(); }

    static SubspaceMultiVector Absorb(std::shared_ptr<SubspaceBasis> const &b, HipMultiVectorWrapper const &X)
    {
        const int n = X.N();
        SubspaceMultiVector out(b, n);
        b->absorb_filled(n, [&](int t0, int j0, int w) { return hip_ok(rails_panel_copy(b->ctx, X.panel(), X.offset() + j0, w, b->P.panel(), t0), "rails_panel_copy"); },
                         [&](int j0) { return out.cptr(j0); });
        return out;
    }
};

inline SubspaceMultiVector operator*(double d, SubspaceMultiVector const &o)
{
    SubspaceMultiVector out(o);
    out *= d;
    return out;
}

class SubspaceOperator
{
    HipOperatorWrapper A_;
    std::shared_ptr<SubspaceBasis> basis_;

public:
    SubspaceOperator() {}
    SubspaceOperator(HipOperatorWrapper const &A, std::shared_ptr<SubspaceBasis> const &b) : A_(A), basis_(b) {}
    virtual ~SubspaceOperator() {}

    int M() const { return A_.M(); }
    int N() const { return A_.N(); }
    SubspaceOperator transpose() const { return SubspaceOperator(A_.transpose(), basis_); }
    double norm() const { return A_.norm(); }

    SubspaceMultiVector operator*(SubspaceMultiVector const &X) const
    {
        SubspaceBasis &b = *basis_;
        const int n = X.N();
        SubspaceMultiVector out(basis_, n);
        if (n <= 0) return out;
        HipMultiVectorWrapper Xd = X.materialise();
        auto product = [&](int t0, int j0, int w) { return A_.apply_into((w == 1) ? Xd.view(j0) : Xd.view(j0, j0 + w - 1), b.P, t0); };
        const int wl = n - (n - 1) / 64 * 64;
        const bool pre = b.prefetch_random && !b.cached_valid && wl < 64;
        const int n_main = pre ? n - wl : n;
        b.absorb_filled(n_main, product, [&](int j0) { return out.cptr(j0); });
        if (!pre) return out;
        std::vector<double> coef;
        b.absorb_filled(wl + 1, [&](int t0, int, int) {
            const bool ok = product(t0, n_main, wl);
            return hip_ok(rails_panel_random(b.ctx, b.P.panel(), t0 + wl, 1), "rails_panel_random") && ok;
        }, [&](int) { return coef.resize((size_t)b.row_cap * (wl + 1)), coef.data(); });
        for (int j = 0; j < wl; ++j) memcpy(out.cptr(n_main + j), coef.data() + (size_t)j * b.row_cap, sizeof(double) * b.row_cap);
        if (!b.cached_random || b.cached_random->ld != b.row_cap) b.cached_random = b.new_store(1, true);
        memcpy(b.cached_random->col(0), coef.data() + (size_t)wl * b.row_cap, sizeof(double) * b.row_cap);
        b.cached_valid = true;
        b.n_prefetched++;
        return out;
    }
};

}

#endif
```

Measured before the change: 237.9.

## Fuse orthogonalisation tail GEMM+Gram, mirror small results to pinned, fuse random column into SpMM

Adds a fused kernel that applies the Cholesky-inverse GEMM and accumulates the Gram of the result in one pass, so the panel does not have to be re-read for the second Gram. Reduction and Cholesky kernels can now write their outputs straight into pinned host memory, removing separate device-to-host copies. The narrow SpMM kernel can also generate the prefetched random column inline, avoiding a separate random-fill launch. All three are enabled by default through an environment flag. The cost is more kernel complexity and a new path that only applies when w is at most 32.

```diff
diff --git a/include/rails_hip.h b/include/rails_hip.h
--- a/include/rails_hip.h
+++ b/include/rails_hip.h
@@ -155,6 +155,17 @@
 int rails_update_gram_deferred_out(rails_ctx *ctx, double alpha, const rails_panel *X, int xc0, int k, const double *C_host, int ldc, int r,
                                    const rails_panel *Y, int yc0, rails_panel *Yout, int oc0, int r2, int slot);
 int rails_deferred_fetch(rails_ctx *ctx, int slot, int64_t n, double *host_out);
+int rails_panel_gemm_gram_deferred(rails_ctx *ctx, double alpha, const rails_panel *X, int xc0, int w, int slot_c, rails_panel *Y, int yc0,
+                                   int slot_g);
+
+#define RAILS_FUSED_TAIL_GEMM_GRAM 2
+#define RAILS_FUSED_TAIL_MIRRORS 4
+#define RAILS_FUSED_TAIL_RANDOM_COLUMN 8
+#define RAILS_FUSED_TAIL_ALL 14
+int rails_ctx_set_fused_tail(rails_ctx *ctx, int parts);
+int rails_ctx_fused_tail(rails_ctx *ctx);
+
+int rails_spmm_random_column(rails_ctx *ctx, rails_csr *A, int trans, const rails_panel *X, int xc0, int nc, rails_panel *Y, int yc0, int *fused);
 
 int rails_panel_gemm_wide(rails_ctx *ctx, double alpha, const rails_panel *X, int xc0, int k, const double *C_host, int ldc, int r,
                           double beta, rails_panel *Y, int yc0);
diff --git a/rails_amd/_lib.py b/rails_amd/_lib.py
--- a/rails_amd/_lib.py
+++ b/rails_amd/_lib.py
@@ -31,6 +31,10 @@
     "rails_panel_gemm_deferred": (C.c_int, [_vp, C.c_double, _vp, C.c_int, C.c_int, C.c_int, C.c_int, C.c_int, C.c_double, _vp, C.c_int]),
     "rails_chol_inverse_deferred": (C.c_int, [_vp, C.c_int, C.c_int, C.c_int]),
     "rails_deferred_fetch": (C.c_int, [_vp, C.c_int, C.c_int64, _dp]),
+    "rails_panel_gemm_gram_deferred": (C.c_int, [_vp, C.c_double, _vp, C.c_int, C.c_int, C.c_int, _vp, C.c_int, C.c_int]),
+    "rails_ctx_set_fused_tail": (C.c_int, [_vp, C.c_int]),
+    "rails_ctx_fused_tail": (C.c_int, [_vp]),
+    "rails_spmm_random_column": (C.c_int, [_vp, _vp, C.c_int, _vp, C.c_int, C.c_int, _vp, C.c_int, _ip]),
     "rails_ctx_stats": (C.c_int, [_vp, C.c_char_p, C.c_int]),
     "rails_ctx_set_seed": (C.c_int, [_vp, C.c_uint64, C.c_uint64]),
     "rails_ctx_rng_state": (C.c_int, [_vp, C.POINTER(C.c_uint64), C.POINTER(C.c_uint64)]),
diff --git a/rails_amd/csrc/ctx.hip b/rails_amd/csrc/ctx.hip
--- a/rails_amd/csrc/ctx.hip
+++ b/rails_amd/csrc/ctx.hip
@@ -110,13 +110,22 @@
     RAILS_REQUIRE(c && buf && cap > 0, "rails_ctx_stats: bad argument");
     int n = snprintf(buf, (size_t)cap,
                      "{\"orth_block\": %ld, \"orth_columnwise\": %ld, \"spmm_tiled\": %ld, \"spmm_planes\": %ld, \"spmm_halo_overlapped\": %ld, \"spmm_sweep\": %ld, \"spmm_rowgather\": %ld, \"spmm_callback\": %ld, \"device_allocations\": %ld, \"allreduce\": %ld, "
-                     "\"lanczos\": %ld, \"lanczos_start\": %ld, \"orth_repair\": %ld, \"update_gram_fused\": %ld, \"rowquad\": %ld, \"orth_range\": %ld, \"orth_range_passes\": %ld, \"orth_range_syncs\": %ld, \"gpu_busy_ms\": %.3f}",
-                     c->n_orth_block, c->n_orth_columnwise, c->n_spmm_tiled, c->n_spmm_planes, c->n_spmm_overlapped, c->n_spmm_sweep, c->n_spmm_rowgather, c->n_spmm_callback, c->n_dev_alloc, c->n_allreduce, c->n_lanczos, c->n_lanczos_start, c->n_orth_repair, c->n_update_gram_fused, c->n_rowquad, c->n_orth_range, c->n_orth_range_passes, c->n_orth_range_syncs, c->gpu_busy_ms);
+                     "\"lanczos\": %ld, \"lanczos_start\": %ld, \"orth_repair\": %ld, \"update_gram_fused\": %ld, \"rowquad\": %ld, \"orth_range\": %ld, \"orth_range_passes\": %ld, \"orth_range_syncs\": %ld, \"gemm_gram_fused\": %ld, \"spmm_random_column\": %ld, \"gpu_busy_ms\": %.3f}",
+                     c->n_orth_block, c->n_orth_columnwise, c->n_spmm_tiled, c->n_spmm_planes, c->n_spmm_overlapped, c->n_spmm_sweep, c->n_spmm_rowgather, c->n_spmm_callback, c->n_dev_alloc, c->n_allreduce, c->n_lanczos, c->n_lanczos_start, c->n_orth_repair, c->n_update_gram_fused, c->n_rowquad, c->n_orth_range, c->n_orth_range_passes, c->n_orth_range_syncs, c->n_gemm_gram_fused, c->n_spmm_random_column, c->gpu_busy_ms);
     RAILS_REQUIRE(n > 0 && n < cap, "rails_ctx_stats: buffer too small");
     return RAILS_OK;
 }
 
 extern "C" void *rails_ctx_stream(rails_ctx *c) { return c ? (void *)c->stream : nullptr; }
+
+extern "C" int rails_ctx_set_fused_tail(rails_ctx *c, int parts)
+{
+    RAILS_REQUIRE(c && parts >= 0 && (parts & ~RAILS_FUSED_TAIL_ALL) == 0, "rails_ctx_set_fused_tail: bad argument (parts = %d)", parts);
+    c->fused_tail = parts;
+    return RAILS_OK;
+}
+
+extern "C" int rails_ctx_fused_tail(rails_ctx *c) { return c ? rails_fused_tail(c) : 0; }
 
 extern "C" int rails_ctx_set_meter(rails_ctx *c, int on)
 {
@@ -496,24 +505,14 @@
     }
 }
 
-__device__ __forceinline__ uint64_t splitmix64(uint64_t x)
-{
-    x += 0x9E3779B97F4A7C15ull;
-    x = (x ^ (x >> 30)) * 0xBF58476D1CE4E5B9ull;
-    x = (x ^ (x >> 27)) * 0x94D049BB133111EBull;
-    return x ^ (x >> 31);
-}
-
 __global__ void k_random(double *__restrict__ P, int ld, int64_t m, int nc, uint64_t seed, uint64_t stream, int64_t row0)
 {
-    uint64_t hs = splitmix64(seed ^ splitmix64(stream * 0xD1342543DE82EF95ull + 0x632BE59BD9B4E019ull));
+    uint64_t hs = rails_random_stream_hash(seed, stream);
     int64_t total = m * nc;
     for (int64_t idx = (int64_t)blockIdx.x * blockDim.x + threadIdx.x; idx < total; idx += (int64_t)gridDim.x * blockDim.x) {
         int64_t r = idx / nc;
         int cidx = (int)(idx - r * nc);
-        uint64_t h = splitmix64(hs ^ splitmix64((uint64_t)(row0 + r) * 0x9E3779B97F4A7C15ull + (uint64_t)cidx * 0xC2B2AE3D27D4EB4Full + 1));
-        double u = (double)(h >> 11) * (1.0 / 9007199254740992.0);
-        P[r * ld + cidx] = 2.0 * u - 1.0;
+        P[r * ld + cidx] = rails_random_value(hs, row0 + r, cidx);
     }
 }
 
diff --git a/rails_amd/csrc/dense.hip b/rails_amd/csrc/dense.hip
--- a/rails_amd/csrc/dense.hip
+++ b/rails_amd/csrc/dense.hip
@@ -96,7 +96,8 @@
 #include "dense_gram_cols.inc"
 }
 
-__global__ __launch_bounds__(1024) void k_reduce_partials(const double *__restrict__ partial, int64_t nslab, int64_t n, double *__restrict__ out)
+__global__ __launch_bounds__(1024) void k_reduce_partials(const double *__restrict__ partial, int64_t nslab, int64_t n, double *__restrict__ out,
+                                                          double *__restrict__ mirror)
 {
     __shared__ double sh[16][64];
     const int tx = threadIdx.x & 63, ty = threadIdx.x >> 6;
@@ -111,6 +112,7 @@
 #pragma unroll
         for (int g = 0; g < 16; ++g) r += sh[g][tx];
         out[e] = r;
+        if (mirror) mirror[e] = r;
     }
 }
 
@@ -350,7 +352,7 @@
     return RAILS_OK;
 }
 
-int rails_gram_dev(rails_ctx *c, const double *X, int ldx, const double *Y, int ldy, int64_t m, int a, int b, double *C_dev)
+int rails_gram_dev(rails_ctx *c, const double *X, int ldx, const double *Y, int ldy, int64_t m, int a, int b, double *C_dev, double *mirror)
 {
     if (a <= 0 || b <= 0) return RAILS_OK;
     int64_t nslab, rps;
@@ -381,7 +383,7 @@
         launch_gram<2, 4>(c, X, ldx, a, Y, ldy, b, m, rps, nslab, c->ws);
     else
         launch_gram<2, 4>(c, X, ldx, a, Y, ldy, b, m, rps, nslab, c->ws);
-    RAILS_LAUNCH(k_reduce_partials, dim3((unsigned)((n + 63) / 64)), dim3(1024), 0, c->stream, c->ws, nslab, (int64_t)n, C_dev);
+    RAILS_LAUNCH(k_reduce_partials, dim3((unsigned)((n + 63) / 64)), dim3(1024), 0, c->stream, c->ws, nslab, (int64_t)n, C_dev, mirror);
     RAILS_HIP_CHECK(hipGetLastError());
     return RAILS_OK;
 }
@@ -389,6 +391,7 @@
 int rails_gram2_dev(rails_ctx *c, const double *X1, int ldx1, int a1, const double *X2, int ldx2, int a2, const double *Y, int ldy, int64_t m, int b,
                     double *C_dev)
 {
+    double *const mirror = nullptr;
     const int a = a1 + a2;
     if (a <= 0 || b <= 0) return RAILS_OK;
     int64_t nslab, rps;
@@ -404,7 +407,7 @@
         launch_gram2<8, 1>(c, X1, ldx1, a1, X2, ldx2, a, Y, ldy, b, m, rps, nslab, c->ws);
     else
         launch_gram2<4, 2>(c, X1, ldx1, a1, X2, ldx2, a, Y, ldy, b, m, rps, nslab, c->ws);
-    RAILS_LAUNCH(k_reduce_partials, dim3((unsigned)((n + 63) / 64)), dim3(1024), 0, c->stream, c->ws, nslab, (int64_t)n, C_dev);
+    RAILS_LAUNCH(k_reduce_partials, dim3((unsigned)((n + 63) / 64)), dim3(1024), 0, c->stream, c->ws, nslab, (int64_t)n, C_dev, mirror);
     RAILS_HIP_CHECK(hipGetLastError());
     return RAILS_OK;
 }
@@ -423,12 +426,13 @@
     size_t n = (size_t)a * b;
     RAILS_TRY(rails_small_reserve(c, n * sizeof(double)));
     RAILS_TRY(rails_pinned_reserve(c, n * sizeof(double)));
+    const bool by_producer = X->m > 0 && rails_producer_mirrors(c);
     if (X->m > 0)
-        RAILS_TRY(rails_gram_dev(c, X->d + xc0, X->ld, Y->d + yc0, Y->ld, X->m, a, b, c->small));
+        RAILS_TRY(rails_gram_dev(c, X->d + xc0, X->ld, Y->d + yc0, Y->ld, X->m, a, b, c->small, by_producer ? c->pinned : nullptr));
     else
         RAILS_HIP_CHECK(hipMemsetAsync(c->small, 0, n * sizeof(double), c->stream));
     RAILS_TRY(rails_allreduce_dev(c, c->small, n));
-    RAILS_HIP_CHECK(hipMemcpyAsync(c->pinned, c->small, n * sizeof(double), hipMemcpyDeviceToHost, c->stream));
+    if (!by_producer) RAILS_HIP_CHECK(hipMemcpyAsync(c->pinned, c->small, n * sizeof(double), hipMemcpyDeviceToHost, c->stream));
     RAILS_HIP_CHECK(rails_stream_sync(c));
     for (int j = 0; j < b; ++j) memcpy(C_host + (size_t)j * ldc, c->pinned + (size_t)j * a, sizeof(double) * a);
     return RAILS_OK;
@@ -516,7 +520,7 @@
     RAILS_TRY(rails_ws_reserve(c, (size_t)nslab * nc * sizeof(double)));
     const int vec_ok = ((((uintptr_t)X) & 15) == 0 && (ldx % 2) == 0) ? 1 : 0;
     RAILS_LAUNCH(k_colnorms2, dim3((unsigned)nslab), dim3(256), 0, c->stream, X, ldx, nc, m, rps, tx_bits, vec_ok, c->ws);
-    RAILS_LAUNCH(k_reduce_partials, dim3((unsigned)((nc + 63) / 64)), dim3(1024), 0, c->stream, c->ws, nslab, (int64_t)nc, out_dev);
+    RAILS_LAUNCH(k_reduce_partials, dim3((unsigned)((nc + 63) / 64)), dim3(1024), 0, c->stream, c->ws, nslab, (int64_t)nc, out_dev, (double *)nullptr);
     RAILS_HIP_CHECK(hipGetLastError());
     return RAILS_OK;
 }
@@ -548,7 +552,7 @@
     for (int64_t q = (int64_t)blockIdx.x * blockDim.x + threadIdx.x; q < n; q += (int64_t)gridDim.x * blockDim.x) dst[q] = src[(q / k) * ld + (q % k)];
 }
 
-__global__ __launch_bounds__(64) void k_small_chol(const double *__restrict__ G, int w, double *__restrict__ M)
+__global__ __launch_bounds__(64) void k_small_chol(const double *__restrict__ G, int w, double *__restrict__ M, double *__restrict__ mirror )
 {
     constexpr int LD = 49;
     __shared__ double S[48 * LD], Ri[48 * LD], d[48];
@@ -582,7 +586,135 @@
     __syncthreads();
     for (int q = t; q < w * w; q += 64) {
         const int j = q / w, i = q % w;
-        M[q] = i <= j ? Ri[j * LD + i] / d[i] : 0.0;
+        const double v = i <= j ? Ri[j * LD + i] / d[i] : 0.0;
+        M[q] = v;
+        if (mirror) mirror[q] = v;
+    }
+}
+
+template <int T, bool VEC>
+__global__ __launch_bounds__(256) __attribute__((amdgpu_waves_per_eu(3, 8))) void k_panel_gemm_gram(double alpha, const double *X, int ldx, int w, const double *__restrict__ C, double *Yp, int ldy, int64_t m,
+                                                         int64_t rows_per_slab, double *__restrict__ partial)
+{
+    constexpr int KC = 32, RL = 16 * T + 4;
+    __shared__ double Cs[KC * RL];
+    __shared__ double red[T * T * 256];
+    const int lane = threadIdx.x & 63;
+    const int wave = threadIdx.x >> 6;
+    const int li = lane & 15, kk = lane >> 4;
+    const int64_t r_begin = (int64_t)blockIdx.x * rows_per_slab;
+    int64_t r_end = r_begin + rows_per_slab;
+    if (r_end > m) r_end = m;
+    for (int idx = threadIdx.x; idx < KC * 16 * T; idx += 256) {
+        const int kl = idx % KC, j = idx / KC;
+        Cs[kl * RL + j] = (kl < w && j < w) ? C[kl + (int64_t)j * w] : 0.0;
+    }
+    __syncthreads();
+    const double *crow = &Cs[(4 * kk) * RL + li];
+
+    v4f64 acc2[T][T];
+#pragma unroll
+    for (int i = 0; i < T; ++i)
+#pragma unroll
+        for (int j = 0; j < T; ++j) acc2[i][j] = (v4f64){0.0, 0.0, 0.0, 0.0};
+
+    const int rin = 16 * (li >> 2) + 4 * wave + (li & 3);
+    auto fetch = [&](int64_t base, double (*xs)[4]) {
+        const int64_t row = base + rin;
+        const bool rok = row < r_end;
+        const double *xrow = X + (rok ? row : r_end - 1) * ldx;
+#pragma unroll
+        for (int h = 0; h < 2; ++h) {
+            const int c0 = 16 * h + 4 * kk;
+            if (VEC) {
+#pragma unroll
+                for (int q = 0; q < 2; ++q) {
+                    const int cq = c0 + 2 * q;
+                    const v2f64 t = *reinterpret_cast<const v2f64 *>(xrow + (cq < w ? cq : 0));
+                    xs[h][2 * q] = (rok && cq < w) ? t.x : 0.0;
+                    xs[h][2 * q + 1] = (rok && cq + 1 < w) ? t.y : 0.0;
+                }
+            } else {
+#pragma unroll
+                for (int s = 0; s < 4; ++s) {
+                    const double t = xrow[c0 + s < w ? c0 + s : 0];
+                    xs[h][s] = (rok && c0 + s < w) ? t : 0.0;
+                }
+            }
+        }
+    };
+    double xa[2][4], xn[2][4];
+    if (r_begin < r_end) fetch(r_begin, xa);
+    for (int64_t base = r_begin; base < r_end; base += 64) {
+        const bool more = base + 64 < r_end;
+        if (more) fetch(base + 64, xn);
+        v4f64 acc[T];
+#pragma unroll
+        for (int t = 0; t < T; ++t) acc[t] = (v4f64){0.0, 0.0, 0.0, 0.0};
+#pragma unroll
+        for (int h = 0; h < 2; ++h)
+#pragma unroll
+            for (int s = 0; s < 4; ++s)
+#pragma unroll
+                for (int t = 0; t < T; ++t) acc[t] = mfma_f64(xa[h][s], crow[(16 * h + s) * RL + 16 * t], acc[t]);
+#pragma unroll
+        for (int v = 0; v < 4; ++v) {
+            const int64_t row = base + 16 * v + 4 * wave + kk;
+            const bool rok = row < r_end;
+            double g[T];
+#pragma unroll
+            for (int t = 0; t < T; ++t) {
+                const double val = alpha * acc[t][v];
+                if (rok && 16 * t + li < w) Yp[row * ldy + 16 * t + li] = val;
+                g[t] = rok ? val : 0.0;
+            }
+#pragma unroll
+            for (int i = 0; i < T; ++i)
+#pragma unroll
+                for (int j = i; j < T; ++j) acc2[i][j] = mfma_f64(g[i], g[j], acc2[i][j]);
+        }
+        if (more) {
+#pragma unroll
+            for (int h = 0; h < 2; ++h)
+#pragma unroll
+                for (int s = 0; s < 4; ++s) xa[h][s] = xn[h][s];
+        }
+    }
+
+    for (int ww = 1; ww < 4; ++ww) {
+        if (wave == ww) {
+#pragma unroll
+            for (int i = 0; i < T; ++i)
+#pragma unroll
+                for (int j = i; j < T; ++j)
+#pragma unroll
+                    for (int v = 0; v < 4; ++v) red[((i * T + j) * 4 + v) * 64 + lane] = acc2[i][j][v];
+        }
+        __syncthreads();
+        if (wave == 0) {
+#pragma unroll
+            for (int i = 0; i < T; ++i)
+#pragma unroll
+                for (int j = i; j < T; ++j)
+#pragma unroll
+                    for (int v = 0; v < 4; ++v) acc2[i][j][v] += red[((i * T + j) * 4 + v) * 64 + lane];
+        }
+        __syncthreads();
+    }
+    if (wave == 0) {
+        double *P = partial + (int64_t)blockIdx.x * w * w;
+#pragma unroll
+        for (int i = 0; i < T; ++i)
+#pragma unroll
+            for (int j = i; j < T; ++j)
+#pragma unroll
+                for (int v = 0; v < 4; ++v) {
+                    const int ci = 16 * i + kk + 4 * v, cj = 16 * j + li;
+                    if (ci < w && cj < w) {
+                        P[ci + (int64_t)cj * w] = acc2[i][j][v];
+                        if (j > i) P[cj + (int64_t)ci * w] = acc2[i][j][v];
+                    }
+                }
     }
 }
 
@@ -617,13 +749,14 @@
     RAILS_REQUIRE(a >= 1 && b >= 1 && xc0 >= 0 && yc0 >= 0 && xc0 + a <= X->cap && yc0 + b <= Y->cap && X->m == Y->m, "rails_gram_deferred: bad windows");
     const size_t n = (size_t)a * b;
     RAILS_SLOT_CHECK(slot, n, "rails_gram_deferred");
-    double *out = c->defer_dev + (size_t)slot * c->defer_slot;
+    double *out = c->defer_dev + (size_t)slot * c->defer_slot, *pin = c->defer_pin + (size_t)slot * c->defer_slot;
+    const bool by_producer = X->m > 0 && rails_producer_mirrors(c);
     if (X->m > 0)
-        RAILS_TRY(rails_gram_dev(c, X->d + xc0, X->ld, Y->d + yc0, Y->ld, X->m, a, b, out));
+        RAILS_TRY(rails_gram_dev(c, X->d + xc0, X->ld, Y->d + yc0, Y->ld, X->m, a, b, out, by_producer ? pin : nullptr));
     else
         RAILS_HIP_CHECK(hipMemsetAsync(out, 0, n * sizeof(double), c->stream));
     RAILS_TRY(rails_allreduce_dev(c, out, n));
-    RAILS_HIP_CHECK(hipMemcpyAsync(c->defer_pin + (size_t)slot * c->defer_slot, out, n * sizeof(double), hipMemcpyDeviceToHost, c->stream));
+    if (!by_producer) RAILS_HIP_CHECK(hipMemcpyAsync(pin, out, n * sizeof(double), hipMemcpyDeviceToHost, c->stream));
     return RAILS_OK;
 }
 
@@ -644,6 +777,47 @@
         C = c->small;
     }
     return rails_panel_gemm_dev(c, alpha, X->d + xc0, X->ld, k, C, r, beta, Y->d + yc0, Y->ld, X->m);
+}
+
+extern "C" int rails_panel_gemm_gram_deferred(rails_ctx *c, double alpha, const rails_panel *X, int xc0, int w, int slot_c, rails_panel *Y, int yc0, int slot_g)
+{
+    if (c) hipSetDevice(c->device);
+    RAILS_REQUIRE(c && X && Y, "rails_panel_gemm_gram_deferred: null argument");
+    RAILS_REQUIRE(w >= 1 && w <= 32 && xc0 >= 0 && yc0 >= 0 && xc0 + w <= X->cap && yc0 + w <= Y->cap && X->m == Y->m && slot_c != slot_g,
+                  "rails_panel_gemm_gram_deferred: bad shapes (w = %d)", w);
+    const size_t n = (size_t)w * w;
+    RAILS_SLOT_CHECK(slot_c, n, "rails_panel_gemm_gram_deferred");
+    RAILS_SLOT_CHECK(slot_g, n, "rails_panel_gemm_gram_deferred");
+    if (X->d == Y->d) RAILS_REQUIRE(xc0 == yc0 || xc0 + w <= yc0 || yc0 + w <= xc0, "rails_panel_gemm_gram_deferred: partially overlapping windows of one panel");
+    const double *C = c->defer_dev + (size_t)slot_c * c->defer_slot;
+    double *out = c->defer_dev + (size_t)slot_g * c->defer_slot, *pin = c->defer_pin + (size_t)slot_g * c->defer_slot;
+    const int64_t m = X->m;
+    const bool by_producer = m > 0 && rails_producer_mirrors(c);
+    if (m > 0) {
+        int64_t nslab, rps;
+        gram_slabs(m, w, w, &nslab, &rps);
+        RAILS_TRY(rails_ws_reserve(c, (size_t)nslab * n * sizeof(double)));
+        const double *Xp = X->d + xc0;
+        double *Yp = Y->d + yc0;
+        const bool vec = ((((uintptr_t)Xp) & 15) == 0 && (X->ld % 2) == 0) && ((w % 2) == 0 || xc0 + w + 1 <= X->ld);
+        const dim3 grid((unsigned)nslab), block(256);
+        if (w <= 16) {
+            if (vec)
+                RAILS_LAUNCH((k_panel_gemm_gram<1, true>), grid, block, 0, c->stream, alpha, Xp, X->ld, w, C, Yp, Y->ld, m, rps, c->ws);
+            else
+                RAILS_LAUNCH((k_panel_gemm_gram<1, false>), grid, block, 0, c->stream, alpha, Xp, X->ld, w, C, Yp, Y->ld, m, rps, c->ws);
+        } else if (vec)
+            RAILS_LAUNCH((k_panel_gemm_gram<2, true>), grid, block, 0, c->stream, alpha, Xp, X->ld, w, C, Yp, Y->ld, m, rps, c->ws);
+        else
+            RAILS_LAUNCH((k_panel_gemm_gram<2, false>), grid, block, 0, c->stream, alpha, Xp, X->ld, w, C, Yp, Y->ld, m, rps, c->ws);
+        RAILS_LAUNCH(k_reduce_partials, dim3((unsigned)((n + 63) / 64)), dim3(1024), 0, c->stream, c->ws, nslab, (int64_t)n, out, by_producer ? pin : (double *)nullptr);
+        RAILS_HIP_CHECK(hipGetLastError());
+        c->n_gemm_gram_fused++;
+    } else
+        RAILS_HIP_CHECK(hipMemsetAsync(out, 0, n * sizeof(double), c->stream));
+    RAILS_TRY(rails_allreduce_dev(c, out, n));
+    if (!by_producer) RAILS_HIP_CHECK(hipMemcpyAsync(pin, out, n * sizeof(double), hipMemcpyDeviceToHost, c->stream));
+    return RAILS_OK;
 }
 
 template <int NBW, int NE>
@@ -795,7 +969,9 @@
     if (Y->d == Yout->d) RAILS_REQUIRE(yc0 == oc0 || yc0 + r <= oc0 || oc0 + r <= yc0, "rails_update_gram_deferred: partially overlapping windows of one panel");
     const size_t n = (size_t)k * r2;
     RAILS_SLOT_CHECK(slot, n, "rails_update_gram_deferred");
-    double *out = c->defer_dev + (size_t)slot * c->defer_slot;
+    double *out = c->defer_dev + (size_t)slot * c->defer_slot, *pin = c->defer_pin + (size_t)slot * c->defer_slot;
+    const bool by_producer = X->m > 0 && rails_producer_mirrors(c);
+    double *const mirror = by_producer ? pin : nullptr;
     if (X->m == 0) {
         RAILS_HIP_CHECK(hipMemsetAsync(out, 0, n * sizeof(double), c->stream));
     } else {
@@ -824,17 +1000,17 @@
                 launch_update_gram<6>(c, ne, grid, alpha, Xp, X->ld, k, c->small, r, Ypp, Y->ld, Yop, Yout->ld, r2, X->m, ntiles);
             else
                 launch_update_gram<8>(c, ne, grid, alpha, Xp, X->ld, k, c->small, r, Ypp, Y->ld, Yop, Yout->ld, r2, X->m, ntiles);
-            RAILS_LAUNCH(k_reduce_partials, dim3((unsigned)((n + 63) / 64)), dim3(1024), 0, c->stream, c->ws, (int64_t)grid, (int64_t)n, out);
+            RAILS_LAUNCH(k_reduce_partials, dim3((unsigned)((n + 63) / 64)), dim3(1024), 0, c->stream, c->ws, (int64_t)grid, (int64_t)n, out, mirror);
             RAILS_HIP_CHECK(hipGetLastError());
             c->n_update_gram_fused++;
         } else {
             if (Yop != Ypp) RAILS_TRY(rails_panel_copy(c, Y, yc0, r, Yout, oc0));
             RAILS_TRY(rails_panel_gemm_dev(c, alpha, Xp, X->ld, k, c->small, r, 1.0, Yop, Yout->ld, X->m));
-            RAILS_TRY(rails_gram_dev(c, Xp, X->ld, Yop, Yout->ld, X->m, k, r2, out));
+            RAILS_TRY(rails_gram_dev(c, Xp, X->ld, Yop, Yout->ld, X->m, k, r2, out, mirror));
         }
     }
     RAILS_TRY(rails_allreduce_dev(c, out, n));
-    RAILS_HIP_CHECK(hipMemcpyAsync(c->defer_pin + (size_t)slot * c->defer_slot, out, n * sizeof(double), hipMemcpyDeviceToHost, c->stream));
+    if (!by_producer) RAILS_HIP_CHECK(hipMemcpyAsync(pin, out, n * sizeof(double), hipMemcpyDeviceToHost, c->stream));
     return RAILS_OK;
 }
 
@@ -850,10 +1026,12 @@
     RAILS_REQUIRE(c && w >= 1 && w <= 48 && slot_in != slot_out, "rails_chol_inverse_deferred: bad argument (w = %d)", w);
     RAILS_SLOT_CHECK(slot_in, (size_t)w * w, "rails_chol_inverse_deferred");
     RAILS_SLOT_CHECK(slot_out, (size_t)w * w, "rails_chol_inverse_deferred");
-    RAILS_LAUNCH(k_small_chol, dim3(1), dim3(64), 0, c->stream, c->defer_dev + (size_t)slot_in * c->defer_slot, w, c->defer_dev + (size_t)slot_out * c->defer_slot);
+    double *pin = c->defer_pin + (size_t)slot_out * c->defer_slot;
+    const bool by_producer = rails_producer_mirrors(c);
+    RAILS_LAUNCH(k_small_chol, dim3(1), dim3(64), 0, c->stream, c->defer_dev + (size_t)slot_in * c->defer_slot, w, c->defer_dev + (size_t)slot_out * c->defer_slot,
+                 by_producer ? pin : (double *)nullptr);
     RAILS_HIP_CHECK(hipGetLastError());
-    RAILS_HIP_CHECK(hipMemcpyAsync(c->defer_pin + (size_t)slot_out * c->defer_slot, c->defer_dev + (size_t)slot_out * c->defer_slot, (size_t)w * w * sizeof(double),
-                                   hipMemcpyDeviceToHost, c->stream));
+    if (!by_producer) RAILS_HIP_CHECK(hipMemcpyAsync(pin, c->defer_dev + (size_t)slot_out * c->defer_slot, (size_t)w * w * sizeof(double), hipMemcpyDeviceToHost, c->stream));
     return RAILS_OK;
 }
 
diff --git a/rails_amd/csrc/rails_internal.h b/rails_amd/csrc/rails_internal.h
--- a/rails_amd/csrc/rails_internal.h
+++ b/rails_amd/csrc/rails_internal.h
@@ -79,7 +79,22 @@
     long n_orth_block = 0, n_orth_columnwise = 0, n_spmm_tiled = 0, n_spmm_planes = 0, n_spmm_overlapped = 0, n_spmm_sweep = 0, n_spmm_rowgather = 0, n_spmm_callback = 0, n_dev_alloc = 0, n_allreduce = 0, n_lanczos = 0, n_lanczos_start = 0, n_orth_repair = 0, n_update_gram_fused = 0, n_rowquad = 0;
     long n_orth_range = 0, n_orth_range_passes = 0, n_orth_range_syncs = 0;
     int last_update_gram_nbw = 0, last_gram_cols_ti = 0, last_gemm_wide_tr = 0;
-};
+    int fused_tail = -1;
+    long n_gemm_gram_fused = 0, n_spmm_random_column = 0;
+};
+
+inline int rails_fused_tail_from_env()
+{
+    const char *e = getenv("RAILS_SUBSPACE_FUSED_TAIL");
+    const int v = e ? atoi(e) : 1;
+    return v == 1 ? RAILS_FUSED_TAIL_ALL : (v & RAILS_FUSED_TAIL_ALL);
+}
+inline int rails_fused_tail(rails_ctx *c)
+{
+    if (c->fused_tail < 0) c->fused_tail = rails_fused_tail_from_env();
+    return c->fused_tail;
+}
+inline bool rails_producer_mirrors(rails_ctx *c) { return (rails_fused_tail(c) & RAILS_FUSED_TAIL_MIRRORS) && c->nranks <= 1 && !c->allreduce && !c->rccl; }
 
 constexpr int RAILS_METER_PAIRS = 512;
 inline bool rails_meter_before(rails_ctx *c)
@@ -213,6 +228,26 @@
     return e ? atoi(e) : def;
 }
 
+#ifdef __HIPCC__
+__device__ __forceinline__ uint64_t rails_splitmix64(uint64_t x)
+{
+    x += 0x9E3779B97F4A7C15ull;
+    x = (x ^ (x >> 30)) * 0xBF58476D1CE4E5B9ull;
+    x = (x ^ (x >> 27)) * 0x94D049BB133111EBull;
+    return x ^ (x >> 31);
+}
+__device__ __forceinline__ uint64_t rails_random_stream_hash(uint64_t seed, uint64_t stream)
+{
+    return rails_splitmix64(seed ^ rails_splitmix64(stream * 0xD1342543DE82EF95ull + 0x632BE59BD9B4E019ull));
+}
+__device__ __forceinline__ double rails_random_value(uint64_t hs, int64_t global_row, int column)
+{
+    const uint64_t h = rails_splitmix64(hs ^ rails_splitmix64((uint64_t)global_row * 0x9E3779B97F4A7C15ull + (uint64_t)column * 0xC2B2AE3D27D4EB4Full + 1));
+    const double u = (double)(h >> 11) * (1.0 / 9007199254740992.0);
+    return 2.0 * u - 1.0;
+}
+#endif
+
 int rails_ws_reserve(rails_ctx *ctx, size_t bytes);
 void rails_library_gemm_release(rails_ctx *ctx);
 int rails_small_reserve(rails_ctx *ctx, size_t bytes);
@@ -240,7 +275,7 @@
                      int x_room, bool *done);
 void rails_tiled_release(rails_csr *A);
 int rails_gram_dev(rails_ctx *ctx, const double *X, int ldx, const double *Y, int ldy, int64_t m, int a, int b,
-                   double *C_dev);
+                   double *C_dev, double *mirror = nullptr);
 int rails_panel_gemm_dev(rails_ctx *ctx, double alpha, const double *X, int ldx, int k, const double *C_dev,
                          int r, double beta, double *Y, int ldy, int64_t m);
 int rails_colnorms2_dev(rails_ctx *ctx, const double *X, int ldx, int64_t m, int nc, double *out_dev);
diff --git a/rails_amd/csrc/solver_capi.cpp b/rails_amd/csrc/solver_capi.cpp
--- a/rails_amd/csrc/solver_capi.cpp
+++ b/rails_amd/csrc/solver_capi.cpp
@@ -352,9 +352,9 @@
     s->sub_hist = solver.residual_history();
     s->sub_profile = solver.profile();
     char buf[1536];
-    snprintf(buf, sizeof(buf), "{\"dim\": %d, \"absorb\": %ld, \"absorb_columns\": %ld, \"one_by_one\": %ld, \"dropped\": %ld, \"compress\": %ld, \"materialise\": %ld, \"prefetched_random\": %ld, \"second_rounds\": %ld, \"delicate_blocks\": %ld, \"reprojected_blocks\": %ld, \"overlapped_blocks\": %ld, \"scratch_blocks\": %ld, \"replaced_columns\": %ld, \"verified\": %d, \"verify_representation\": %.3e, \"verify_orthonormality\": %.3e, \"seconds\": {\"materialise\": %.4f, \"absorb\": %.4f, \"compress_qr\": %.4f, \"compress_rotate\": %.4f, "
+    snprintf(buf, sizeof(buf), "{\"dim\": %d, \"absorb\": %ld, \"absorb_columns\": %ld, \"one_by_one\": %ld, \"dropped\": %ld, \"compress\": %ld, \"materialise\": %ld, \"prefetched_random\": %ld, \"second_rounds\": %ld, \"delicate_blocks\": %ld, \"reprojected_blocks\": %ld, \"overlapped_blocks\": %ld, \"scratch_blocks\": %ld, \"fused_tail_blocks\": %ld, \"replaced_columns\": %ld, \"verified\": %d, \"verify_representation\": %.3e, \"verify_orthonormality\": %.3e, \"seconds\": {\"materialise\": %.4f, \"absorb\": %.4f, \"compress_qr\": %.4f, \"compress_rotate\": %.4f, "
              "\"compress_coefficients\": %.4f}}",
-             basis->dim, basis->n_absorb, basis->n_absorb_cols, basis->n_single, basis->n_dropped, basis->n_compress, basis->n_materialise, basis->n_prefetched, basis->n_second_round, basis->n_delicate, basis->n_reprojected, basis->n_overlapped, basis->n_scratch_blocks, basis->n_replaced, basis->verify ? 1 : 0, basis->verify_repr, basis->verify_orth,
+             basis->dim, basis->n_absorb, basis->n_absorb_cols, basis->n_single, basis->n_dropped, basis->n_compress, basis->n_materialise, basis->n_prefetched, basis->n_second_round, basis->n_delicate, basis->n_reprojected, basis->n_overlapped, basis->n_scratch_blocks, basis->n_fused_tail_blocks, basis->n_replaced, basis->verify ? 1 : 0, basis->verify_repr, basis->verify_orth,
              basis->t_materialise, basis->t_absorb, basis->t_qr, basis->t_rotate, basis->t_recoef);
     s->sub_stats = buf;
     if (basis->failed) {
diff --git a/rails_amd/csrc/spmm.hip b/rails_amd/csrc/spmm.hip
--- a/rails_amd/csrc/spmm.hip
+++ b/rails_amd/csrc/spmm.hip
@@ -97,9 +97,15 @@
     }
 }
 
+struct SpmmRandom {
+    uint64_t seed = 0, stream = 0;
+    int64_t row0 = 0;
+    bool done = false;
+};
 struct RowSpan {
     int64_t r0 = 0, nrows = -1;
     hipStream_t st = nullptr;
+    SpmmRandom *rnd = nullptr;
 };
 #define RAILS_LAUNCH_ON(st__, kern__, grid__, block__, lds__, ...)                           \
     do {                                                                                     \
@@ -212,11 +218,11 @@
     }
 }
 
-template <int RPG, bool GHOST, int LPR = 8>
+template <int RPG, bool GHOST, int LPR = 8, bool RAND = false>
 __global__ __launch_bounds__(256) void k_spmm_narrow(int64_t m, const int64_t *__restrict__ rowptr, const int32_t *__restrict__ col,
                                                      const double *__restrict__ val, const double *__restrict__ X, uint32_t ldx8,
                                                      const double *__restrict__ Xg, uint32_t ldg8, double *__restrict__ Y, int ldy, int nc,
-                                                     int64_t blocks_per_xcd, int y_vec, int64_t mc)
+                                                     int64_t blocks_per_xcd, int y_vec, int64_t mc, uint64_t rnd_seed, uint64_t rnd_stream, int64_t rnd_row0)
 {
     constexpr int GROUPS = 256 / LPR, ROWS = GROUPS * RPG, CAP = 2048;
     __shared__ double s_val[CAP];
@@ -236,6 +242,8 @@
         }
         __syncthreads();
     }
+    if (RAND && threadIdx.x < ROWS && r0 + threadIdx.x < m)
+        Y[(r0 + threadIdx.x) * ldy + nc] = rails_random_value(rails_random_stream_hash(rnd_seed, rnd_stream), rnd_row0 + r0 + threadIdx.x, 0);
     const int cb = l * 2;
     if (cb >= nc) return;
     const bool full = (cb + 2 <= nc);
@@ -320,12 +328,16 @@
     const int64_t grid = bpx * 8 * nchunks;
     RAILS_REQUIRE(grid <= 0x7fffffffLL, "rails_spmm: grid too large");
     const int y_vec = ch.y_vec ? 1 : 0;
-    if (ch.kind == RowChoice::NARROW && !ch.ghost)
+    if (ch.kind == RowChoice::NARROW && !ch.ghost && sp.rnd && sp.r0 == 0 && sp.nrows < 0 && st == c->stream && nchunks == 1) {
+        RAILS_LAUNCH((k_spmm_narrow<RPG, false, NLPR, true>), dim3((unsigned)grid), dim3(256), 0, c->stream, m_rows, rowptr, A->col, A->val, X, (uint32_t)ldx * 8u, X, 0u, Y, ldy,
+                     nc, bpx, y_vec, A->m, sp.rnd->seed, sp.rnd->stream, sp.rnd->row0);
+        sp.rnd->done = true;
+    } else if (ch.kind == RowChoice::NARROW && !ch.ghost)
         RAILS_LAUNCH_ON(st, (k_spmm_narrow<RPG, false, NLPR>), dim3((unsigned)grid), dim3(256), 0, m_rows, rowptr, A->col, A->val, X, (uint32_t)ldx * 8u, X, 0u, Y, ldy, nc,
-                        bpx, y_vec, A->m);
+                        bpx, y_vec, A->m, (uint64_t)0, (uint64_t)0, (int64_t)0);
     else if (ch.kind == RowChoice::NARROW)
         RAILS_LAUNCH_ON(st, (k_spmm_narrow<RPG, true, NLPR>), dim3((unsigned)grid), dim3(256), 0, m_rows, rowptr, A->col, A->val, X, (uint32_t)ldx * 8u, Xg,
-                        (uint32_t)ldg * 8u, Y, ldy, nc, bpx, y_vec, A->m);
+                        (uint32_t)ldg * 8u, Y, ldy, nc, bpx, y_vec, A->m, (uint64_t)0, (uint64_t)0, (int64_t)0);
     else {
         const int lds_cap = 2048;
         RAILS_LAUNCH_ON(st, (k_spmm_rowgather_cc<LPR, RPG>), dim3((unsigned)grid), dim3(256), (size_t)lds_cap * 12, m_rows, rowptr, A->col, A->val, X, ldx, Xg, ldg, Y,
@@ -627,7 +639,7 @@
     return RAILS_OK;
 }
 
-extern "C" int rails_spmm(rails_ctx *c, rails_csr *A, int trans, const rails_panel *X, int xc0, int nc, rails_panel *Y, int yc0)
+static int spmm_product(rails_ctx *c, rails_csr *A, int trans, const rails_panel *X, int xc0, int nc, rails_panel *Y, int yc0, SpmmRandom *rnd)
 {
     if (c) hipSetDevice(c->device);
     rails_slow_guard slow__(c, "rails_spmm", nc, A ? A->m : 0);
@@ -758,10 +770,35 @@
         const bool x_vec2 = (xc0 & 1) == 0 && (X->ld % 2 == 0) && (ldg % 2 == 0);
         const bool y_vec2 = (yc0 & 1) == 0 && (Y->ld % 2 == 0);
         const RowChoice ch = rails_row_choice(row_facts(A, nc, x_vec2, y_vec2, vec2, Xp, X->ld, Xg, ldg, -1));
-        RAILS_TRY(launch_rows(c, A, ch, Xp, X->ld, Xg, ldg, Yp, Y->ld, nc));
+        RowSpan all;
+        all.rnd = rnd;
+        RAILS_TRY(launch_rows(c, A, ch, Xp, X->ld, Xg, ldg, Yp, Y->ld, nc, all));
         A->last_kernel = ROW_KERNEL[ch.kind];
         c->n_spmm_rowgather++;
     }
     RAILS_HIP_CHECK(hipGetLastError());
     return RAILS_OK;
 }
+
+extern "C" int rails_spmm(rails_ctx *c, rails_csr *A, int trans, const rails_panel *X, int xc0, int nc, rails_panel *Y, int yc0)
+{
+    return spmm_product(c, A, trans, X, xc0, nc, Y, yc0, nullptr);
+}
+
+extern "C" int rails_spmm_random_column(rails_ctx *c, rails_csr *A, int trans, const rails_panel *X, int xc0, int nc, rails_panel *Y, int yc0, int *fused)
+{
+    RAILS_REQUIRE(c && A && X && Y, "rails_spmm_random_column: null argument");
+    RAILS_REQUIRE(nc >= 0 && yc0 >= 0 && yc0 + nc + 1 <= Y->cap, "rails_spmm_random_column: Y columns [%d,%d] outside capacity %d", yc0, yc0 + nc, Y->cap);
+    if (X->d == Y->d) RAILS_REQUIRE(xc0 + nc <= yc0 || yc0 + nc + 1 <= xc0, "rails_spmm_random_column: X and Y windows alias");
+    SpmmRandom rnd;
+    rnd.seed = c->seed;
+    rnd.stream = c->next_stream;
+    rnd.row0 = c->row0;
+    const bool may_fuse = (rails_fused_tail(c) & RAILS_FUSED_TAIL_RANDOM_COLUMN) != 0 && !trans;
+    RAILS_TRY(spmm_product(c, A, trans, X, xc0, nc, Y, yc0, may_fuse ? &rnd : nullptr));
+    if (fused) *fused = rnd.done ? 1 : 0;
+    if (!rnd.done) return rails_panel_random(c, Y, yc0 + nc, 1);
+    c->next_stream++;
+    c->n_spmm_random_column++;
+    return RAILS_OK;
+}
diff --git a/rails_amd/include/rails/HipWrappers.hpp b/rails_amd/include/rails/HipWrappers.hpp
--- a/rails_amd/include/rails/HipWrappers.hpp
+++ b/rails_amd/include/rails/HipWrappers.hpp
@@ -577,6 +577,12 @@
     {
         if (X.n_ <= 0) return true;
         return hip_ok(rails_spmm(ctx_, h_->A, transpose_ ? 1 : 0, X.panel_->p, X.c0_, X.n_, Y.panel_->p, Y.c0_ + ycol), "rails_spmm");
+    }
+
+    bool apply_into_with_random(HipMultiVectorWrapper const &X, HipMultiVectorWrapper &Y, int ycol) const
+    {
+        if (X.n_ <= 0) return hip_ok(rails_panel_random(ctx_, Y.panel_->p, Y.c0_ + ycol, 1), "rails_panel_random");
+        return hip_ok(rails_spmm_random_column(ctx_, h_->A, transpose_ ? 1 : 0, X.panel_->p, X.c0_, X.n_, Y.panel_->p, Y.c0_ + ycol, nullptr), "rails_spmm_random_column");
     }
 
     double norm_rectangular(int64_t m, int64_t nc) const
diff --git a/rails_amd/include/rails/SubspaceWrappers.hpp b/rails_amd/include/rails/SubspaceWrappers.hpp
--- a/rails_amd/include/rails/SubspaceWrappers.hpp
+++ b/rails_amd/include/rails/SubspaceWrappers.hpp
@@ -68,6 +68,14 @@
     enum { SLOT_C2 = 0, SLOT_G = 1, SLOT_M1 = 2, SLOT_G2 = 3, SLOT_M2 = 4, N_SLOTS = 5 };
     bool block_scratch = !(getenv("RAILS_SUBSPACE_BLOCK_SCRATCH") && atoi(getenv("RAILS_SUBSPACE_BLOCK_SCRATCH")) == 0);
     long n_scratch_blocks = 0;
+    int fused_tail = rails_fused_tail_env();
+    long n_fused_tail_blocks = 0;
+    static int rails_fused_tail_env()
+    {
+        const char *e = getenv("RAILS_SUBSPACE_FUSED_TAIL");
+        const int v = e ? atoi(e) : 1;
+        return v == 1 ? RAILS_FUSED_TAIL_ALL : (v & RAILS_FUSED_TAIL_ALL);
+    }
     std::shared_ptr<PanelHandle> S;
     rails_panel *scratch_panel(int w)
     {
@@ -81,6 +89,7 @@
     {
         P.set_global_rows(mg);
         P.resize(0);
+        rails_ctx_set_fused_tail(c, fused_tail);
     }
 
     void preallocate_compress_panel()
@@ -317,8 +326,13 @@
         }
         ok = ok && hip_ok(rails_gram_deferred(ctx, xp, x0, w, xp, x0, w, SLOT_G), "rails_gram_deferred");
         ok = ok && hip_ok(rails_chol_inverse_deferred(ctx, SLOT_G, w, SLOT_M1), "rails_chol_inverse_deferred");
-        ok = ok && hip_ok(rails_panel_gemm_deferred(ctx, 1.0, xp, x0, w, SLOT_M1, w, w, 0.0, bp, b0), "rails_panel_gemm_deferred");
-        ok = ok && hip_ok(rails_gram_deferred(ctx, bp, b0, w, bp, b0, w, SLOT_G2), "rails_gram_deferred");
+        if ((fused_tail & RAILS_FUSED_TAIL_GEMM_GRAM) && w <= 32) {
+            ok = ok && hip_ok(rails_panel_gemm_gram_deferred(ctx, 1.0, xp, x0, w, SLOT_M1, bp, b0, SLOT_G2), "rails_panel_gemm_gram_deferred");
+            n_fused_tail_blocks++;
+        } else {
+            ok = ok && hip_ok(rails_panel_gemm_deferred(ctx, 1.0, xp, x0, w, SLOT_M1, w, w, 0.0, bp, b0), "rails_panel_gemm_deferred");
+            ok = ok && hip_ok(rails_gram_deferred(ctx, bp, b0, w, bp, b0, w, SLOT_G2), "rails_gram_deferred");
+        }
         ok = ok && hip_ok(rails_chol_inverse_deferred(ctx, SLOT_G2, w, SLOT_M2), "rails_chol_inverse_deferred");
         ok = ok && hip_ok(rails_panel_gemm_deferred(ctx, 1.0, bp, b0, w, SLOT_M2, w, w, 0.0, pp, dim), "rails_panel_gemm_deferred");
         if (!ok) return fail("the overlapped block orthogonalisation could not be queued");
@@ -964,8 +978,7 @@
         if (!pre) return out;
         std::vector<double> coef;
         b.absorb_filled(wl + 1, [&](int t0, int, int) {
-            const bool ok = product(t0, n_main, wl);
-            return hip_ok(rails_panel_random(b.ctx, b.P.panel(), t0 + wl, 1), "rails_panel_random") && ok;
+            return A_.apply_into_with_random((wl == 1) ? Xd.view(n_main) : Xd.view(n_main, n_main + wl - 1), b.P, t0);
         }, [&](int) { return coef.resize((size_t)b.row_cap * (wl + 1)), coef.data(); });
         for (int j = 0; j < wl; ++j) memcpy(out.cptr(n_main + j), coef.data() + (size_t)j * b.row_cap, sizeof(double) * b.row_cap);
         if (!b.cached_random || b.cached_random->ld != b.row_cap) b.cached_random = b.new_store(1, true);
```

Result: faster. 241.0, median of 6 (+1.3%).
